# vitoplantamura/OnnxStream

Hardware: AMD Instinct MI355X
Metric: sd15_unet_step_latency_ms+images_per_sec_512x512_20step (higher is better)
Workload: dtype f16

## Files before the change

### include/osgpu.h

```cpp
#ifndef OSGPU_H
#define OSGPU_H

#include <stddef.h>
#include <stdint.h>

#ifdef __cplusplus
extern "C" {
#endif

typedef struct osg_ctx osg_ctx;
typedef struct osg_graph osg_graph;

typedef enum { OSG_U8 = 1, OSG_F16 = 2, OSG_F32 = 3, OSG_I64 = 4 } osg_dtype;

typedef enum {
  OSG_ACT_NONE = 0,
  OSG_ACT_SILU = 1,
  OSG_ACT_SIGMOID = 2,
  OSG_ACT_GEGLU = 3
} osg_act;

typedef enum {
  OSG_UN_SIGMOID = 0,
  OSG_UN_ERF = 1,
  OSG_UN_SQRT = 2,
  OSG_UN_SIN = 3,
  OSG_UN_COS = 4,
  OSG_UN_NEG = 5,
  OSG_UN_POW = 6,
  OSG_UN_SILU = 7,
  OSG_UN_GELU_ERF = 8
} osg_unary_kind;

typedef enum {
  OSG_BIN_ADD = 0,
  OSG_BIN_SUB = 1,
  OSG_BIN_MUL = 2,
  OSG_BIN_DIV = 3
} osg_binary_kind;

int osg_device_count(void);
int osg_init(int device, osg_ctx** out);
void osg_destroy(osg_ctx* ctx);
const char* osg_last_error(const osg_ctx* ctx);
const char* osg_device_name(const osg_ctx* ctx);
void* osg_stream(const osg_ctx* ctx);
int osg_set_autotune(osg_ctx* ctx, int on);
int osg_tune_misses(void);

int osg_malloc(osg_ctx* ctx, size_t bytes, void** dptr);
int osg_free(osg_ctx* ctx, void* dptr);
int osg_upload(osg_ctx* ctx, void* dst, const void* host_src, size_t bytes);
int osg_upload_sync(osg_ctx* ctx, void* dst, const void* host_src, size_t bytes);
int osg_host_register(osg_ctx* ctx, void* host_ptr, size_t bytes);
int osg_host_unregister(osg_ctx* ctx, void* host_ptr);
int osg_upload_pinned(osg_ctx* ctx, void* dst, const void* pinned_host_src, size_t bytes);
int osg_upload_pinned_async(osg_ctx* ctx, void* dst, const void* pinned_host_src, size_t bytes);
int osg_copy_fence(osg_ctx* ctx);
int osg_download(osg_ctx* ctx, void* host_dst, const void* src, size_t bytes);
int osg_marker_record(osg_ctx* ctx, int slot);
int osg_copy_wait_marker(osg_ctx* ctx, int slot);
int osg_copy(osg_ctx* ctx, void* dst, const void* src, size_t bytes);
int osg_memset(osg_ctx* ctx, void* dst, int value, size_t bytes);
int osg_sync(osg_ctx* ctx);

int osg_graph_begin(osg_ctx* ctx);
int osg_graph_end(osg_ctx* ctx, osg_graph** out);
int osg_graph_launch(osg_ctx* ctx, osg_graph* g);
void osg_graph_destroy(osg_graph* g);

int osg_timer_start(osg_ctx* ctx);
int osg_timer_stop(osg_ctx* ctx, float* ms);
int osg_timer_mark(osg_ctx* ctx, int index);
int osg_timer_between(osg_ctx* ctx, int a, int b, float* ms);

void osg_range_push(const char* name);
void osg_range_pop(void);

int osg_conv2d_nhwc(osg_ctx* ctx, osg_dtype dtype, const void* x, const void* w_ohwi, const void* bias, osg_dtype bias_dtype,
                    const void* residual, void* y, int N, int H, int W, int Cin, int Cout, int KH, int KW, int stride_h,
                    int stride_w, int pad_top, int pad_left, int pad_bottom, int pad_right, osg_act act);

int osg_conv2d_nhwc_rb(osg_ctx* ctx, osg_dtype dtype, const void* x, const void* w_ohwi, const void* bias, osg_dtype bias_dtype,
                       const void* image_bias, long image_bias_ld, const void* residual, void* y, int N, int H, int W, int Cin, int Cout,
                       int KH, int KW, int stride_h, int stride_w, int pad_top, int pad_left, int pad_bottom, int pad_right, osg_act act);

int osg_conv2d_nhwc_v(osg_ctx* ctx, osg_dtype dtype, const void* x, const void* w_ohwi, const void* bias, osg_dtype bias_dtype,
                      const void* image_bias, long image_bias_ld, const void* residual, void* y, long y_ld, void* y2, long y2_ld, int N, int H, int W,
                      int Cin, int Cout, int KH, int KW, int stride_h, int stride_w, int pad_top, int pad_left, int pad_bottom, int pad_right,
                      osg_act act);

int osg_gemm(osg_ctx* ctx, osg_dtype dtype, const void* A, const void* B, int b_is_nk, const void* bias, osg_dtype bias_dtype,
             const void* residual, void* C, int M, int N, int K, int batch, long stride_a, long stride_b, long stride_c,
             osg_act act);

int osg_gemm_w8(osg_ctx* ctx, const void* A, const void* Bq_nk, float w_scale, int w_zero_point, const void* bias, osg_dtype bias_dtype,
                const void* residual, void* C, int M, int N, int K, osg_act act);
int osg_conv2d_nhwc_w8(osg_ctx* ctx, const void* x, const void* wq_ohwi, float w_scale, int w_zero_point, const void* bias,
                       osg_dtype bias_dtype, const void* image_bias, long image_bias_ld, const void* residual, void* y, int N, int H, int W,
                       int Cin, int Cout, int KH, int KW, int stride_h, int stride_w, int pad_top, int pad_left, int pad_bottom,
                       int pad_right, osg_act act);
int osg_gemm_w8_v(osg_ctx* ctx, const void* A, const void* Bq_nk, float w_scale, int w_zero_point, const float* w_scale_vec,
                  const float* w_zero_point_vec, const void* bias, osg_dtype bias_dtype, const void* residual, void* C, int M, int N, int K,
                  osg_act act);
int osg_conv2d_nhwc_w8_v(osg_ctx* ctx, const void* x, const void* wq_ohwi, float w_scale, int w_zero_point, const float* w_scale_vec,
                         const float* w_zero_point_vec, const void* bias, osg_dtype bias_dtype, const void* image_bias, long image_bias_ld,
                         const void* residual, void* y, long y_ld, void* y2, long y2_ld, int N, int H, int W, int Cin, int Cout, int KH, int KW,
                         int stride_h, int stride_w, int pad_top, int pad_left, int pad_bottom, int pad_right, osg_act act);

int osg_transpose_kn_to_nk(osg_ctx* ctx, osg_dtype dtype, const void* src_kn, void* dst_nk, int K, int N);
int osg_gemm_ln(osg_ctx* ctx, const void* x, const void* w_nk_folded, const float* c1, const float* c2, float eps, const float* rowstats,
                const void* residual, void* y, int M, int N, int K, osg_act act);
int osg_gemm_rowstats(osg_ctx* ctx, const void* A, const void* B_nk, const void* bias, osg_dtype bias_dtype, const void* residual, void* C,
                      int M, int N, int K, osg_act act, float* rowstats);
int osg_last_route(const osg_ctx* ctx, int out[5]);
int osg_last_epilogue(const osg_ctx* ctx, int out[2]);
int osg_last_kernel(const osg_ctx* ctx, int out[8]);

int osg_gemm_kernarg_check(osg_ctx* ctx, long lda, int splits);
int osg_attention_kernarg_check(osg_ctx* ctx, long kv_stride, int heads, int kv_div);

int osg_attention(osg_ctx* ctx, osg_dtype dtype, const void* q, const void* k, const void* v, void* o, int heads, int Tq, int Tkv,
                  int D, float scale, int k_is_dt);
int osg_attention_strided(osg_ctx* ctx, osg_dtype dtype, const void* q, long q_tok, long q_head, long q_batch, const void* k,
                          long k_tok, long k_head, long k_batch, const void* v, long v_tok, long v_head, long v_batch, void* o,
                          long o_tok, long o_head, long o_batch, int batch, int heads, int Tq, int Tkv, int D, float scale);
typedef struct {
  const void *a1, *x0;
  const void *wo1, *bo1;
  const void *g2, *be2;
  float eps2;
  const void *wq2, *bq2;
  const void *kp, *vtp;
  float scale;
  int Tk;
  const void *wo2, *bo2;
  const void *g3, *be3;
  float eps3;
  const void *w1, *b1, *w2, *b2;
  const void *wpo, *bpo, *xin;
  void *out, *out2;
  long ldo, ldo2;
  int M, rows_per_img, C, heads;
  void* dbg[8];
  int rows_per_block;
} osg_tblock_tail_args;
int osg_tblock_tail_supported(int M, int rows_per_img, int C, int heads, int Tk);
int osg_tblock_tail(osg_ctx* ctx, const osg_tblock_tail_args* a);
int osg_tblock_pack_weight(osg_ctx* ctx, const void* w_nk, int N, int K, void* w_kn8);
size_t osg_tblock_kv_pack_elems(int imgs, int heads, int D);
int osg_tblock_kv_pack_jobs(osg_ctx* ctx, const void* base, long ld, int imgs, int Tk, int heads, int njobs, const int* jobs_dev, void* dst);
int osg_rms_norm(osg_ctx* ctx, osg_dtype dtype, const void* x, const void* w, void* y, long rows, int C, float eps);
int osg_rope(osg_ctx* ctx, osg_dtype dtype, const void* x, const void* cos_t, const void* sin_t, void* y, long bh, long T, int d);
int osg_sdpa(osg_ctx* ctx, osg_dtype dtype, const void* q, const void* k, const void* v, const void* mask, void* o, int batch, int q_heads,
             int kv_heads, int Tq, int Tkv, int D, float scale);

int osg_instance_norm(osg_ctx* ctx, osg_dtype dtype, const void* x, const float* scale, const float* bias, void* y, int rows,
                      long L, int n_scale, float eps);
int osg_group_norm_nhwc(osg_ctx* ctx, osg_dtype dtype, const void* x, const void* gamma, const void* beta, void* y, int N, long HW,
                        int C, int groups, float eps, osg_act act);
int osg_set_stat_sinks(osg_ctx* ctx, void* table0, int groups0, int cpg0, int ch_off0, void* table1, int groups1, int cpg1, int ch_off1, int rows_per_image);
int osg_group_norm_stats_nhwc(osg_ctx* ctx, const void* x, const void* gamma, const void* beta, void* y, int N, long HW, int C, int G, float eps, osg_act act,
                              const void* stat_table);
int osg_layer_norm(osg_ctx* ctx, osg_dtype dtype, const void* x, const void* gamma, const void* beta, void* y, long rows, int C,
                   float eps);
int osg_reduce_mean_last(osg_ctx* ctx, osg_dtype dtype, const void* x, void* y, long rows, long C);
int osg_softmax_last(osg_ctx* ctx, osg_dtype dtype, const void* x, void* y, long rows, long C);

int osg_unary(osg_ctx* ctx, osg_dtype dtype, osg_unary_kind kind, const void* x, void* y, long n, float param);
int osg_binary(osg_ctx* ctx, osg_dtype dtype, osg_binary_kind kind, const void* a, const long* a_shape, const void* b,
               const long* b_shape, void* y, int rank);
int osg_geglu(osg_ctx* ctx, osg_dtype dtype, const void* x, void* y, long rows, long C);

// ... 66 lines not shown
```

### onnxstream_amd/build.py

```python
from __future__ import annotations

import glob
import os
import subprocess
import sys

ROOT = os.path.dirname(os.path.abspath(__file__))
REPO = os.path.dirname(ROOT)
CSRC = os.path.join(ROOT, "csrc")
INC = os.path.join(REPO, "include")
LIB_GPU = os.path.join(ROOT, "libosgpu.so")
LIB_HOST = os.environ.get("OSA_LIB_HOST") or os.path.join(ROOT, "libonnxstream_amd.so")
ORACLE_REF = os.path.join(REPO, "oracle", "_ref", "libonnxstream_ref.so")
HIPCC = os.environ.get("HIPCC", "/opt/rocm/bin/hipcc")
NO_PRELOAD = os.environ.get("OSG_NO_KERNARG_PRELOAD", "") not in ("", "0")
PRELOAD_FLAGS = [] if NO_PRELOAD else ["-mllvm", "-amdgpu-kernarg-preload-count=16"]
LIB_GPU_BUILT = os.path.join(ROOT, "libosgpu_nopreload.so") if NO_PRELOAD else LIB_GPU


def _newer(target, deps):
    if not os.path.exists(target):
        return True
    t = os.path.getmtime(target)
    return any(os.path.getmtime(d) > t for d in deps)


def _run(cmd, **kw):
    r = subprocess.run(cmd, stdout=subprocess.PIPE, stderr=subprocess.STDOUT, text=True, **kw)
    if r.returncode != 0:
        sys.stderr.write(r.stdout)
        raise RuntimeError("build failed: " + " ".join(cmd))
    return r.stdout


def build_gpu(force=False, verbose=False):
    srcs = sorted(glob.glob(os.path.join(CSRC, "osg_*.hip")))
    hdrs = sorted(glob.glob(os.path.join(CSRC, "*.h"))) + [os.path.join(INC, "osgpu.h")]
    objdir = os.path.join(CSRC, "build", "nopreload") if NO_PRELOAD else os.path.join(CSRC, "build")
    os.makedirs(objdir, exist_ok=True)
    objs, procs = [], []
    for s in srcs:
        o = os.path.join(objdir, os.path.basename(s)[:-4] + ".o")
        objs.append(o)
        if force or _newer(o, [s] + hdrs):
            cmd = [HIPCC, "--offload-arch=gfx950", "-O3", "-std=c++17", "-fPIC", "-mllvm", "-amdgpu-mfma-vgpr-form"] + PRELOAD_FLAGS + ["-I" + INC, "-I" + CSRC, "-c", s, "-o", o]
            procs.append((cmd, subprocess.Popen(cmd, stdout=subprocess.PIPE, stderr=subprocess.STDOUT, text=True)))
    for cmd, p in procs:
        out, _ = p.communicate()
        if p.returncode != 0:
            sys.stderr.write(out)
            raise RuntimeError("build failed: " + " ".join(cmd))
        if verbose and out:
            print(out)
    if force or procs or _newer(LIB_GPU_BUILT, objs):
        _run([HIPCC, "--offload-arch=gfx950", "-shared", "-fPIC", "-o", LIB_GPU_BUILT] + objs)
    return LIB_GPU_BUILT


def build_host(force=False):
    hdir = os.path.join(CSRC, "host")
    srcs = sorted(glob.glob(os.path.join(hdir, "*.cpp")))
    if not srcs:
        return None
    hdrs = sorted(glob.glob(os.path.join(hdir, "*.h"))) + sorted(glob.glob(os.path.join(hdir, "*.inc"))) + [os.path.join(INC, "osgpu.h")]
    if force or _newer(LIB_HOST, srcs + hdrs):
        _run(["g++", "-std=c++20", "-O2", "-fPIC", "-shared", "-I" + INC, "-I" + hdir, "-o", LIB_HOST] + srcs +
             ["-ldl", "-lpthread"])
    return LIB_HOST


def build_oracle_ref():
    if os.path.isdir("/root/reference/src"):
        _run(["make", "-C", os.path.join(REPO, "oracle"), "ref"])
    return ORACLE_REF if os.path.exists(ORACLE_REF) else None


def build_all(force=False):
    build_gpu(force)
    build_host(force)
    build_oracle_ref()


if __name__ == "__main__":
    build_all("--force" in sys.argv)
    print("built:", LIB_GPU, LIB_HOST if os.path.exists(LIB_HOST) else "(no host yet)")
```

### onnxstream_amd/csrc/host/backend.h

```cpp
#pragma once

#include <dlfcn.h>

#include <stdexcept>
#include <string>

#include "osgpu.h"

namespace onnxstream {

#define OSG_API_LIST(X) \
    X(osg_device_count) X(osg_init) X(osg_destroy) X(osg_last_error) X(osg_device_name) X(osg_stream) \
    X(osg_set_autotune) X(osg_malloc) X(osg_free) X(osg_upload) X(osg_upload_sync) X(osg_host_register) \
    X(osg_host_unregister) X(osg_upload_pinned) X(osg_upload_pinned_async) X(osg_copy_fence) X(osg_download) X(osg_copy) X(osg_memset) X(osg_sync) \
    X(osg_graph_begin) X(osg_graph_end) X(osg_graph_launch) X(osg_graph_destroy) \
    X(osg_timer_start) X(osg_timer_stop) X(osg_conv2d_nhwc) X(osg_conv2d_nhwc_rb) X(osg_conv2d_nhwc_v) X(osg_set_stat_sinks) X(osg_group_norm_stats_nhwc) X(osg_gemm) \
    X(osg_gemm_ln) X(osg_gemm_rowstats) X(osg_gemm_w8) X(osg_conv2d_nhwc_w8) X(osg_gemm_w8_v) X(osg_conv2d_nhwc_w8_v) X(osg_transpose_kn_to_nk) X(osg_attention) \
    X(osg_attention_strided) X(osg_sdpa) X(osg_rms_norm) X(osg_rope) X(osg_instance_norm) X(osg_group_norm_nhwc) X(osg_layer_norm) \
    X(osg_reduce_mean_last) X(osg_softmax_last) X(osg_unary) X(osg_binary) X(osg_geglu) X(osg_transpose) \
    X(osg_copy_2d) X(osg_concat2) X(osg_resize_nearest) X(osg_gather_rows) X(osg_maxpool_nhwc) X(osg_convert) \
    X(osg_sampler_prepare) X(osg_sampler_cfg_euler_a) X(osg_sampler_cfg_multistep) X(osg_sampler_prepare_rescale) X(osg_sampler_prepare_single) X(osg_sampler_euler_a_single) X(osg_sampler_multistep_single) X(osg_decode_gather) X(osg_decode_blend) X(osg_qu8_conv2d_nhwc) X(osg_qu8_conv2d_nhwc_t) X(osg_qu8_conv_tap_sums) X(osg_qu8_gemm) X(osg_qu8_lut) X(osg_qu8_binary) \
    X(osg_qu8_instance_norm) X(osg_qu8_instance_norm_nhwc) X(osg_qu8_affine_act) X(osg_qu8_norm_affine_act_nhwc) X(osg_qu8_softmax_last) X(osg_range_push) X(osg_range_pop) X(osg_marker_record) \
    X(osg_copy_wait_marker) X(osg_timer_mark) X(osg_timer_between) X(osg_tblock_tail_supported) X(osg_tblock_tail) X(osg_tblock_kv_pack_elems) X(osg_tblock_kv_pack_jobs) X(osg_tblock_pack_weight)

struct OsgApi {
#define OSG_FN(name) decltype(&::name) name = nullptr;
    OSG_API_LIST(OSG_FN)
#undef OSG_FN
};

class HipBackend {
public:
    OsgApi api;
    osg_ctx* ctx = nullptr;

    explicit HipBackend(int device) {
        std::string path;
        if (const char* e = std::getenv("OSGPU_LIB")) path = e;
        if (path.empty()) {
            Dl_info info;
            if (dladdr((void*)&HipBackend::anchor, &info) && info.dli_fname) {
                std::string self = info.dli_fname;
                auto p = self.find_last_of('/');
                path = (p == std::string::npos ? std::string(".") : self.substr(0, p)) + "/libosgpu.so";
            } else {
                path = "libosgpu.so";
            }
        }
        m_handle = dlopen(path.c_str(), RTLD_NOW | RTLD_LOCAL);
        if (!m_handle) throw std::runtime_error("HipBackend: unable to load " + path + ": " + dlerror() + " (no CPU fallback exists)");
#define OSG_FN(name)                                                                                   \
    api.name = reinterpret_cast<decltype(api.name)>(dlsym(m_handle, #name));                           \
    if (!api.name) throw std::runtime_error(std::string("HipBackend: symbol missing in libosgpu.so: ") + #name);
        OSG_API_LIST(OSG_FN)
#undef OSG_FN
        if (api.osg_device_count() <= 0)
            throw std::runtime_error("HipBackend: no HIP device visible; the MI355X backend has no CPU fallback");
        int rc = api.osg_init(device, &ctx);
        if (rc) throw std::runtime_error("HipBackend: osg_init(device " + std::to_string(device) + ") failed with code " + std::to_string(rc));
    }

    ~HipBackend() {
        if (ctx) api.osg_destroy(ctx);
    }

    HipBackend(const HipBackend&) = delete;
    HipBackend& operator=(const HipBackend&) = delete;

    void check(int rc, const char* what) const {
        if (rc) throw std::runtime_error(std::string(what) + ": " + api.osg_last_error(ctx));
    }

    void* malloc(size_t bytes) {
        void* p = nullptr;
        check(api.osg_malloc(ctx, bytes, &p), "osg_malloc");
        return p;
    }
    void free(void* p) { if (p) api.osg_free(ctx, p); }

private:
    static void anchor() {}
    void* m_handle = nullptr;
};

}
```

### onnxstream_amd/csrc/host/exports.cpp

```cpp
#include <cstdio>
#include <cstring>

#include "onnxstream.h"
#include "plan.h"

using namespace onnxstream;

namespace {

char* dup_cstr(const std::string& s) {
    char* p = (char*)std::malloc(s.size() + 1);
    std::memcpy(p, s.c_str(), s.size() + 1);
    return p;
}

struct Handle {
    explicit Handle(int threads) : model(threads) {}
    Model model;
    std::string definition;
    std::string provider;
};

const char* dtype_name(TensorDataType t) {
    switch (t) {
// ... 119 lines not shown
            r->data_num = t.get_vector<float>().size();
            r->data = t.get_vector<float>().data();
            return r;
        }
    return nullptr;
}

void* model_hip_get_tensor_batch(Handle* h, char* name, unsigned int index) {
    struct Ret {
        size_t dims_num;
        size_t* dims;
        size_t data_num;
        float* data;
    };
    for (auto& t : h->model.m_data)
        if (t.m_name == name) {
            Tensor* src = &t;
            if (index > 0) {
                if (!t.m_batch || index - 1 >= t.m_batch->size()) return nullptr;
                src = &(*t.m_batch)[index - 1];
            }
            if (src->m_type != TensorDataType::float32) return nullptr;
            Ret* r = (Ret*)std::malloc(sizeof(Ret));
            r->dims_num = src->m_shape.size();
            r->dims = src->m_shape.data();
            r->data_num = src->get_vector<float>().size();
            r->data = src->get_vector<float>().data();
            return r;
        }
    return nullptr;
}

char* model_get_all_tensor_names(Handle* h) {
    std::string out;
    for (auto& t : h->model.m_data) out += (out.empty() ? "" : "|") + t.m_name;
    return dup_cstr(out);
}

void model_run(Handle* h) {
    try {
        h->model.run();
    } catch (const std::exception& e) {
        printf("=== ERROR === %s\n", e.what());
        throw;
    }
}

char* model_run_2(Handle* h) {
    try {
        h->model.run();
        return nullptr;
    } catch (const std::exception& e) {
        return dup_cstr(e.what());
    }
}

void model_clear_tensors(Handle* h) { h->model.m_data.clear(); }

void model_set_option(Handle* h, char* name, unsigned int value) {
    Model& m = h->model;
    const std::string n = name;
    const bool b = value != 0;
    if (n == "use_fp16_arithmetic") m.m_use_fp16_arithmetic = b;
    else if (n == "use_uint8_qdq") m.m_use_uint8_qdq = b;
    else if (n == "use_uint8_arithmetic") m.m_use_uint8_arithmetic = b;
    else if (n == "fuse_ops_in_attention") m.m_fuse_ops_in_attention = b;
    else if (n == "force_fp16_storage") m.m_force_fp16_storage = b;
    else if (n == "support_dynamic_shapes") m.m_support_dynamic_shapes = b;
    else if (n == "use_ops_cache") m.m_use_ops_cache = b;
    else if (n == "use_scaled_dp_attn_op") m.m_use_scaled_dp_attn_op = b;
    else if (n == "use_next_op_cache") m.m_use_next_op_cache = b;
    else if (n == "ops_printf") m.m_ops_printf = b;
    else if (n == "ops_times_printf") m.m_ops_times_printf = b;
    else if (n == "use_nchw_convs") m.m_use_nchw_convs = b;
    else if (n == "range_data_calibrate") m.m_range_data_calibrate = b;
    else if (n == "attention_fused_ops_parts") m.m_attention_fused_ops_parts = value;
    else if (n == "hip_device") m.m_hip_device = (int)value;
    else if (n == "hip_fusion_level") m.m_hip_fusion_level = (int)value;
    else if (n == "hip_use_graph") m.m_hip_use_graph = b;
    else if (n == "hip_autotune") m.m_hip_autotune = b;
    else if (n == "hip_fuse_ln_gemm") m.m_hip_fuse_ln_gemm = b;
    else if (n == "hip_concat_views") m.m_hip_concat_views = b;
    else if (n == "hip_fuse_tblock") m.m_hip_fuse_tblock = b;
    else if (n == "hip_gn_stats") m.m_hip_gn_stats = (int)value;
    else if (n == "hip_stream_weights") m.m_hip_stream_weights = b;
    else if (n == "hip_w8_resident") m.m_hip_w8_resident = b;
    else if (n == "hip_resident_outputs") m.m_hip_resident_outputs = b;
    else {
        const char* err = "model_set_option: 'name' not found.";
        printf("=== ERROR === %s\n", err);
        throw std::invalid_argument(err);
    }
}

void model_add_extra_output(Handle* h, char* name) { h->model.m_extra_outputs.emplace_back(name); }

void model_free_buffer(void* ptr) { std::free(ptr); }

double model_hip_last_pass_ms(Handle* h) { return h->model.hip_last_pass_ms(); }
unsigned long long model_hip_last_kernel_count(Handle* h) { return h->model.hip_last_kernel_count(); }
void model_hip_invalidate_plan(Handle* h) { h->model.hip_invalidate_plan(); }
unsigned long long model_hip_plans_built(Handle* h) { return h->model.hip_plans_built(); }
unsigned long long model_hip_streamed_bytes(Handle* h) { return h->model.hip_streamed_bytes(); }
unsigned long long model_hip_resident_weight_bytes(Handle* h) { return h->model.hip_resident_weight_bytes(); }
void model_hip_set_vram_budget(Handle* h, unsigned long long bytes) { h->model.set_cuda_options(CudaOptions(bytes, false)); }
void model_hip_set_upcast_substrings(Handle* h, const char* list) {
    std::vector<std::string> subs;
    std::string cur;
    for (const char* p = list ? list : ""; ; p++) {
        if (*p == '|' || *p == 0) {
            if (!cur.empty()) subs.push_back(cur);
            cur.clear();
            if (!*p) break;
        } else cur.push_back(*p);
    }
    if (subs.empty()) h->model.m_requires_upcast = nullptr;
    else
        h->model.m_requires_upcast = [subs](const std::string&, const std::string& name) {
            for (auto& s : subs)
                if (name.find(s) != std::string::npos) return true;
            return false;
        };
    h->model.hip_invalidate_plan();
}
void model_hip_add_outputs_convert(Handle* h, char* name) { h->model.m_outputs_convert_set.insert(name); }
int model_hip_drop_tensor(Handle* h, char* name) {
    auto& d = h->model.m_data;
    for (size_t i = 0; i < d.size(); i++)
        if (d[i].m_name == name) { d.erase(d.begin() + i); return 1; }
    return 0;
}
char* model_hip_fetch_tensor(Handle* h, char* name) {
    try {
        h->model.hip_fetch_tensor(name);
        return nullptr;
    } catch (const std::exception& e) {
        return dup_cstr(e.what());
    }
}
int model_hip_rename_tensor(Handle* h, char* from, char* to) {
    for (auto& t : h->model.m_data)
        if (t.m_name == from) { t.m_name = to; return 1; }
    return 0;
}
char* model_hip_replay(Handle* h, int n, float* ms_each) {
    try {
        h->model.hip_replay(n, ms_each);
        return nullptr;
    } catch (const std::exception& e) {
        return dup_cstr(e.what());
    }
}
char* model_hip_set_input(Handle* h, char* name, long long index, const float* data, unsigned long long count) {
    try {
        h->model.hip_set_input(name, (long)index, data, (size_t)count);
        return nullptr;
    } catch (const std::exception& e) {
        return dup_cstr(e.what());
    }
}
char* model_hip_sampler_loop(Handle* h, char* sample_name, char* timestep_name, char* out_name, int steps, int prompts, float* x, const float* noise,
                             const float* c_in, const float* c_out, const float* t, const float* sigma, const float* d_sigma, const float* sigma_up, float guidance, const float* clip,
                             double* ms) {
    try {
        const double v = h->model.hip_sampler_loop(sample_name, timestep_name, out_name, steps, prompts, x, noise, c_in, c_out, t, sigma, d_sigma, sigma_up, guidance, clip);
        if (ms) *ms = v;
// ... 85 lines not shown
```

### onnxstream_amd/csrc/host/lowering_graph.inc

```
    static bool wants_f32(const Operation& op, size_t idx) {
        if (op.m_type == "InstanceNormalization" && (idx == 1 || idx == 2)) return true;
        if (op.m_type == "Resize") return true;
        if (op.m_type == "Pow" && idx == 1) return true;
        return false;
    }

    template <typename T>
    tensor_vector<T> fetch(WeightsProvider* wp, const std::string& fn) {
        if constexpr (std::is_same_v<T, uint8_t>) return wp->get_uint8(fn);
        else if constexpr (std::is_same_v<T, uint16_t>) return wp->get_float16(fn);
        else if constexpr (std::is_same_v<T, float>) return wp->get_float32(fn);
        else return wp->get_int64(fn);
    }

    struct Occ { std::string fn, key; Shape shape; Lay lay; osg_dtype want; long count; };
    Occ resolve(const Operation& op, size_t i, const Tensor& t, TensorDataType ty) const {
        Occ o;
        o.fn = t.m_name;
        o.shape = to_shape(t.m_shape);
        o.lay = Lay::plain;
        auto pos = o.fn.find("_nchw.bin");
        if (pos != std::string::npos) {
            if (o.shape.size() == 3) o.shape.push_back(1);
            if (o.shape.size() != 4) throw std::invalid_argument("Model::get_tensor_data: layout is nhwc but invalid shape.");
// ... 249 lines not shown
            return (sh.size() == 3 && sh[0] == C) || (sh.size() == 4 && sh[1] == C);
        };
        for (size_t i = 0; i < ops().size(); i++) {
            if (!is((int)i, "Mul")) continue;
            Operation& mu = ops()[i];
            if (mu.m_input.size() != 2 || mu.m_output.size() != 1) continue;
            int xi = -1;
            for (int k = 0; k < 2; k++)
                if (act(mu.m_input[k]) && mu.m_input[k].m_shape.size() == 4 && mu.m_input[k].m_shape[0] == 1 && chan_const(mu.m_input[1 - k], (long)mu.m_input[k].m_shape[1])) xi = k;
            if (xi < 0) continue;
            const Tensor x = mu.m_input[xi], gam = mu.m_input[1 - xi];
            const long C = (long)x.m_shape[1];
            const int ad = sole_consumer(mu.m_output[0]);
            if (!is(ad, "Add") || ops()[ad].m_input.size() != 2) continue;
            const int bidx = other(ops()[ad], mu.m_output[0].m_name);
            if (!chan_const(ops()[ad].m_input[bidx], C)) continue;
            const Tensor bet = ops()[ad].m_input[bidx];
            int sg = -1, m2 = -1;
            const std::string& an = ops()[ad].m_output[0].m_name;
            if (use_count(an) == 2) {
                auto it = consumers.find(an);
                if (it != consumers.end() && it->second.size() == 2) {
                    for (int c : it->second)
                        if (is(c, "Sigmoid")) sg = c;
                        else if (is(c, "Mul")) m2 = c;
                    if (sg >= 0 && m2 >= 0 && sole_consumer(ops()[sg].m_output[0]) == m2 && ops()[m2].m_input.size() == 2) {
                        const std::string &p0 = ops()[m2].m_input[0].m_name, &p1 = ops()[m2].m_input[1].m_name, &sn = ops()[sg].m_output[0].m_name;
                        if (!((p0 == an && p1 == sn) || (p0 == sn && p1 == an))) sg = m2 = -1;
                    } else
                        sg = m2 = -1;
                }
            }
            const bool silu = sg >= 0 && m2 >= 0;
            if (!silu && use_count(an) != 1) {
            }
            Operation f;
            const int last = silu ? m2 : ad;
            f.m_name = ops()[last].m_name;
            f.m_type = "osg.qu8.AffineAct";
            f.m_input = {x, gam, bet};
            f.m_output = {ops()[last].m_output[0]};
            f.m_attributes = {{"mul", mu.m_name}, {"add", ops()[ad].m_name}};
            if (silu) {
                f.m_attributes.emplace_back("sigmoid", ops()[sg].m_name);
                f.m_attributes.emplace_back("mul2", ops()[m2].m_name);
            }
            const int nrm = prod_of(x);
            if (is(nrm, "osg.qu8.InstanceNormNHWC") && use_count(x.m_name) == 1) {
                f.m_type = "osg.qu8.NormAffineAct";
                f.m_input = {ops()[nrm].m_input[0], gam, bet, ops()[nrm].m_input[1], ops()[nrm].m_input[2]};
                f.m_attributes.emplace_back("norm", ops()[nrm].m_name);
                for (auto& a : ops()[nrm].m_attributes) f.m_attributes.emplace_back("norm_" + a.first, a.second);
                dead[nrm] = 1;
            }
            dead[i] = 1;
            if (silu) dead[ad] = dead[sg] = 1;
            ops()[last] = std::move(f);
        }
    }

    void run_fusions() {
        dead.assign(ops().size(), 0);
        if (P.u8 && m.m_hip_fusion_level >= 1 && has_type("InstanceNormalization")) { index_graph(); fuse_u8_instance_norm_nhwc(); }
        if (P.u8 && m.m_hip_fusion_level >= 1 && has_type("Mul") && has_type("Add")) { index_graph(); fuse_u8_affine_act(); }
        if (m.m_use_scaled_dp_attn_op && has_type("Softmax")) { index_graph(); fuse_sdpa(); }
        if (P.fusion >= 1) {
            if (m.m_requires_upcast && has_type("Pow") && has_type("ReduceMean")) { index_graph(); fuse_rms_norm(); }
            if (has_type("Neg") && has_type("Slice")) { index_graph(); fuse_rope(); }
            if (has_type("Sigmoid")) { index_graph(); fuse_silu(); }
            if (has_type("InstanceNormalization")) { index_graph(); fuse_group_norm(); }
            if (has_type("ReduceMean") && has_type("Sub")) { index_graph(); fuse_layer_norm(); }
            if (has_type("Erf")) { index_graph(); fuse_geglu(); }
        }
        if (P.fusion >= 2) {
            if (has_type("Softmax")) { index_graph(); fuse_attention(true); }
            if (has_type("MatMul")) { index_graph(); fuse_linear(); }
            if (has_type("Conv") || has_type("osg.Linear")) { index_graph(); fuse_residual(); }
            if (has_type("Conv")) { index_graph(); fuse_conv_act(); }
            if (has_type("osg.GEGLU")) { index_graph(); fuse_linear_geglu(); }
            if (has_type("osg.Attention") && has_type("osg.LayerNorm")) { index_graph(); fuse_tblock_tail(); }
            if (has_type("osg.SiLU")) { index_graph(); cse_silu(); }
            if (has_type("osg.SiLU") && has_type("Gemm")) { index_graph(); fuse_gemm_act(); }
            if (has_type("Conv")) { index_graph(); fuse_image_bias(); }
        } else if (m.m_fuse_ops_in_attention && has_type("Softmax")) {
            index_graph(); fuse_attention(false);
        }
        std::vector<Operation> live;
        for (size_t i = 0; i < ops().size(); i++)
            if (!dead[i]) live.push_back(std::move(ops()[i]));
        ops() = std::move(live);
    }

    void fuse_silu() {
        for (size_t i = 0; i < ops().size(); i++) {
            if (!is((int)i, "Sigmoid")) continue;
            Operation& sg = ops()[i];
            if (sg.m_input.size() != 1 || sg.m_output.size() != 1 || !act(sg.m_input[0])) continue;
            int j = sole_consumer(sg.m_output[0]);
            if (!is(j, "Mul")) continue;
            Operation& mul = ops()[j];
            if (mul.m_input.size() != 2) continue;
            const std::string& s = sg.m_output[0].m_name;
            int o = other(mul, s);
            if (mul.m_input[o].m_name != sg.m_input[0].m_name || mul.m_input[1 - o].m_name != s) continue;
            mul.m_type = "osg.SiLU";
            Tensor x = mul.m_input[o];
            mul.m_input.clear();
            mul.m_input.push_back(x);
            dead[i] = 1;
        }
    }

    void fuse_group_norm() {
        for (size_t i = 0; i < ops().size(); i++) {
            if (!is((int)i, "InstanceNormalization")) continue;
            Operation& in = ops()[i];
            if (in.m_input.size() != 3 || in.m_output.size() != 1) continue;
            const Val* sc = cval(in.m_input[1]);
            const Val* bi = cval(in.m_input[2]);
            if (!sc || !bi || !sc->host_valid || !bi->host_valid) continue;
            bool unit = true;
            for (float f : sc->host_f) unit &= f == 1.0f;
            for (float f : bi->host_f) unit &= f == 0.0f;
            if (!unit) continue;
            int r0 = prod_of(in.m_input[0]);
            if (!is(r0, "Reshape") || use_count(in.m_input[0].m_name) != 1) continue;
            const Tensor& x = ops()[r0].m_input[0];
            if (!act(x) || x.m_shape.size() != 4) continue;
            if (in.m_input[0].m_shape.size() != 3 || in.m_input[0].m_shape[0] != 1) continue;
            long G = (long)in.m_input[0].m_shape[1];
            int r1 = sole_consumer(in.m_output[0]);
            if (!is(r1, "Reshape") || ops()[r1].m_output[0].m_shape != x.m_shape) continue;
            int mu = sole_consumer(ops()[r1].m_output[0]);
            if (!is(mu, "Mul")) continue;
            int gi = other(ops()[mu], ops()[r1].m_output[0].m_name);
            const Val* gam = cval(ops()[mu].m_input[gi]);
            long C = (long)x.m_shape[1];
            auto chan_shape = [&](const Val* v) {
                if (!v || v->numel() != C) return false;
                const Shape& s = v->shape;
                return (s.size() == 3 && s[0] == C) || (s.size() == 4 && s[1] == C);
            };
            if (!chan_shape(gam)) continue;
            int ad = sole_consumer(ops()[mu].m_output[0]);
            if (!is(ad, "Add")) continue;
            int bidx = other(ops()[ad], ops()[mu].m_output[0].m_name);
            if (!chan_shape(cval(ops()[ad].m_input[bidx]))) continue;
            if (C % G || x.m_shape[0] != 1) continue;
            float eps = 1e-5f;
            if (auto* e = attr(in, "epsilon")) eps = std::stof(*e);
            int last = ad;
            bool silu = false;
            int sl = sole_consumer(ops()[ad].m_output[0]);
            if (is(sl, "osg.SiLU")) { silu = true; last = sl; }
            Operation f;
            f.m_name = in.m_name + "_GroupNorm";
            f.m_type = "osg.GroupNorm";
            f.m_input = {x, ops()[mu].m_input[gi], ops()[ad].m_input[bidx]};
            f.m_output = {ops()[last].m_output[0]};
            f.m_attributes = {{"groups", std::to_string(G)}, {"epsilon", std::to_string(eps)}, {"silu", silu ? "1" : "0"}};
            char buf[64];
            snprintf(buf, sizeof buf, "%.9g", eps);
            f.m_attributes[1].second = buf;
            for (int k : {r0, (int)i, r1, mu, ad}) dead[k] = 1;
            if (silu) dead[sl] = 1;
            dead[last] = 0;
// ... 547 lines not shown
            if (op.m_output.size() != 1 || attr(op, "osg_residual")) continue;
            if (attr(op, "osg_act")) continue;
            int ad = sole_consumer(op.m_output[0]);
            if (!is(ad, "Add")) continue;
            int ti = other(ops()[ad], op.m_output[0].m_name);
            const Tensor& t = ops()[ad].m_input[ti];
            const auto& os = op.m_output[0].m_shape;
            if (!act(t) || os.size() != 4 || t.m_shape != std::vector<size_t>{1, os[1], 1, 1}) continue;
            int u1 = prod_of(t);
            if (!is(u1, "Unsqueeze") || use_count(t.m_name) != 1) continue;
            int u0 = prod_of(ops()[u1].m_input[0]);
            if (!is(u0, "Unsqueeze") || use_count(ops()[u1].m_input[0].m_name) != 1) continue;
            const Tensor g = ops()[u0].m_input[0];
            if (!act(g) || g.m_shape != std::vector<size_t>{1, os[1]} || use_count(g.m_name) != 1) continue;
            Operation f = op;
            while (f.m_input.size() < 4) f.m_input.push_back(Tensor());
            f.m_input.push_back(g);
            f.m_attributes.emplace_back("osg_image_bias", "1");
            f.m_output = {ops()[ad].m_output[0]};
            dead[i] = dead[u0] = dead[u1] = 1;
            ops()[ad] = std::move(f);
        }
    }

    void fuse_linear() {
        for (size_t i = 0; i < ops().size(); i++) {
            if (!is((int)i, "MatMul")) continue;
            Operation& mm = ops()[i];
            const Val* w = cval(mm.m_input[1]);
            if (!act(mm.m_input[0]) || !w || w->shape.size() != 2) continue;
            mm.m_type = "osg.Linear";
            int ad = sole_consumer(mm.m_output[0]);
            if (!is(ad, "Add")) continue;
            int bi = other(ops()[ad], mm.m_output[0].m_name);
            const Val* b = cval(ops()[ad].m_input[bi]);
            if (!b || b->shape.size() != 1 || b->shape[0] != w->shape[1]) continue;
            Operation f = mm;
            f.m_input.push_back(ops()[ad].m_input[bi]);
            f.m_output = {ops()[ad].m_output[0]};
            dead[i] = 1;
            ops()[ad] = std::move(f);
        }
    }

    void fuse_residual() {
        for (size_t i = 0; i < ops().size(); i++) {
            const bool conv = is((int)i, "Conv"), lin = is((int)i, "osg.Linear");
            if (!conv && !lin) continue;
            Operation& op = ops()[i];
            if (op.m_output.size() != 1) continue;
            if (attr(op, "osg_residual")) continue;
            int ad = sole_consumer(op.m_output[0]);
            if (!is(ad, "Add")) continue;
            int ri = other(ops()[ad], op.m_output[0].m_name);
            const Tensor& r = ops()[ad].m_input[ri];
            if (!act(r) || r.m_shape != op.m_output[0].m_shape || r.m_name == op.m_output[0].m_name) continue;
            if (conv && op.m_output[0].m_shape.size() != 4) continue;
            Operation f = op;
            if (conv && f.m_input.size() == 2) f.m_input.push_back(Tensor());
            if (lin && f.m_input.size() == 2) f.m_input.push_back(Tensor());
            f.m_input.push_back(r);
            f.m_attributes.emplace_back("osg_residual", "1");
            f.m_output = {ops()[ad].m_output[0]};
            dead[i] = 1;
            ops()[ad] = std::move(f);
        }
    }

    void fuse_conv_act() {
        for (size_t i = 0; i < ops().size(); i++) {
            if (!is((int)i, "Conv")) continue;
            Operation& op = ops()[i];
            if (op.m_output.size() != 1 || attr(op, "osg_act")) continue;
            int sl = sole_consumer(op.m_output[0]);
            if (!is(sl, "osg.SiLU") || ops()[sl].m_input.size() != 1) continue;
            Operation f = op;
            f.m_attributes.emplace_back("osg_act", "silu");
            f.m_output = {ops()[sl].m_output[0]};
            dead[i] = 1;
            ops()[sl] = std::move(f);
        }
    }

    void fuse_gemm_act() {
        for (size_t i = 0; i < ops().size(); i++) {
            if (!is((int)i, "Gemm")) continue;
            Operation& op = ops()[i];
            if (op.m_output.size() != 1 || op.m_input.size() != 3 || attr(op, "osg_act")) continue;
            const Val* w = cval(op.m_input[1]);
            if (!w || (w->dtype != OSG_F16 && w->dtype != OSG_U8)) continue;
            int sl = sole_consumer(op.m_output[0]);
            if (!is(sl, "osg.SiLU") || ops()[sl].m_input.size() != 1) continue;
            Operation f = op;
            f.m_attributes.emplace_back("osg_act", "silu");
            f.m_output = {ops()[sl].m_output[0]};
            dead[i] = 1;
            ops()[sl] = std::move(f);
        }
    }

    int in_val_raw(const Tensor& t) {
        if (is_const_tensor(t)) return const_val(t);
        auto it = P.by_name.find(t.m_name);
        if (it == P.by_name.end()) throw std::invalid_argument("Model::get_tensor_data: input tensor not found: " + t.m_name);
        const int r = P.root_of(it->second);
        if (V(r).host_only && !V(r).dptr) {
            const size_t bytes = std::max<size_t>(P.val_bytes(r), 8);
            V(r).dptr = P.small_alloc(bytes);
            if (V(r).dtype == OSG_I64) be.check(be.api.osg_upload_sync(be.ctx, V(r).dptr, V(r).host_i.data(), V(r).host_i.size() * 8), "osg_upload_sync");
            else if (V(r).dtype == OSG_F32 && P.fp16) {
                std::vector<uint16_t> h(V(r).host_f.size());
                for (size_t k = 0; k < h.size(); k++) h[k] = float_to_half(V(r).host_f[k]);
                be.check(be.api.osg_upload_sync(be.ctx, V(r).dptr, h.data(), h.size() * 2), "osg_upload_sync");
                V(r).dtype = OSG_F16;
            } else if (V(r).dtype == OSG_F32) be.check(be.api.osg_upload_sync(be.ctx, V(r).dptr, V(r).host_f.data(), V(r).host_f.size() * 4), "osg_upload_sync");
            else throw std::invalid_argument("Model::get_tensor_data: unsupported tensor data format.");
        }
        return it->second;
    }
    const Val* hval(const Tensor& t) const {
        if (is_const_tensor(t)) return &P.vals[const_val(t)];
        auto it = P.by_name.find(t.m_name);
        if (it == P.by_name.end()) return nullptr;
        const Val& v = P.vals[it->second];
        return v.host_valid && v.host_only ? &v : nullptr;
    }
    int host_val(const Operation& op, const Shape& shape, std::vector<int64_t> ints, std::vector<float> floats = {}) {
        const bool is_int = floats.empty();
        check_out(op, shape);
        int v = P.new_val(op.m_output[0].m_name, shape, is_int ? OSG_I64 : OSG_F32, Lay::plain, false);
        V(v).is_const = true;
        V(v).host_valid = V(v).host_only = true;
        V(v).host_i = std::move(ints);
        V(v).host_f = std::move(floats);
        return v;
    }

    struct HT {
        Shape shape;
        bool is_int = true;
        std::vector<double> v;
        long numel() const { return (long)v.size(); }
    };
    static HT to_ht(const Val* v) {
        HT h;
        h.shape = v->shape;
        h.is_int = v->dtype == OSG_I64;
        if (h.is_int) h.v.assign(v->host_i.begin(), v->host_i.end());
        else h.v.assign(v->host_f.begin(), v->host_f.end());
        return h;
    }
    int host_out(const Operation& op, HT h) {
        if (h.is_int) {
            std::vector<int64_t> o(h.v.size());
            for (size_t k = 0; k < o.size(); k++) o[k] = (int64_t)h.v[k];
            return host_val(op, h.shape, std::move(o));
        }
        std::vector<float> f(h.v.size());
        for (size_t k = 0; k < f.size(); k++) f[k] = (float)h.v[k];
        check_out(op, h.shape);
        int v = P.new_val(op.m_output[0].m_name, h.shape, OSG_F32, Lay::plain, false);
        V(v).is_const = true;
        V(v).host_valid = V(v).host_only = true;
        V(v).host_f = std::move(f);
        return v;
    }
// ... 293 lines not shown
```

### onnxstream_amd/csrc/host/lowering_ops.inc

```
    void lower(const Operation& op) {
        const std::string& t = op.m_type;
        if (try_host_eval(op)) return;
        if (P.u8) return lower_u8(op);
        if (t == "Gather") return lower_gather(op);
        if (t == "Cast") return lower_cast(op);
        if (t == "Conv") {
            conv1d_out = Conv1dOut{};
            lower_conv(op);
            if (conv1d_out.y >= 0) {
                check_out(op, {1, conv1d_out.Cout, conv1d_out.Lo});
                P.alias(P.ensure_plain(conv1d_out.y), {1, conv1d_out.Cout, conv1d_out.Lo}, Lay::plain, op.m_output[0].m_name);
            }
            return;
        }
        if (t == "MatMul") return lower_matmul(op);
        if (t == "osg.Linear") return lower_linear(op);
        if (t == "Gemm") return lower_gemm(op);
        if (t == "Add" || t == "Sub" || t == "Mul" || t == "Div") return lower_binary(op);
        if (t == "Sigmoid" || t == "Erf" || t == "Sqrt" || t == "Sin" || t == "Cos" || t == "Neg" || t == "osg.SiLU") return lower_unary(op);
        if (t == "Pow") return lower_pow(op);
        if (t == "InstanceNormalization") return lower_instance_norm(op);
        if (t == "osg.GroupNorm") return lower_group_norm(op);
        if (t == "osg.LayerNorm") return lower_layer_norm(op);
        if (t == "osg.GEGLU") return lower_geglu(op);
        if (t == "osg.Attention") return lower_attention(op);
        if (t == "osg.TBlockTail") return lower_tblock_tail(op);
        if (t == "AttentionFusedOps") return lower_attention_fused_ops(op);
        if (t == "ScaledDotProductAttention") return lower_sdpa(op);
        if (t == "Expand") return lower_expand(op);
        if (t == "osg.RMSNorm") return lower_rms_norm(op);
        if (t == "osg.RoPE") return lower_rope(op);
        if (t == "ReduceMean") return lower_reduce_mean(op);
        if (t == "Softmax") return lower_softmax(op);
        if (t == "Reshape") return lower_reshape(op);
        if (t == "Flatten") return lower_flatten(op);
        if (t == "Unsqueeze" || t == "Squeeze") return lower_squeeze(op, t == "Unsqueeze");
        if (t == "Transpose") return lower_transpose(op);
        if (t == "Concat") return lower_concat(op);
        if (t == "Split") return lower_split(op);
        if (t == "Slice") return lower_slice(op);
        if (t == "Resize") return lower_resize(op);
        if (t == "MaxPool") return lower_maxpool(op);
        throw std::invalid_argument("Model::run: operation not implemented on the HIP backend: " + t);
    }

    static void need(const Operation& op, bool cond, const char* msg) {
        if (!cond) throw std::invalid_argument(op.m_type + ": " + msg);
    }

    struct RsProducer { size_t step; int a, w, bias, res, y; long M, N, K; };
    std::map<int, RsProducer> rs_producers;
    void note_rs_producer(int a, int w, int bias, int res, int y, long M, long Nn, long K) {
        if (P.fusion < 2 || !P.fuse_ln_gemm || Nn % 32 || K % 64 || Nn > 1280) return;
        rs_producers[P.root_of(y)] = RsProducer{P.steps.size() - 1, a, w, bias, res, y, M, Nn, K};
    }
    int upgrade_rs_producer(int x, long rows, long C) {
        auto it = rs_producers.find(P.root_of(x));
        if (it == rs_producers.end()) return -1;
        const RsProducer r = it->second;
        if (r.M != rows || r.N != C || V(x).view_off != 0 || r.step >= P.steps.size()) return -1;
        if (viewed_steps.count(r.step)) return -1;
        {
            auto cpit = conv_producers.find(P.root_of(r.y));
            if (cpit != conv_producers.end() && (cpit->second.out->sink[0].off >= 0 || cpit->second.out->sink[1].off >= 0)) return -1;
        }
        if (V(r.y).batched != V(x).batched) return -1;
        int rs = P.new_val("", {r.M / (V(x).batched ? N : 1), C / 32, 2}, OSG_F32, Lay::plain, V(x).batched);
        Step& st = P.steps[r.step];
        st.writes.push_back(rs);
        st.what += " +rowstats";
        const int a = r.a, w = r.w, bias = r.bias, res = r.res, y = r.y;
        const long M = r.M, Nn = r.N, K = r.K;
        const std::string what = st.what;
        st.run = [=, this] {
            be.check(be.api.osg_gemm_rowstats(be.ctx, P.ptr(a), P.ptr(w), bias >= 0 ? P.ptr(bias) : nullptr, bias >= 0 ? P.vals[bias].dtype : OSG_F16,
                                              res >= 0 ? P.ptr(res) : nullptr, P.ptr(y), (int)M, (int)Nn, (int)K, OSG_ACT_NONE, (float*)P.ptr(rs)),
                     what.c_str());
        };
        rs_producers.erase(it);
        conv_producers.erase(P.root_of(y));
        return rs;
    }

    struct StatSinkRef { long off = -1; int groups = 0, cpg = 0, ch_off = 0; };
    struct ConvOut { int dst; long dst_ld = 0; size_t dst_off = 0; int dst2 = -1; long dst2_ld = 0; size_t dst2_off = 0; StatSinkRef sink[2]; int sink_hw = 0; bool no_sinks = false; };
    struct ConcatPart { std::shared_ptr<ConvOut> out; int slot; long ch_off; size_t step; };
    std::map<int, std::vector<ConcatPart>> concat_parts;
    struct ConvProducer { size_t step; std::shared_ptr<ConvOut> out; int y; };
    std::map<int, ConvProducer> conv_producers;
    std::set<size_t> viewed_steps;

    struct Conv1dOut { int y = -1; long Cout = 0, Lo = 0; } conv1d_out;
    void lower_conv(const Operation& op) {
        const bool has_res = attr(op, "osg_residual") != nullptr;
        const bool has_ib = attr(op, "osg_image_bias") != nullptr;
        const osg_act cact = attr(op, "osg_act") ? OSG_ACT_SILU : OSG_ACT_NONE;
        const size_t nin = op.m_input.size();
        need(op, nin == 2 || nin == 3 || (has_res && nin == 4) || (has_ib && nin == 5), "wrong number of inputs.");
        need(op, op.m_output.size() == 1, "wrong number of outputs.");
        std::vector<int> dil = {1, 1}, ks, pads = {0, 0, 0, 0}, strides = {1, 1};
        int group = 1;
        for (auto& a : op.m_attributes) {
            if (a.first == "dilations") dil = int_list(a.second);
            else if (a.first == "group") group = std::stoi(a.second);
            else if (a.first == "kernel_shape") ks = int_list(a.second);
            else if (a.first == "pads") pads = int_list(a.second);
            else if (a.first == "strides") strides = int_list(a.second);
            else if (a.first == "osg_residual" || a.first == "osg_image_bias" || a.first == "osg_act") {}
            else throw std::invalid_argument(op.m_type + ": unrecognized attribute: " + a.first + ".");
        }
        int x = in_val(op.m_input[0]);
        const bool is1d = V(x).shape.size() == 3;
        for (auto& a : op.m_attributes)
            if (a.first == "dilations") need(op, (dil.size() == 1) == is1d, "invalid dilations attribute value.");
        if (is1d) {
            need(op, !has_res && !has_ib, "Conv1D with fused epilogue inputs not implemented on the HIP backend.");
            bool have_pads = false, have_strides = false, have_dil = false;
            for (auto& a : op.m_attributes) { have_pads |= a.first == "pads"; have_strides |= a.first == "strides"; have_dil |= a.first == "dilations"; }
            if (have_dil) { need(op, dil.size() == 1, "invalid dilations attribute value."); dil.push_back(1); }
            if (!ks.empty()) { need(op, ks.size() == 1, "invalid kernel_shape attribute value."); ks.push_back(1); }
            if (have_pads) { need(op, pads.size() == 2, "invalid pads attribute value."); pads = {pads[0], 0, pads[1], 0}; }
            if (have_strides) { need(op, strides.size() == 1, "invalid strides attribute value."); strides.push_back(strides[0]); }
            Shape s4 = V(x).shape;
            s4.push_back(1);
            x = P.alias(P.ensure_plain(x), s4, Lay::plain);
        }
        need(op, V(x).shape.size() == 4, "invalid shape of input.");
        for (int d : dil) need(op, d == 1, "dilations != 1 not supported (not implemented).");
        need(op, group == 1, "group != 1 not supported (not implemented).");
        need(op, pads.size() == 4 && strides.size() == 2, "invalid pads/strides.");
        x = P.ensure_nhwc(x);
        int w = in_val(op.m_input[1]);
        const Shape ws = V(w).shape;
        need(op, V(w).is_const && V(w).lay == Lay::nhwc && ws.size() == 4, "weights must be a static *_nchw.bin tensor.");
        const Shape xs = V(x).shape;
        need(op, xs[0] == 1, "batch size must be 1 (push several samples instead).");
        const long Cin = xs[1], H = xs[2], W = xs[3], Cout = ws[0], KH = ws[2], KW = ws[3];
        need(op, ws[1] == Cin, "invalid shape of weights.");
        if (!ks.empty()) need(op, ks.size() == 2 && ks[0] == KH && ks[1] == KW, "kernel_shape does not match the weights.");
        const int ph = pads[0] + pads[2], pw = pads[1] + pads[3];
        const int pt = ph / 2, pb = ph - pt, pl = pw / 2, pr = pw - pl;
        const long Ho = (H + ph - KH) / strides[0] + 1, Wo = (W + pw - KW) / strides[1] + 1;
        int bias = -1;
        if (nin >= 3 && !op.m_input[2].m_name.empty()) {
            bias = in_val(op.m_input[2]);
            need(op, V(bias).numel() == Cout, "invalid shape of bias.");
        }
        int res = -1;
        if (has_res) res = P.ensure_nhwc(in_val(op.m_input[3]));
        int ib = -1;
        long ib_ld = 0;
        if (has_ib) {
            ib = in_val_raw(op.m_input[4]);
            need(op, V(ib).numel() == Cout && V(ib).dtype == OSG_F16 && V(ib).batched == V(x).batched, "invalid image bias.");
            ib_ld = V(ib).ld ? V(ib).ld : Cout;
        }
        int y = is1d ? P.new_val("", {1, Cout, Ho, Wo}, OSG_F16, Lay::nhwc, V(x).batched) : out_val(op, {1, Cout, Ho, Wo}, Lay::nhwc, V(x).batched);
        if (is1d) conv1d_out = Conv1dOut{y, Cout, Ho};
        const long nb = B(x);
        const int sh = strides[0], sw = strides[1];
        std::vector<int> reads = {x, w};
        if (bias >= 0) reads.push_back(bias);
        if (res >= 0) reads.push_back(res);
        if (ib >= 0) reads.push_back(ib);
        const bool w8 = V(w).dtype == OSG_U8;
        const float qs = w8 ? V(w).qscale : 0.f;
        const int qz = w8 ? V(w).qzp : 0;
        auto co = std::make_shared<ConvOut>();
        co->dst = y;
        P.add_step((w8 ? "Conv w8 " : "Conv ") + op.m_name, reads, {y}, [=, this] {
            const ConvOut& o = *co;
            if (o.sink[0].off >= 0 || o.sink[1].off >= 0)
                be.check(be.api.osg_set_stat_sinks(be.ctx, o.sink[0].off >= 0 ? P.gn_stats + o.sink[0].off : nullptr, o.sink[0].groups, o.sink[0].cpg, o.sink[0].ch_off,
                                                   o.sink[1].off >= 0 ? P.gn_stats + o.sink[1].off : nullptr, o.sink[1].groups, o.sink[1].cpg, o.sink[1].ch_off, o.sink_hw),
                         "osg_set_stat_sinks");
            if (w8)
                be.check(be.api.osg_conv2d_nhwc_w8_v(be.ctx, P.ptr(x), P.ptr(w), qs, qz, nullptr, nullptr, bias >= 0 ? P.ptr(bias) : nullptr,
                                                     bias >= 0 ? P.vals[bias].dtype : OSG_F16, ib >= 0 ? P.ptr(ib) : nullptr, ib_ld,
                                                     res >= 0 ? P.ptr(res) : nullptr, (char*)P.ptr(o.dst) + o.dst_off, o.dst_ld,
                                                     o.dst2 >= 0 ? (char*)P.ptr(o.dst2) + o.dst2_off : nullptr, o.dst2_ld, (int)nb, (int)H, (int)W, (int)Cin,
                                                     (int)Cout, (int)KH, (int)KW, sh, sw, pt, pl, pb, pr, cact),
                         "Conv");
            else
            be.check(be.api.osg_conv2d_nhwc_v(be.ctx, OSG_F16, P.ptr(x), P.ptr(w), bias >= 0 ? P.ptr(bias) : nullptr,
                                              bias >= 0 ? P.vals[bias].dtype : OSG_F16, ib >= 0 ? P.ptr(ib) : nullptr, ib_ld,
                                              res >= 0 ? P.ptr(res) : nullptr, (char*)P.ptr(o.dst) + o.dst_off, o.dst_ld,
                                              o.dst2 >= 0 ? (char*)P.ptr(o.dst2) + o.dst2_off : nullptr, o.dst2_ld, (int)nb, (int)H, (int)W, (int)Cin, (int)Cout,
                                              (int)KH, (int)KW, sh, sw, pt, pl, pb, pr, cact),
                     "Conv");
        });
        P.steps.back().flops = 2.0 * nb * Ho * Wo * Cout * KH * KW * Cin;
        if (V(w).dtype == OSG_F16 || w8) conv_producers[P.root_of(y)] = ConvProducer{P.steps.size() - 1, co, y};
        if (KH == 1 && KW == 1 && sh == 1 && sw == 1 && ph == 0 && pw == 0 && ib < 0 && cact == OSG_ACT_NONE)
            if (!w8) note_rs_producer(x, w, bias, res, y, nb * Ho * Wo, Cout, Cin);
    }

    int weight_nk(int w) {
        Val& wv = V(w);
        if (wv.as_nhwc >= 0) return wv.as_nhwc;
        const long K = wv.shape[0], Nn = wv.shape[1];
        int t = P.new_val("", {Nn, K}, OSG_F16, Lay::plain, false);
        Val& tv = V(t);
        tv.is_const = true;
        tv.name = V(w).name + "|nk";
        size_t bytes = (size_t)K * Nn * 2;
        bool fresh;
        tv.dptr = P.const_alloc(tv.name, bytes, &fresh);
        if (fresh) be.check(be.api.osg_transpose_kn_to_nk(be.ctx, OSG_F16, P.ptr(w), tv.dptr, (int)K, (int)Nn), "osg_transpose_kn_to_nk");
        V(w).as_nhwc = t;
        return t;
    }

    int weight_nk_u8(int w) {
        if (V(w).as_nk_u8 >= 0) return V(w).as_nk_u8;
        const long K = V(w).shape[0], Nn = V(w).shape[1];
        int t = P.new_val("", {Nn, K}, OSG_U8, Lay::plain, false);
        V(t).is_const = true;
        V(t).name = V(w).name + "|nk_u8";
        V(t).qscale = V(w).qscale;
        V(t).qzp = V(w).qzp;
        bool fresh;
        V(t).dptr = P.const_alloc(V(t).name, (size_t)K * Nn, &fresh);
        if (fresh) {
            long shape[2] = {K, Nn};
            int perm[2] = {1, 0};
            be.check(be.api.osg_transpose(be.ctx, 1, P.ptr(w), V(t).dptr, 2, shape, perm), "osg_transpose");
            be.check(be.api.osg_sync(be.ctx), "osg_sync");
        }
        V(w).as_nk_u8 = t;
        return t;
    }

    void emit_gemm_w8q(const std::string& what, int a, int wq, int qv, int bias, int res, int y, long M, long Nn, long K, osg_act act_ = OSG_ACT_NONE) {
        const float qs = V(wq).qscale;
        const int qz = V(wq).qzp;
        std::vector<int> reads = {a, wq};
        if (qv >= 0) reads.push_back(qv);
        if (bias >= 0) reads.push_back(bias);
        if (res >= 0) reads.push_back(res);
        P.add_step(what, reads, {y}, [=, this] {
            const float* sc = qv >= 0 ? (const float*)P.ptr(qv) : nullptr;
            be.check(be.api.osg_gemm_w8_v(be.ctx, P.ptr(a), P.ptr(wq), qs, qz, sc, sc ? sc + Nn : nullptr, bias >= 0 ? P.ptr(bias) : nullptr,
                                          bias >= 0 ? P.vals[bias].dtype : OSG_F16, res >= 0 ? P.ptr(res) : nullptr, P.ptr(y), (int)M, (int)Nn, (int)K, act_),
                     what.c_str());
        });
        P.steps.back().flops = 2.0 * M * Nn * K;
    }
    void emit_gemm_w8(const std::string& what, int a, int w, int bias, int res, int y, long M, long Nn, long K, osg_act act_ = OSG_ACT_NONE) {
        emit_gemm_w8q(what, a, weight_nk_u8(w), -1, bias, res, y, M, Nn, K, act_);
    }

    struct LnFold { int x, g, b; float eps; long C; int rs; };

    void emit_gemm(const std::string& what, int a, int wnk, int bias, int res, int y, long M, long Nn, long K, long batch, long sa, long sb,
                   long sc, int b_is_nk, osg_act act_ = OSG_ACT_NONE) {
        std::vector<int> reads = {a, wnk};
        if (bias >= 0) reads.push_back(bias);
        if (res >= 0) reads.push_back(res);
        P.add_step(what, reads, {y}, [=, this] {
            be.check(be.api.osg_gemm(be.ctx, OSG_F16, P.ptr(a), P.ptr(wnk), b_is_nk, bias >= 0 ? P.ptr(bias) : nullptr,
                                     bias >= 0 ? P.vals[bias].dtype : OSG_F16, res >= 0 ? P.ptr(res) : nullptr, P.ptr(y), (int)M, (int)Nn,
                                     (int)K, (int)batch, sa, sb, sc, act_),
                     what.c_str());
        });
        P.steps.back().flops = 2.0 * M * Nn * K * batch;
        if (b_is_nk && batch == 1 && V(y).ld == 0 && act_ == OSG_ACT_NONE) note_rs_producer(a, wnk, bias, res, y, M, Nn, K);
    }

    struct LinGroup {
        std::vector<int> members;
        std::vector<long> off;
        long ntot = 0;
        int y = -1;
    };
    bool indexed = false;
    std::vector<LinGroup> groups;
    std::map<int, std::pair<int, int>> group_of;
// ... 1254 lines not shown
```

### onnxstream_amd/csrc/host/model.cpp

```cpp
#include "onnxstream.h"

#include <algorithm>
#include <cstring>

#include <thread>

#include "backend.h"
#include "plan.h"
#include <chrono>
#include <cstdio>
#include <cstdlib>

namespace onnxstream {

std::string& trim(std::string& s) {
    const char* ws = " \t\n\r\f\v";
    s.erase(s.find_last_not_of(ws) + 1);
    s.erase(0, s.find_first_not_of(ws));
    return s;
}

namespace {

std::vector<std::string> split(const std::string& s, char delim) {
    std::vector<std::string> out;
    size_t b = 0;
    for (;;) {
        size_t e = s.find(delim, b);
        if (e == std::string::npos) {
            out.emplace_back(s.substr(b));
            return out;
        }
        out.emplace_back(s.substr(b, e - b));
        b = e + 1;
    }
}

}

Model::Model(int threads_count) {
    m_backend_wanted = threads_count >= 0;
    m_threads = threads_count > 0 ? (size_t)threads_count : std::max(1u, std::thread::hardware_concurrency());
}

Model::~Model() {
    m_data.clear();
    delete m_plan;
    m_alive.reset();
    if (m_pool && m_backend) m_pool->clear(*m_backend);
    delete m_pool;
    delete m_backend;
}

void Model::hip_fetch_tensor(const std::string& name) {
    for (auto& t : m_data)
        if (t.m_name == name) {
            if (!t.m_hip_resident) return;
            if (!m_backend) throw std::runtime_error("Model::hip_fetch_tensor: no backend.");
            tensor_vector<uint16_t> host(t.m_hip_resident_bytes / 2);
            m_backend->check(m_backend->api.osg_download(m_backend->ctx, host.data(), t.m_hip_resident.get(), t.m_hip_resident_bytes), "osg_download");
            t.set_vector(std::move(host));
            t.m_hip_resident.reset();
            t.m_hip_resident_bytes = 0;
            return;
        }
    throw std::invalid_argument("Model::hip_fetch_tensor: tensor not found: " + name);
}

void Model::set_cuda_options(const CudaOptions& options) { m_cuda_options = options; }

void Model::read_file(const char* filename) {
    m_model = onnxstream::read_file<std::vector<char>>(filename);
    std::string fn(filename);
    auto sep = fn.find_last_of("/\\");
    m_path = sep == std::string::npos ? std::string() : fn.substr(0, sep + 1);
    get_wp()->m_path = m_path;
    m_ops_parsed = false;
    m_init_done = false;
    hip_invalidate_plan();
    if (m_pool && m_backend) m_pool->clear(*m_backend);
}

void Model::read_string(const char* string, const char* path_with_slash) {
    m_model.assign(string, string + std::strlen(string));
    m_path = path_with_slash;
    get_wp()->m_path = m_path;
    m_ops_parsed = false;
    m_init_done = false;
    hip_invalidate_plan();
    if (m_pool && m_backend) m_pool->clear(*m_backend);
}

std::string Model::next_line() {
    const size_t n = m_model.size();
    while (m_pos < n && (m_model[m_pos] == '\r' || m_model[m_pos] == '\n')) m_pos++;
    const size_t start = m_pos;
    while (m_pos < n && m_model[m_pos] != '\r' && m_model[m_pos] != '\n') m_pos++;
    return std::string(m_model.data() + start, m_pos - start);
}

Tensor Model::parse_tensor_string(std::string& str) {
    Tensor t;
    if (str.empty()) return t;
    const auto open = str.find('(');
    if (open == std::string::npos || open == 0 || str.back() != ')' || str.find('(', open + 1) != std::string::npos ||
        str.size() < open + 2)
        throw std::invalid_argument("Model::parse_tensor_string: invalid tensor format.");
    t.m_name = str.substr(0, open);
    std::string inner = str.substr(open + 1, str.size() - open - 2);

    std::string shape = inner;
    const auto fields = split(inner, ':');
    if (fields.size() == 2) {
        const std::string& ty = fields[0];
        shape = fields[1];
        if (ty.rfind("uint8[", 0) == 0 && ty.back() == ']') {
            auto rng = split(ty.substr(6, ty.size() - 7), ',');
            if (rng.size() != 2) throw std::invalid_argument("Model::parse_tensor_string: invalid uint8 range.");
            t.m_type = TensorDataType::uint8;
            t.m_scale = (float)std::stod(rng[0]);
            t.m_zero_point = (uint8_t)std::stoi(rng[1]);
        } else if (ty == "float16") t.m_type = TensorDataType::float16;
        else if (ty == "float32") t.m_type = TensorDataType::float32;
        else if (ty == "int64") t.m_type = TensorDataType::int64;
        else throw std::invalid_argument("Model::parse_tensor_string: unsupported tensor data format.");
    } else if (fields.size() != 1) {
        throw std::invalid_argument("Model::parse_tensor_string: invalid tensor format.");
    }
    if (!shape.empty())
        for (auto& d : split(shape, ',')) {
            int i = std::stoi(d);
            if (i < 0) throw std::invalid_argument("Model::parse_tensor_string: invalid shape (dim < 0).");
            if (i == 0 && !m_support_dynamic_shapes) throw std::invalid_argument("Model::parse_tensor_string: invalid shape (dim == 0).");
            t.m_shape.push_back((size_t)i);
// ... 191 lines not shown
```

### onnxstream_amd/csrc/host/plan.cpp

```cpp
#include "plan.h"
#include "qu8.h"

#include <algorithm>
#include <chrono>
#include <cmath>
#include <cstdio>
#include <cstring>
#include <thread>
#include <string_view>
#include <unordered_map>
#include <unordered_set>

namespace onnxstream {

namespace {

using Shape = std::vector<long>;

long prod(const Shape& s, size_t from = 0, size_t to = (size_t)-1) {
    long n = 1;
    for (size_t i = from; i < std::min(to, s.size()); i++) n *= s[i];
    return n;
}

Shape to_shape(const std::vector<size_t>& s) { return Shape(s.begin(), s.end()); }

std::string shape_str(const Shape& s) {
    std::string r = "(";
    for (size_t i = 0; i < s.size(); i++) r += (i ? "," : "") + std::to_string(s[i]);
    return r + ")";
}

std::vector<int> int_list(const std::string& s) {
    std::vector<int> out;
    size_t b = 0;
    while (b <= s.size()) {
        size_t e = s.find(',', b);
        if (e == std::string::npos) e = s.size();
        if (e > b) out.push_back(std::stoi(s.substr(b, e - b)));
        b = e + 1;
    }
    return out;
}

const std::string* attr(const Operation& op, const char* key) {
    for (auto& a : op.m_attributes)
        if (a.first == key) return &a.second;
    return nullptr;
}

size_t esize(osg_dtype d) { return d == OSG_U8 ? 1 : d == OSG_F16 ? 2 : d == OSG_F32 ? 4 : 8; }


uint16_t float_to_half(float f) {
    uint32_t x;
    std::memcpy(&x, &f, 4);
    const uint32_t sign = (x >> 16) & 0x8000u;
    int32_t e = (int32_t)((x >> 23) & 0xff) - 127 + 15;
    uint32_t m = x & 0x7fffffu;
    if (((x >> 23) & 0xff) == 0xff) return (uint16_t)(sign | 0x7c00u | (m ? 0x200u : 0));
    if (e >= 31) return (uint16_t)(sign | 0x7c00u);
    if (e <= 0) {
        if (e < -10) return (uint16_t)sign;
        m |= 0x800000u;
        const int shift = 14 - e;
        uint32_t hm = m >> shift;
        const uint32_t rem = m & ((1u << shift) - 1), half = 1u << (shift - 1);
        if (rem > half || (rem == half && (hm & 1))) hm++;
        return (uint16_t)(sign | hm);
    }
    uint32_t h = ((uint32_t)e << 10) | (m >> 13);
    const uint32_t rem = m & 0x1fffu;
    if (rem > 0x1000u || (rem == 0x1000u && (h & 1))) h++;
    return (uint16_t)(sign | h);
}

bool is_const_tensor(const Tensor& t) { return !t.m_name.empty() && t.m_type != TensorDataType::none; }

}

Plan::Plan(Model& model, HipBackend& backend, ConstPool& cpool, size_t batch) : m(model), be(backend), pool(cpool), N((long)batch) {
    fp16 = m.m_use_fp16_arithmetic;
    fusion = fusion_req = m.m_hip_fusion_level;
    stream_weights = m.m_hip_stream_weights;
    vram_budget = (size_t)m.m_cuda_options.m_vram_to_use;
    budgeted = vram_budget > 0;
    if (budgeted) stream_weights = true;
    w8_resident = m.m_hip_w8_resident && !stream_weights;
    fuse_ln_gemm = m.m_hip_fuse_ln_gemm;
    concat_views = m.m_hip_concat_views;
    fuse_tblock = m.m_hip_fuse_tblock;
    gn_stats_req = m.m_hip_gn_stats;
    gn_stats_min_elems = m.m_hip_gn_stats == 2 ? (8L << 20) : 0;
    gn_stats_on = m.m_hip_gn_stats != 0 && !stream_weights && m.m_hip_fusion_level >= 2 && !m.m_use_uint8_arithmetic && !m.m_range_data_calibrate;
    u8 = m.m_use_uint8_arithmetic;
    u8_qdq = m.m_use_uint8_qdq;
    autotune = m.m_hip_autotune;
    calibrate = m.m_range_data_calibrate;
    fuse_attn = m.m_fuse_ops_in_attention;
    sdp_attn = m.m_use_scaled_dp_attn_op;
    outputs_convert_set = m.m_outputs_convert_set;
    extra_outputs = m.m_extra_outputs;
    recycle = m.m_support_dynamic_shapes && !stream_weights;
    resident_outputs = m.m_hip_resident_outputs && m.m_support_dynamic_shapes && !stream_weights && !m.m_outputs_convert_set.empty();
}

bool Plan::compatible(Model& mm, size_t batch) const {
    static const bool say = getenv("OSG_PLAN_TIMING") != nullptr;
    auto no = [&](const char* why) {
        if (say) fprintf(stderr, "[plan] re-plan: %s\n", why);
        return false;
    };
    const bool want_stream = mm.m_hip_stream_weights || mm.m_cuda_options.m_vram_to_use > 0;
    if ((long)batch != N) return no("batch size");
    if (mm.m_use_fp16_arithmetic != fp16 || mm.m_use_uint8_arithmetic != u8 || mm.m_use_uint8_qdq != u8_qdq) return no("arithmetic type");
    if (mm.m_hip_fusion_level != fusion_req || mm.m_hip_fuse_ln_gemm != fuse_ln_gemm || mm.m_hip_concat_views != concat_views || mm.m_hip_fuse_tblock != fuse_tblock || mm.m_hip_gn_stats != gn_stats_req ||
        mm.m_fuse_ops_in_attention != fuse_attn || mm.m_use_scaled_dp_attn_op != sdp_attn || mm.m_hip_autotune != autotune)
        return no("fusion / tuning options");
    if (want_stream != stream_weights || (size_t)mm.m_cuda_options.m_vram_to_use != vram_budget ||
        (mm.m_hip_w8_resident && !want_stream) != w8_resident)
        return no("weight residency options");
    if (mm.m_extra_outputs != extra_outputs || mm.m_outputs_convert_set != outputs_convert_set ||
        (mm.m_hip_resident_outputs && mm.m_support_dynamic_shapes && !want_stream && !mm.m_outputs_convert_set.empty()) != resident_outputs)
        return no("output set");
    if (mm.m_range_data_calibrate != calibrate) return no("calibration mode");
    for (auto& in : inputs)
        for (auto& t : mm.m_data)
            if (t.m_name == in.name) {
                if (t.m_type != in.host_type || t.m_shape != in.shape) return no("an input's type or shape");
                if (t.m_hip_resident != in.resident) return no("a device-resident input");
                if (t.m_type == TensorDataType::int64) {
                    auto& v = t.get_vector<int64_t>();
                    if (v.size() != in.ivals.size() || !std::equal(v.begin(), v.end(), in.ivals.begin())) return no("an int64 input's values");
                }
            }
    return true;
}

int Plan::new_val(const std::string& name, const Shape& shape, osg_dtype dt, Lay lay, bool batched) {
    Val v;
    v.name = name;
    v.shape = shape;
    v.dtype = dt;
    v.lay = lay;
    v.batched = batched;
    vals.push_back(std::move(v));
    int id = (int)vals.size() - 1;
    if (!name.empty()) by_name[name] = id;
    return id;
}

int Plan::root_of(int v) const {
    while (vals[v].root >= 0) v = vals[v].root;
    return v;
}

int Plan::alias(int v, const Shape& shape, Lay lay, const std::string& name) {
    Val a;
    a.name = name;
    a.shape = shape;
    a.dtype = vals[v].dtype;
    a.lay = lay;
    a.batched = vals[v].batched;
    a.is_const = vals[v].is_const;
    a.root = v;
    a.qscale = vals[v].qscale;
    a.qzp = vals[v].qzp;
    a.qdyn = vals[v].qdyn;
    a.host_f = vals[v].host_f;
    a.host_i = vals[v].host_i;
    a.host_valid = vals[v].host_valid;
    vals.push_back(std::move(a));
    int id = (int)vals.size() - 1;
    if (!name.empty()) by_name[name] = id;
    return id;
}

const Val& Plan::qv(int v) const {
    for (int guard = 0; guard < 64; guard++) {
        if (vals[v].qown) break;
        if (vals[v].qsrc >= 0) v = vals[v].qsrc;
        else if (vals[v].root >= 0) v = vals[v].root;
        else break;
    }
    return vals[v];
}

void Plan::share_q(int dst, int src) {
    if (vals[src].dtype != OSG_U8 || dst == src) return;
    int s = src;
    while (!vals[s].qown && vals[s].qsrc < 0 && vals[s].root >= 0) s = vals[s].root;
    if (!vals[s].qown && vals[s].qsrc >= 0) s = vals[s].qsrc;
    int d = dst;
    while (!vals[d].qown && vals[d].root >= 0) d = vals[d].root;
    if (d == s) return;
    vals[d].qsrc = s;
    vals[d].qscale = vals[s].qscale;
    vals[d].qzp = vals[s].qzp;
    vals[d].qdyn = vals[s].qdyn;
// ... 137 lines not shown
        long shape[3] = {b, C, HW};
        int perm[3] = {0, 2, 1};
        be.check(be.api.osg_transpose(be.ctx, es, ptr(v), ptr(o), 3, shape, perm), "osg_transpose");
    });
    vals[v].as_nhwc = o;
    share_q(o, v);
    return o;
}

struct Lowering {
    Plan& P;
    Model& m;
    HipBackend& be;
    long N;
    std::unordered_map<std::string, int> uses;
    std::unordered_map<std::string, int> producer;
    std::unordered_map<std::string, std::vector<int>> consumers;
    std::vector<char> dead;
    std::map<std::string, int> const_cache;

    explicit Lowering(Plan& p) : P(p), m(p.m), be(p.be), N(p.N) {}

    std::vector<Operation>& ops() { return P.ops; }
    Val& V(int v) { return P.vals[v]; }
    osg_dtype act_dtype() const { return OSG_F16; }

#include "lowering_graph.inc"
#include "lowering_u8.inc"
#include "lowering_ops.inc"
};

Plan::~Plan() {
    if (in_flight) be.api.osg_sync(be.ctx);
    steps.clear();
    steps.shrink_to_fit();
    delete lowering;
    lowering = nullptr;
    for (auto& o : outputs)
        if (o.dev) pool.give_class(be, o.dev, ConstPool::size_class(o.dev_bytes));
    for (auto& r : recyclable) pool.give(be, r.first, r.second);
    for (auto& kv : registered) be.api.osg_host_unregister(be.ctx, (void*)kv.first);
    if (graph) be.api.osg_graph_destroy(graph);
    if (samp_x) be.api.osg_free(be.ctx, samp_x);
    if (samp_noise) be.api.osg_free(be.ctx, samp_noise);
    if (samp_hist) be.api.osg_free(be.ctx, samp_hist);
    if (dec_lat) be.api.osg_free(be.ctx, dec_lat);
    if (dec_img) be.api.osg_free(be.ctx, dec_img);
    if (dec_pix) be.api.osg_free(be.ctx, dec_pix);
    if (ring) be.free(ring);
    for (void* p : owned) be.free(p);
    if (arena && !arena_pooled) be.free(arena);
}

void Plan::build() {
    if (!fp16 && !u8)
        throw std::runtime_error("Model::run: the HIP backend implements f16 arithmetic (m_use_fp16_arithmetic, the configuration the reference uses for "
                                 "the SD UNet, src/sd.cpp:1633) and uint8 arithmetic (m_use_uint8_arithmetic, src/sd.cpp:1218); fp32 arithmetic is not implemented.");
    if (m.m_use_uint8_qdq)
        throw std::runtime_error("Model::run: m_use_uint8_qdq (uint8 storage between fp32 ops) is not implemented on the HIP backend.");
    if (m.m_requires_upcast && u8)
        throw std::runtime_error("Model::run: m_requires_upcast with uint8 arithmetic is not implemented on the HIP backend.");
    if (calibrate) {
        if (u8) throw std::invalid_argument("Model::run: m_range_data_calibrate runs in floating-point arithmetic (src/sd.cpp:1216-1222), not with m_use_uint8_arithmetic.");
        fusion = 0;
    }
    if (calibrate && stream_weights)
        throw std::invalid_argument("Model::run: m_range_data_calibrate cannot be combined with streamed weights (hip_stream_weights / a VRAM budget) on the HIP backend: calibrate with resident weights.");
    if (u8) {
        if (N != 1) throw std::invalid_argument("Model::run: uint8 arithmetic runs one sample per pass on the HIP backend (every pushed sample is quantised with its own scale).");
        fusion = 0;
    }
    be.check(be.api.osg_set_autotune(be.ctx, m.m_hip_autotune ? 1 : 0), "osg_set_autotune");
    static const bool timing = std::getenv("OSG_PLAN_TIMING") != nullptr;
    auto now = [] { return std::chrono::steady_clock::now(); };
    auto ms_since = [&](std::chrono::steady_clock::time_point t0) { return std::chrono::duration<double, std::milli>(now() - t0).count(); };
    const auto t_begin = now();
    vals.reserve(m.m_ops.size() * 12 + 1024);
    lowering = new Lowering(*this);
    Lowering& L = *lowering;
    std::string key;
    const bool cacheable = m.m_support_dynamic_shapes && !stream_weights && !budgeted;
    if (cacheable) {
        key = std::to_string(fusion) + "|" + std::to_string(m.m_hip_fusion_level) + (u8 ? "|u8" : "|f") + (fp16 ? "h" : "-") + (w8_resident ? "8" : "-") + (fuse_attn ? "a" : "-") +
              (sdp_attn ? "s" : "-") + (fuse_ln_gemm ? "l" : "-") + "|" + std::to_string(m.m_attention_fused_ops_parts) + "|" + std::to_string(m.m_ops.size()) + "|";
        for (auto& e : extra_outputs) key += e + ",";
        key += "|";
        if (m.m_requires_upcast)
            for (auto& op : m.m_ops) key += m.m_requires_upcast(op.m_type, op.m_name) ? '1' : '0';
    }
    const bool reuse = cacheable && pool.complete && pool.fused_valid && pool.fused_key == key && pool.snap_vals.size() == pool.fused_const_vals && !pool.snap_vals.empty();
    if (reuse) {
        vals.assign(pool.snap_vals.begin(), pool.snap_vals.end());
        weight_bytes = pool.snap_weight_bytes;
        ops = pool.fused_ops;
        L.dead.assign(ops.size(), 0);
    } else {
        ops = m.m_ops;
        L.load_weights();
    }
    const double t_weights = ms_since(t_begin);
    const size_t n_const_vals_after_load = vals.size();

    {
        std::vector<std::string> found;
        if (!(reuse && !pool.in_names.empty())) {
            std::unordered_set<std::string_view> produced, seen;
            produced.reserve(m.m_ops.size() * 2);
            for (auto& op : m.m_ops)
                for (auto& o : op.m_output) produced.insert(o.m_name);
            for (auto& op : m.m_ops)
                for (auto& in : op.m_input) {
                    if (in.m_name.empty() || in.m_type != TensorDataType::none || produced.count(in.m_name) || seen.count(in.m_name)) continue;
                    seen.insert(in.m_name);
                    found.push_back(in.m_name);
                }
            if (cacheable) pool.in_names = found;
        }
        for (const std::string& iname : (reuse && !pool.in_names.empty()) ? pool.in_names : found) {
            Tensor* src = nullptr;
            for (auto& t : m.m_data)
                if (t.m_name == iname) { src = &t; break; }
            if (!src) throw std::invalid_argument("Model::get_tensor_data: input tensor not found: " + iname);
            if (src->m_type != TensorDataType::float32 && src->m_type != TensorDataType::int64 && !(src->m_type == TensorDataType::float16 && fp16 && !u8))
                throw std::invalid_argument("Model::run: graph inputs must be float32, float16 (fp16 arithmetic) or int64 host tensors on the HIP backend (" + iname + ").");
            Shape shape = to_shape(src->m_shape);
            In inp;
            inp.name = iname;
            inp.host_type = src->m_type;
            inp.shape = src->m_shape;
            if (src->m_type == TensorDataType::int64) {
                if (u8 || N != 1) throw std::invalid_argument("Model::run: int64 graph inputs need one sample per pass and floating-point arithmetic (" + iname + ").");
                auto& iv = src->get_vector<int64_t>();
                inp.ivals.assign(iv.begin(), iv.end());
                inp.staging = inp.val = new_val(iname, shape, OSG_I64, Lay::plain, false);
                vals[inp.val].is_const = true;
                vals[inp.val].host_valid = vals[inp.val].host_only = true;
                vals[inp.val].host_i = inp.ivals;
                inputs.push_back(std::move(inp));
                continue;
            }
            if (src->m_type == TensorDataType::float16 && prod(shape) != 0 && src->m_hip_resident) {
                if (N != 1) throw std::invalid_argument("Model::run: float16 graph inputs need one sample per pass (" + iname + ").");
                if (src->m_hip_resident_bytes != (size_t)prod(shape) * 2) throw std::invalid_argument("Model::get_tensor_data: mismatch between tensor shape and data size.");
                inp.staging = inp.val = new_val(iname, shape, OSG_F16, Lay::plain, true);
                vals[inp.val].dptr = src->m_hip_resident.get();
                vals[inp.val].pinned = true;
                inp.resident = src->m_hip_resident;
                inputs.push_back(std::move(inp));
                continue;
            }
            if (src->m_type == TensorDataType::float16 && prod(shape) != 0) {
                if (N != 1) throw std::invalid_argument("Model::run: float16 graph inputs need one sample per pass (" + iname + ").");
                inp.staging = inp.val = new_val(iname, shape, OSG_F16, Lay::plain, true);
                vals[inp.val].dptr = small_alloc(val_bytes(inp.val));
                vals[inp.val].pinned = true;
                inputs.push_back(std::move(inp));
                continue;
            }
            if (prod(shape) == 0) {
                inp.staging = inp.val = new_val(iname, shape, u8 ? OSG_U8 : OSG_F16, Lay::plain, true);
                vals[inp.val].pinned = true;
                inputs.push_back(std::move(inp));
                continue;
            }
            if (u8) {
                inp.staging = inp.val = new_val(iname, shape, OSG_U8, Lay::plain, true);
                vals[inp.val].dptr = small_alloc(val_bytes(inp.val));
// ... 187 lines not shown
```

### onnxstream_amd/csrc/host/plan.h

```cpp
#pragma once

#include <cmath>
#include <cstdint>
#include <functional>
#include <map>
#include <unordered_map>
#include <set>
#include <string>
#include <vector>

#include "backend.h"
#include "onnxstream.h"

namespace onnxstream {

enum class Lay { plain, nhwc };

struct Val {
    std::string name;
    std::vector<long> shape;
    osg_dtype dtype = OSG_F16;
    Lay lay = Lay::plain;
    bool batched = false;
    bool is_const = false;
// ... 34 lines not shown
    struct Base {
        void* dptr = nullptr;
        size_t bytes = 0;
        std::vector<float> host_f;
        std::vector<int64_t> host_i;
        bool host_valid = false;
    };
    std::map<std::string, Base> base;
    std::map<std::string, std::pair<void*, size_t>> derived;
    std::vector<TensorDataType> occ_types;
    bool complete = false;
    size_t bytes = 0;
    std::string fused_key;
    std::vector<Operation> fused_ops;
    size_t fused_const_vals = 0;
    bool fused_valid = false;
    std::vector<Val> snap_vals;
    size_t snap_weight_bytes = 0;
    std::vector<std::string> in_names;
    std::vector<std::pair<void*, size_t>> spare;
    void* take(size_t bytes, size_t* got) {
        int best = -1;
        for (size_t i = 0; i < spare.size(); i++)
            if (spare[i].second >= bytes && (best < 0 || spare[i].second < spare[best].second)) best = (int)i;
        if (best < 0 || spare[best].second > 4 * bytes + ((size_t)8 << 20)) return nullptr;
        void* p = spare[best].first;
        *got = spare[best].second;
        spare.erase(spare.begin() + best);
        return p;
    }
    std::map<size_t, std::vector<void*>> spare_class;
    static size_t size_class(size_t bytes) {
        size_t c = 4096;
        while (c < bytes) c <<= 1;
        return c;
    }
    void* take_class(HipBackend& be, size_t cls) {
        auto it = spare_class.find(cls);
        if (it != spare_class.end() && !it->second.empty()) {
            void* p = it->second.back();
            it->second.pop_back();
            return p;
        }
        return be.malloc(cls);
    }
    void give_class(HipBackend& be, void* p, size_t cls) {
        auto& v = spare_class[cls];
        if (v.size() >= 512) be.free(p);
        else v.push_back(p);
    }
    void give(HipBackend& be, void* p, size_t bytes) {
        if (spare.size() >= 8) {
            size_t k = 0;
            for (size_t i = 1; i < spare.size(); i++)
                if (spare[i].second < spare[k].second) k = i;
            be.free(spare[k].first);
            spare.erase(spare.begin() + k);
        }
        spare.push_back({p, bytes});
    }
    void clear(HipBackend& be) {
        for (auto& kv : base) be.free(kv.second.dptr);
        for (auto& kv : derived) be.free(kv.second.first);
        for (auto& sp : spare) be.free(sp.first);
        spare.clear();
        for (auto& kv : spare_class)
            for (void* p : kv.second) be.free(p);
        spare_class.clear();
        base.clear(); derived.clear(); occ_types.clear();
        complete = false; bytes = 0;
        fused_valid = false; fused_ops.clear(); fused_key.clear(); snap_vals.clear(); snap_weight_bytes = 0; in_names.clear();
    }
};

inline float half_to_float(uint16_t h) {
    uint32_t sign = (h >> 15) & 1, exp = (h >> 10) & 0x1f, man = h & 0x3ff;
    float v;
    if (exp == 0) v = std::ldexp((float)man, -24);
    else if (exp == 31) v = man ? NAN : INFINITY;
    else v = std::ldexp((float)(man | 0x400), (int)exp - 25);
    return sign ? -v : v;
}

struct Plan {
    Plan(Model& m, HipBackend& be, ConstPool& pool, size_t batch);
    ~Plan();
    void build();
    void execute(const std::function<void()>& while_device_runs = nullptr);
    void replay(int n, float* ms_each);
    void set_input(const std::string& name, long index, const float* data, size_t count);
    double sampler_loop(const std::string& sample_name, const std::string& timestep_name, const std::string& out_name, int n_steps, int prompts,
                        float* x, const float* noise, const float* c_in, const float* c_out, const float* t, const float* sigma, const float* d_sigma,
                        const float* sigma_up, float guidance, const float* clip, int branches = 2);
    double sampler_loop_multistep(const std::string& sample_name, const std::string& timestep_name, const std::string& out_name, int n_steps, int prompts,
                                  int sampler, float* x, const float* c_in, const float* c_out, const float* t, const float* sigma, const int* order,
                                  const float* coef, size_t n_coef, const double* dcoef, size_t n_dcoef, float guidance, int branches = 2);
    static double run_sampler_loop_multistep(Model& m, const std::string& sample_name, const std::string& timestep_name, const std::string& out_name,
                                             int n_steps, int prompts, int sampler, float* x, const float* c_in, const float* c_out, const float* t,
                                             const float* sigma, const int* order, const float* coef, size_t n_coef, const double* dcoef, size_t n_dcoef,
                                             float guidance, int branches = 2);
    static double run_sampler_loop(Model& m, const std::string& sample_name, const std::string& timestep_name, const std::string& out_name, int n_steps,
                                   int prompts, float* x, const float* noise, const float* c_in, const float* c_out, const float* t, const float* sigma,
                                   const float* d_sigma, const float* sigma_up, const float* clip, int branches);
    double decode_tiles(const std::string& in_name, const std::string& out_name, int images, int H, int W, float factor, const float* latents, float* image,
                        size_t image_elems, uint8_t* pixels, size_t pixels_elems);
    static double run_decode(Model& m, const std::string& in_name, const std::string& out_name, int images, int H, int W, float factor, const float* latents,
                             float* image, size_t image_elems, uint8_t* pixels, size_t pixels_elems);
    std::string profile(int reps);
    std::string info() const;
    bool compatible(Model& m, size_t batch) const;
    size_t kernel_count() const { return steps.size(); }
    double last_ms() const { return m_last_ms; }

    Model& m;
    HipBackend& be;
    ConstPool& pool;
    long N;

    std::vector<Operation> ops;
    std::vector<Val> vals;
    std::unordered_map<std::string, int> by_name;
    std::vector<Step> steps;
    std::vector<char> io_block;
    size_t gathered_up = 0, gathered_down = 0;
    std::vector<std::pair<char*, size_t>> slabs;
    bool in_one_slab(const char* lo, const char* hi) const;
    std::vector<void*> owned;
    std::vector<std::pair<void*, size_t>> recyclable;
    bool recycle = false, arena_pooled = false;
    void* pooled_malloc(size_t bytes);
    void* small_alloc(size_t bytes);
    char* slab = nullptr;
    size_t slab_left = 0;
    void* arena = nullptr;
    size_t arena_bytes = 0, weight_bytes = 0;

    struct WRecipe {
        int val = -1;
        std::string fn;
        TensorDataType ty = TensorDataType::none;
        osg_dtype have = OSG_F16, want = OSG_F16;
        long count = 0;
        float scale = 1.f;
        int zp = 0;
        void* raw = nullptr;
        bool resident = false;
        bool ring = false;
    };
    size_t vram_budget = 0, resident_bytes = 0, ring_weight_bytes = 0;
    bool budgeted = false;
    void* ring = nullptr;
    size_t ring_bytes = 0, ring_head = 0;
    struct RingOcc { size_t off, size; int last; int marker; };
    std::vector<RingOcc> ring_occ;
    int next_marker = 0, cur_step = 0;
    std::vector<WRecipe> recipes;
    std::vector<size_t> flush_upto;
    std::map<const void*, size_t> registered;
    size_t streamed_bytes = 0;
    void restream(const WRecipe& r);

    struct In {
        std::string name; int val; int staging; TensorDataType host_type; std::vector<size_t> shape; std::vector<int64_t> ivals;
        std::shared_ptr<void> resident;
    };
    struct Out {
        std::string name; int val; int f32val; std::vector<size_t> shape; bool raw16 = false;
        void* dev = nullptr;
        size_t dev_bytes = 0;
    };
    bool resident_outputs = false;
    struct Calib { int step; std::string op; int val; };
    std::vector<Calib> calib;
    std::vector<In> inputs;
    std::vector<Out> outputs;

    void* samp_x = nullptr;
    void* samp_noise = nullptr;
    void* samp_hist = nullptr;
    size_t samp_x_bytes = 0, samp_noise_bytes = 0, samp_hist_bytes = 0;
    struct SamplerIO { const In* in_s = nullptr; const In* in_t = nullptr; const Out* out = nullptr; long L = 0, TL = 0; };
    void sampler_check_state(const std::string& fn, int prompts, int branches) const;
    SamplerIO sampler_io(const std::string& fn, const std::string& sample_name, const std::string& timestep_name, const std::string& out_name) const;
    void sampler_grow(void*& p, size_t& have, size_t need);
    void* dec_lat = nullptr;
    void* dec_img = nullptr;
    void* dec_pix = nullptr;
    size_t dec_lat_bytes = 0, dec_img_bytes = 0, dec_pix_bytes = 0;

    osg_graph* graph = nullptr;
    Lowering* lowering = nullptr;
    int runs = 0;
    bool in_capture = false;
    double m_last_ms = 0;
    bool fp16 = true;
    bool u8_qdq = false, autotune = false, calibrate = false, fuse_attn = false, sdp_attn = false;
    std::set<std::string> outputs_convert_set;
    bool u8 = false;
    bool stream_weights = false;
    bool fuse_ln_gemm = false;
    bool concat_views = true;
    bool fuse_tblock = true;
    bool in_flight = false;
    bool gn_stats_on = false;
    int gn_stats_req = 2;
    long gn_stats_min_elems = 0;
    char* gn_stats = nullptr;
    size_t gn_stats_bytes = 0;
    void zero_gn_stats();
    void run_steps(size_t begin = 0, size_t end = (size_t)-1);
    size_t dyn_end = 0;
    bool w8_resident = false;
    int fusion = 2;
    int fusion_req = 2;
    std::vector<std::string> extra_outputs;

    int new_val(const std::string& name, const std::vector<long>& shape, osg_dtype dt, Lay lay, bool batched);
    int alias(int v, const std::vector<long>& shape, Lay lay, const std::string& name = "");
    int root_of(int v) const;
    void* ptr(int v) const;
    size_t val_bytes(int v) const;
    long total_elems(int v) const;
    void add_step(const std::string& what, std::vector<int> reads, std::vector<int> writes, std::function<void()> fn);
    const Val& qv(int v) const;
    void share_q(int dst, int src);
    void own_q(int v, float scale, int zp);
    int ensure_plain(int v);
    int ensure_nhwc(int v);
    void* const_alloc(const std::string& tag, size_t bytes, bool* fresh);
    int ensure_dense(int v);
};

}
```

### onnxstream_amd/csrc/osg_conv3x3_kernel.h

```cpp
#pragma once
#include "osg_gemm_common.h"
#include <algorithm>
#include <array>
#include <cmath>
#include <cstdlib>
#include <type_traits>

using namespace osg_mm;

namespace {

template <int I> using ic = std::integral_constant<int, I>;
template <int B, int E, class F>
__device__ __forceinline__ void static_for(F&& f) {
    if constexpr (B < E) {
        f(ic<B>{});
        static_for<B + 1, E>(f);
    }
}

template <int N> __device__ __forceinline__ void wait_vmcnt() { asm volatile("s_waitcnt vmcnt(%0)" ::"n"(N) : "memory"); }

template <int W_, int BN, int NLW = 4, int WQ = 0>
struct Geo {
    static constexpr int TI = W_ == 8 ? 2 : 1;
    static constexpr int TH = 128 / (W_ * TI);
    static constexpr int PW = W_ == 8 ? 16 : W_ + 2;
    static constexpr int PH = TH + 2;
    static constexpr int PPI = PH * PW;
    static constexpr int PP = TI * PPI;
    static constexpr int NPW = ((PP + 7) / 8 + NLW - 1) / NLW;
    static constexpr int PATCH_BYTES = NPW * NLW * 1024;
    static constexpr int BRW = WQ ? 16 : 8;
    static constexpr int WLB = ((BN + BRW - 1) / BRW + NLW - 1) / NLW;
    static constexpr int BST_BYTES = WLB * NLW * 1024;
    static constexpr int NSTW_ = (160 * 1024 - 2 * PATCH_BYTES) / BST_BYTES;
    static constexpr int NSTW = NSTW_ > 8 ? 8 : NSTW_;
    static constexpr int D = NSTW - 1;
    static constexpr int PT = 10 - D;
    static constexpr int PPT = (NPW + PT - 1) / PT;
    static constexpr size_t SMEM = 2 * (size_t)PATCH_BYTES + (size_t)NSTW * BST_BYTES;
    static constexpr bool OK = D >= 3 && PT >= 2;
    static constexpr int patch_loads(int t) {
        if (t >= PT) return 0;
        int n = NPW - t * PPT;
        return n < 0 ? 0 : (n > PPT ? PPT : n);
    }
    static constexpr int allowed_outstanding(int t) {
        int n = 0;
        for (int d = 1; d <= D - 2; d++) n += WLB + patch_loads((t - d + 18) % 9);
        return n;
    }
};

template <int W_, int BN, int WGM, int WGN, int MODE, int NLW, int WQ = 0>
__device__ __forceinline__ void conv3x3_body(const GemmParams& p) {
    using G = Geo<W_, BN, NLW, WQ>;
    constexpr int TI = G::TI, TH = G::TH, PW = G::PW, PPI = G::PPI, PP = G::PP, NPW = G::NPW, PATCH_BYTES = G::PATCH_BYTES;
    constexpr int WLB = G::WLB, BST_BYTES = G::BST_BYTES, NSTW = G::NSTW, D = G::D, PPT = G::PPT;
    constexpr int WM = 128 / WGM, WN = BN / WGN, TM = WM / 16, TN = WN / 16;
    static_assert(WM % 16 == 0 && WN % 16 == 0 && WGM * WGN == 4, "bad wave layout");
    constexpr unsigned OOB = 0x80000000u;

    extern __shared__ __attribute__((aligned(16))) char smem3[];
    typedef __attribute__((address_space(3))) void* lds_ptr;
    char* const patch0 = smem3;
    char* const bst0 = smem3 + 2 * PATCH_BYTES;

    kdbg_stamp(p, 0);
    const int tid = threadIdx.x;
    const int lane = tid & 63;
    const int wave8 = __builtin_amdgcn_readfirstlane(tid >> 6);
    const bool loader = wave8 >= 4;
    const int wave = loader ? wave8 - 4 : wave8;

    int L;
    {
        const int total = p.grid, bid = blockIdx.x, x = bid & 7, i = bid >> 3, q = total >> 3, r = total & 7;
        L = (x < r ? x * (q + 1) : r * (q + 1) + (x - r) * q) + i;
    }
    int m_tile, n_tile, zs;
    if (p.n_major) {
        n_tile = L / (p.splits * p.mt); L -= n_tile * p.splits * p.mt;
        zs = L / (p.mt); m_tile = L - zs * p.mt;
    } else {
        m_tile = L / (p.splits * p.nt); L -= m_tile * p.splits * p.nt;
        zs = L / (p.nt); n_tile = L - zs * p.nt;
    }
    const int m0 = m_tile * 128, n0 = n_tile * BN;
    const int slab_b = zs * (p.k_per_split >> 6);
    const int slab_e = min(p.Cin >> 6, slab_b + (p.k_per_split >> 6));

    if (loader) {
        const int img0 = m0 / (p.H * W_);
        const int y0 = (m0 - img0 * p.H * W_) / W_;
        __amdgpu_buffer_rsrc_t rsA = __builtin_amdgcn_make_buffer_rsrc((void*)p.A, 0, p.a_bytes, 0x00020000);
        __amdgpu_buffer_rsrc_t rsB = __builtin_amdgcn_make_buffer_rsrc((void*)p.Bt, 0, p.b_bytes, 0x00020000);
        const int rsub = lane >> 3;
        const int gch = (lane & 7) ^ rsub;
        unsigned pa_off[NPW];
#pragma unroll
        for (int pc = 0; pc < NPW; pc++) {
            const int pp = (pc * NLW + wave) * 8 + rsub;
            const int ti = pp / PPI, rr = pp - ti * PPI;
            const int py = rr / PW, px = rr - py * PW;
            const int img = img0 + ti, y = y0 + py - 1, x = px - 1;
            const bool ok = pp < PP && (unsigned)y < (unsigned)p.H && (unsigned)x < (unsigned)W_ && img * p.H * W_ < p.M;
            pa_off[pc] = ok ? (unsigned)((((img * p.H + y) * W_ + x) * p.Cin + gch * 8) * 2) : OOB;
        }
        unsigned b_off[WLB];
#pragma unroll
        for (int j = 0; j < WLB; j++) {
            if constexpr (WQ) {
                const int nl = (j * NLW + wave) * 16 + (lane >> 2);
                const int n = n0 + nl;
                b_off[j] = (nl < BN && n < p.N) ? (unsigned)((long)n * p.K + (((lane & 3) ^ ((lane >> 4) & 3)) << 4)) : OOB;
            } else {
                const int nl = (j * NLW + wave) * 8 + rsub;
                const int n = n0 + nl;
                b_off[j] = (nl < BN && n < p.N) ? (unsigned)(((long)n * p.K + gch * 8) * 2) : OOB;
            }
        }
        auto issue_patch_piece = [&](int pc, int slab, char* buf) {
            if (MODE >= 3 && MODE != 6) return;
            const unsigned kill = (slab < slab_e && MODE != 2) ? 0u : OOB;
            __builtin_amdgcn_raw_ptr_buffer_load_lds(rsA, (lds_ptr)(buf + (pc * NLW + wave) * 1024), 16, pa_off[pc] | kill, slab * 128, 0, 0);
        };
        auto issue_weights = [&](int stage, int tap, int slab) {
            if (MODE >= 3 && MODE != 6) return;
            const unsigned kill = (slab < slab_e && MODE != 2) ? 0u : OOB;
            const int soff = (tap * p.Cin + slab * 64) * (WQ ? 1 : 2);
            char* dst = bst0 + stage * BST_BYTES;
#pragma unroll
            for (int j = 0; j < WLB; j++)
                __builtin_amdgcn_raw_ptr_buffer_load_lds(rsB, (lds_ptr)(dst + (j * NLW + wave) * 1024), 16, b_off[j] | kill, soff, 0, 0);
        };
        issue_weights(0, 0, slab_b);
#pragma unroll
        for (int pc = 0; pc < NPW; pc++) issue_patch_piece(pc, slab_b, patch0);
#pragma unroll
        for (int d = 1; d < D; d++) issue_weights(d, d % 9, slab_b + d / 9);
        wait_vmcnt<(D - 1) * WLB>();
        __builtin_amdgcn_s_barrier();
        int ust = 0;
        for (int slab = slab_b; slab < slab_e; slab++) {
            char* patch_next = patch0 + (((slab - slab_b) & 1) ^ 1) * PATCH_BYTES;
            static_for<0, 9>([&](auto tc) {
                constexpr int t = decltype(tc)::value;
                wait_vmcnt<G::allowed_outstanding(t)>();
                if (MODE != 5) __builtin_amdgcn_s_barrier();
                constexpr int td = (t + D) % 9;
                int std_ = ust + D;
                std_ = std_ >= NSTW ? std_ - NSTW : std_;
                issue_weights(std_, td, slab + (t + D) / 9);
                static_for<0, G::patch_loads(t)>([&](auto pc) { issue_patch_piece(t * PPT + decltype(pc)::value, slab + 1, patch_next); });
                ust = ust + 1 == NSTW ? 0 : ust + 1;
            });
        }
        asm volatile("s_waitcnt vmcnt(0)" ::: "memory");
        return;
    }

    OSG_PIN(p.bias); OSG_PIN(p.residual); OSG_PIN(p.rowbias); OSG_PIN(p.rb_ld); OSG_PIN(p.rb_rows); OSG_PIN(p.bias_f32); OSG_PIN(p.act); OSG_PIN(p.no_epre);
    if constexpr (WQ) { OSG_PIN(p.wq_sc); OSG_PIN(p.wq_zp); OSG_PIN(p.w_zp); }
    const int wm0 = (wave / WGN) * WM;
    const int wn0 = (wave % WGN) * WN;
    f32x4 acc[TM][TN];
#pragma unroll
    for (int i = 0; i < TM; i++)
#pragma unroll
        for (int j = 0; j < TN; j++) acc[i][j] = f32x4{0.f, 0.f, 0.f, 0.f};

    const int frow = lane & 15, fq = lane >> 4;
    int pp0[TM];
#pragma unroll
    for (int i = 0; i < TM; i++) {
        const int ml = wm0 + i * 16 + frow;
        const int ti = ml / (TH * W_), rr = ml - ti * (TH * W_);
        const int ty = rr / W_, tx = rr - ty * W_;
        pp0[i] = ti * PPI + ty * PW + tx;
    }
    const int b_rd = WQ ? (wn0 + frow) * 64 + ((((lane >> 5) & 1) ^ ((frow >> 2) & 3)) << 4) + ((lane >> 4) & 1) * 8 : (wn0 + frow) * 128 + ((fq ^ (frow & 7)) << 4);
    constexpr bool W8SC = false;
    W8Ops<WQ ? TN : 1, W8SC> w8;
    if constexpr (WQ) w8_prefetch<TN, W8SC>(p, w8, n0, wn0, lane);

    f16x8 fa0[TM], fb0[TN], fa1[TM], fb1[TN];
    auto read_frags = [&](f16x8 (&fa)[TM], f16x8 (&fb)[TN], const char* pbuf, const char* bbuf, int tap_off, int ks) {
        if (MODE == 1 || (MODE == 4 && ks == 1)) return;
#pragma unroll
        for (int i = 0; i < TM; i++) {
            const int pp = pp0[i] + tap_off;
            fa[i] = *reinterpret_cast<const f16x8*>(pbuf + ((pp * 128 + ((fq ^ (pp & 7)) << 4)) ^ (ks << 6)));
        }
#pragma unroll
        for (int j = 0; j < TN; j++) {
            if constexpr (WQ) fb[j] = w8_frag(*reinterpret_cast<const u32x2v*>(bbuf + ((b_rd + j * 16 * 64) ^ (ks << 5))), w8.zz[j]);
            else fb[j] = *reinterpret_cast<const f16x8*>(bbuf + ((b_rd + j * 16 * 128) ^ (ks << 6)));
        }
    };
    auto mma = [&](f16x8 (&fa)[TM], f16x8 (&fb)[TN]) {
        if (MODE == 1) return;
#pragma unroll
        for (int i = 0; i < TM; i++)
#pragma unroll
            for (int j = 0; j < TN; j++) acc[i][j] = __builtin_amdgcn_mfma_f32_16x16x32_f16(fb[j], fa[i], acc[i][j], 0, 0, 0);
    };

    u32x2v rb0[WQ ? TN : 1], rb1[WQ ? TN : 1];
    auto read_a = [&](f16x8 (&fa)[TM], const char* pbuf, int tap_off, int ks) {
#pragma unroll
        for (int i = 0; i < TM; i++) {
            const int pp = pp0[i] + tap_off;
            fa[i] = *reinterpret_cast<const f16x8*>(pbuf + ((pp * 128 + ((fq ^ (pp & 7)) << 4)) ^ (ks << 6)));
        }
    };
    auto read_codes = [&](u32x2v (&rb)[WQ ? TN : 1], const char* bbuf, int ks) {
        if constexpr (WQ) {
#pragma unroll
            for (int j = 0; j < TN; j++) rb[j] = *reinterpret_cast<const u32x2v*>(bbuf + ((b_rd + j * 16 * 64) ^ (ks << 5)));
        }
    };
    auto convert = [&](f16x8 (&fb)[TN], const u32x2v (&rb)[WQ ? TN : 1]) {
        if constexpr (WQ) {
#pragma unroll
            for (int j = 0; j < TN; j++) fb[j] = w8_frag(rb[j], w8.zz[j]);
        }
    };

    constexpr bool EPRE = TM * TN <= 10 && NLW == 4;
    EpiOps<TM, TN, true, EPRE> epre;
    epi_prefetch<TM, TN, true, EPRE>(p, epre, m0, n0, wm0, wn0, lane, 0);
    kdbg_stamp(p, 1);
    __builtin_amdgcn_s_barrier();
    kdbg_stamp(p, 2);
    if constexpr (WQ) {
        w8_finalize<TN, W8SC>(w8);
        read_a(fa0, patch0, 0, 0);
        read_codes(rb0, bst0, 0);
        read_codes(rb1, bst0, 1);
        convert(fb0, rb0);
    } else
    read_frags(fa0, fb0, patch0, bst0, 0, 0);
    if (MODE == 4) {
#pragma unroll
        for (int i = 0; i < TM; i++) fa1[i] = fa0[i];
#pragma unroll
        for (int j = 0; j < TN; j++) fb1[j] = fb0[j];
    }
    int ust = 0;
    for (int slab = slab_b; slab < slab_e; slab++) {
        const char* patch = patch0 + ((slab - slab_b) & 1) * PATCH_BYTES;
        const char* patch_next = patch0 + (((slab - slab_b) & 1) ^ 1) * PATCH_BYTES;
        static_for<0, 9>([&](auto tc) {
            constexpr int t = decltype(tc)::value;
            if (MODE != 5) __builtin_amdgcn_s_barrier();
            constexpr int kh = t / 3, kw = t % 3;
            const char* Bs = bst0 + ust * BST_BYTES;
            if constexpr (WQ) {
                constexpr int KV = (8 * TN + TM * TN - 1) / (TM * TN);
                const int ustn = ust + 1 == NSTW ? 0 : ust + 1;
                const char* Bn = bst0 + ustn * BST_BYTES;
                read_a(fa1, patch, kh * PW + kw, 1);
                read_codes(rb0, Bn, 0);
                convert(fb1, rb1);
                mma(fa0, fb0);
                static_for<0, TM * TN>([&](auto ic_) {
                    __builtin_amdgcn_sched_group_barrier(0x008, 1, 0);
                    if constexpr (decltype(ic_)::value < TM + TN) __builtin_amdgcn_sched_group_barrier(0x100, 1, 0);
                    __builtin_amdgcn_sched_group_barrier(0x002, KV, 0);
                });
                __builtin_amdgcn_sched_barrier(0);
                ust = ustn;
                constexpr int tn8 = (t + 1) % 9;
                read_a(fa0, t == 8 ? patch_next : patch, (tn8 / 3) * PW + tn8 % 3, 0);
                read_codes(rb1, Bn, 1);
                convert(fb0, rb0);
                mma(fa1, fb1);
                static_for<0, TM * TN>([&](auto ic_) {
                    __builtin_amdgcn_sched_group_barrier(0x008, 1, 0);
                    if constexpr (decltype(ic_)::value < TM + TN) __builtin_amdgcn_sched_group_barrier(0x100, 1, 0);
                    __builtin_amdgcn_sched_group_barrier(0x002, KV, 0);
                });
                __builtin_amdgcn_sched_barrier(0);
            } else if constexpr (MODE == 0 || MODE == 7) {
                read_frags(fa1, fb1, patch, Bs, kh * PW + kw, 1);
                mma(fa0, fb0);
                if constexpr (MODE == 0) {
                    static_for<0, TM + TN>([&](auto) { __builtin_amdgcn_sched_group_barrier(0x008, 1, 0); __builtin_amdgcn_sched_group_barrier(0x100, 1, 0); });
                    __builtin_amdgcn_sched_group_barrier(0x008, TM * TN - (TM + TN), 0);
                } else {
                    static_for<0, TM + TN>([&](auto) { __builtin_amdgcn_sched_group_barrier(0x100, 1, 0); __builtin_amdgcn_sched_group_barrier(0x008, 1, 0); });
                    __builtin_amdgcn_sched_group_barrier(0x008, TM * TN - (TM + TN), 0);
                }
                __builtin_amdgcn_sched_barrier(0);
                ust = ust + 1 == NSTW ? 0 : ust + 1;
                constexpr int tn6 = (t + 1) % 9;
                read_frags(fa0, fb0, t == 8 ? patch_next : patch, bst0 + ust * BST_BYTES, (tn6 / 3) * PW + tn6 % 3, 0);
                mma(fa1, fb1);
                if constexpr (MODE == 0) {
                    static_for<0, TM + TN>([&](auto) { __builtin_amdgcn_sched_group_barrier(0x008, 1, 0); __builtin_amdgcn_sched_group_barrier(0x100, 1, 0); });
                    __builtin_amdgcn_sched_group_barrier(0x008, TM * TN - (TM + TN), 0);
                } else {
                    static_for<0, TM + TN>([&](auto) { __builtin_amdgcn_sched_group_barrier(0x100, 1, 0); __builtin_amdgcn_sched_group_barrier(0x008, 1, 0); });
                    __builtin_amdgcn_sched_group_barrier(0x008, TM * TN - (TM + TN), 0);
                }
                __builtin_amdgcn_sched_barrier(0);
            } else {
            read_frags(fa1, fb1, patch, Bs, kh * PW + kw, 1);
            __builtin_amdgcn_sched_barrier(0);
            mma(fa0, fb0);
            __builtin_amdgcn_sched_barrier(0);
            ust = ust + 1 == NSTW ? 0 : ust + 1;
            constexpr int tn = (t + 1) % 9;
            if (MODE != 4) read_frags(fa0, fb0, t == 8 ? patch_next : patch, bst0 + ust * BST_BYTES, (tn / 3) * PW + tn % 3, 0);
            __builtin_amdgcn_sched_barrier(0);
            mma(fa1, fb1);
            __builtin_amdgcn_sched_barrier(0);
            }
        });
    }
    kdbg_stamp(p, 3);
    if constexpr (WQ) { if constexpr (W8SC) w8_scale_acc<TM, TN>(w8, acc); else w8_scale_acc_late<TM, TN>(p, acc, n0, wn0, lane); }
    kdbg_stamp(p, 4);
    float* stat_lds = nullptr;
    if (OSG_UNLIKELY(p.sink[0].table || p.sink[1].table)) {
        __builtin_amdgcn_s_barrier();
        stat_lds = reinterpret_cast<float*>(smem3) + (wave8 & 3) * (WN * 2);
    }
    if constexpr (MODE == 0) {
        if (OSG_UNLIKELY(p.splits > 1 && p.fold_acc)) {
            if (!splitk_fold_acc<TM, TN>(p, acc, m_tile * p.nt + n_tile, zs, reinterpret_cast<int*>(smem3), tid)) return;
            EpiOps<TM, TN, true, false> none;
            none.have = false;
            gemm_epilogue_fast<TM, TN, true, false, false>(p, acc, m0, n0, wm0, wn0, lane, 0, none, nullptr);
            return;
        }
    }
    gemm_epilogue<TM, TN, true, EPRE, false>(p, acc, m0, n0, wm0, wn0, lane, 0, zs, epre, stat_lds);
    kdbg_stamp(p, 5);
    if (OSG_UNLIKELY(p.kdbg != nullptr)) { asm volatile("s_waitcnt vmcnt(0)" ::: "memory"); kdbg_stamp(p, 6); }
}

template <int W_, int BN, int WGM, int WGN, int MODE, int NLW, int WQ = 0>
__global__ __launch_bounds__(256 + 64 * NLW) void conv3x3_kernel(const void* A, const void* Bt, int M, int N, int K, int k_per_split, unsigned a_bytes, unsigned b_bytes, int grid,
                                                                 int H, int Cin, unsigned sp_nm, GemmParams pk) {
    GemmParams p = pk;
    p.A = (const f16*)A; p.Bt = (const f16*)Bt; p.M = M; p.N = N; p.K = K; p.k_per_split = k_per_split; p.a_bytes = a_bytes; p.b_bytes = b_bytes; p.grid = grid; p.H = H; p.Cin = Cin;
    p.splits = (int)(sp_nm & ((1u << kPackSplitsBits) - 1)); p.n_major = (sp_nm & kPackNMajor) != 0;
    p.mt = (M + 127) / 128; p.nt = (N + BN - 1) / BN;
    p.kdbg = nullptr;
    if (OSG_UNLIKELY(sp_nm & kPackKdbg)) p.kdbg = kernarg_rare(pk.kdbg);
    conv3x3_body<W_, BN, WGM, WGN, MODE, NLW, WQ>(p);
}

template <int W_, int BN, int WGM, int WGN, int MODE = 0, int NLW = 4, int WQ = 0>
int launch3(osg_ctx* ctx, GemmParams& p) {
    constexpr size_t smem = Geo<W_, BN, NLW, WQ>::SMEM;
    static_assert(smem <= 160 * 1024, "LDS budget");
    static_assert(Geo<W_, BN, NLW, WQ>::OK, "pipeline depth out of range");
    auto kern = conv3x3_kernel<W_, BN, WGM, WGN, MODE, NLW, WQ>;
    static unsigned long long attr_mask = 0;
    if (osg_first_on_device(attr_mask)) {
        OSG_HIP(ctx, hipFuncSetAttribute((const void*)kern, hipFuncAttributeMaxDynamicSharedMemorySize, (int)smem));
    }
    p.mt = (p.M + 127) / 128;
    p.nt = (p.N + BN - 1) / BN;
    p.no_epre = osg_mm::no_epi_prefetch();
    p.kdbg = kdbg_buffer(ctx, (long)p.mt * p.nt * p.splits);
    const osg_mm::StatSink sinks_in[2] = {p.sink[0], p.sink[1]};
    if (p.sink[0].table || p.sink[1].table) {
        const bool ok = !ctx->tuning && p.splits == 1 && MODE == 0 && (p.N & 3) == 0 && ((p.ldc | p.ldc2) & 3) == 0 && p.sink_hw > 0 && p.sink_hw % 128 == 0 && p.M % p.sink_hw == 0;
        if (ok) { ctx->sink_fused = true; p.sink_imgs = p.M / p.sink_hw; p.sink_per_xcd = ctx->xcd_ids8 ? 1 : 0; }
        else p.sink[0].table = p.sink[1].table = nullptr;
    }
    p.grid = p.mt * p.nt * p.splits;
    int lda32;
    unsigned sp_nm;
    const int bad = kernarg_pack(ctx, 0, p.splits, p.n_major, p.kdbg != nullptr, false, &lda32, &sp_nm);
    if (!bad) hipLaunchKernelGGL(kern, dim3((unsigned)p.grid), dim3(256 + 64 * NLW), smem, ctx->compute, (const void*)p.A, (const void*)p.Bt, p.M, p.N, p.K, p.k_per_split, p.a_bytes, p.b_bytes, p.grid, p.H, p.Cin, sp_nm, p);
    p.sink[0] = sinks_in[0]; p.sink[1] = sinks_in[1];
    if (bad) return 1;
    OSG_LAUNCH_CHECK(ctx);
    return 0;
}

using V3Launch = int (*)(osg_ctx*, GemmParams&);
template <int UNIT, int I>
constexpr V3Launch v3_launcher() {
    constexpr V3Entry e = kV3Entries[I];
    if constexpr (v3_unit(e) == UNIT) return launch3<e.w, e.bn, e.wgm, e.wgn, 0, e.nlw, e.wq>;
    else return nullptr;
}
template <int UNIT, size_t... I>
constexpr std::array<V3Launch, kV3Count> v3_launchers(std::index_sequence<I...>) { return {v3_launcher<UNIT, (int)I>()...}; }
template <int UNIT>
int launch3_in_unit(int entry, osg_ctx* ctx, GemmParams& p) {
    static constexpr std::array<V3Launch, kV3Count> table = v3_launchers<UNIT>(std::make_index_sequence<kV3Count>{});
    return table[entry](ctx, p);
}

}
```

### onnxstream_amd/csrc/osg_gemm_common.h

```cpp
#pragma once
#include <utility>
#include <vector>
#include "osg_common.h"
#include "osg_gemm_select.h"
#include "osg_gemm_epi.h"

#include <algorithm>
#include <type_traits>
#ifndef OSG_EPI_STORE_AUX
#define OSG_EPI_STORE_AUX 0
#endif
namespace osg_mm {

struct StatSink {
    long long* table;
    int groups, cpg, ch_off;
};
constexpr int kStatCopies = 8;
constexpr float kStatSX = 1048576.f;
__host__ __device__ inline int stat_q_shift(long elems) {
    int lg = 0;
    while ((1L << lg) < elems) lg++;
    const int e = 36 - lg;
    return e < 10 ? 10 : (e > 20 ? 20 : e);
}
__host__ __device__ inline float stat_q_scale(long elems) { return (float)(1L << stat_q_shift(elems)); }

struct GemmParams {
    const f16* A;
    const f16* Bt;
    long long* kdbg;
    long lda;
    long strideA, strideB;
    int M, N, K;
    int splits, k_per_split;
    unsigned a_bytes, b_bytes;
    int mt, nt, n_major;
    int grid;
    int H, W, Cin, Ho, Wo, KW, sh, sw, pt, pl;
    const void* bias;
    const f16* residual;
    const f16* rowbias;
    long rb_ld;
    long strideC;
    const float* ln_c1;
    const float* rs_in;
    int rb_rows;
    int bias_f32, act;
    int no_epre;
    int rs_np;
    unsigned rb_bytes;
    f16* C;
    float* partial;
    long a_bytes_l;
    int* tickets;
    int* xcd_err;
    float w_scale;
    int w_zp;
    const float* wq_sc;
    const float* wq_zp;
    int w8;
    float ln_eps;
    float* rs_out;
    long ldc;
    f16* C2;
    long ldc2;
    StatSink sink[2];
    int sink_hw;
    int sink_imgs, sink_per_xcd;
    int fold_acc;
};
constexpr int kPackSplitsBits = 16;
constexpr unsigned kPackNMajor = 1u << 16, kPackKdbg = 1u << 17, kPackBatch = 1u << 18;
template <class T>
__device__ __forceinline__ T kernarg_rare(T v) {
    asm volatile("" : "+s"(v));
    return v;
}
inline int kernarg_pack(osg_ctx* ctx, long lda, int splits, int n_major, bool kdbg, bool batched, int* lda32, unsigned* sp_nm) {
    if (lda < 0 || lda > 0x7fffffffL) {
        ctx->err = "contraction launch: the row pitch of A does not fit the 32-bit kernel parameter";
        return 1;
    }
    if (splits < 1 || splits >= (1 << kPackSplitsBits)) {
        ctx->err = "contraction launch: the number of k-slices does not fit its 16-bit kernel parameter field";
        return 1;
    }
    *lda32 = (int)lda;
// ... 97 lines not shown
        if (PARTIAL) {
            s += __shfl_xor(s, 16, 64); q += __shfl_xor(q, 16, 64);
            s += __shfl_xor(s, 32, 64); q += __shfl_xor(q, 32, 64);
        }
        const double ik = (double)(1.0f / (float)p.K);
        const double mean_d = (double)s * ik;
        const float var = fmaxf((float)((double)q * ik - mean_d * mean_d), 0.f);
        const float mean = (float)mean_d;
        const float rstd = 1.0f / sqrtf(var + p.ln_eps);
#pragma unroll
        for (int j = 0; j < TN; j++) {
            const int n = n0 + wn0 + j * 16 + (lane >> 4) * 4;
            f32x4 c = {0.f, 0.f, 0.f, 0.f};
            if (n < p.N) c = *reinterpret_cast<const f32x4*>(p.ln_c1 + n);
#pragma unroll
            for (int r = 0; r < 4; r++) acc[i][j][r] = rstd * (acc[i][j][r] - mean * c[r]);
        }
    }
}

template <int TM, int TN, bool RB = true, bool ON = true>
struct EpiOps {
    bool have;
    f32x4 bias32[ON ? TN : 1];
    f16x4 bias16[ON ? TN : 1];
    f16x4 rb[ON && RB ? TM : 1][ON && RB ? TN : 1];
    f16x4 res[ON ? TM : 1][ON ? TN : 1];
};
template <int TM, int TN, bool RB, bool ON, int EPI = EPI_ANY>
__device__ __forceinline__ void epi_prefetch(const GemmParams& p, EpiOps<TM, TN, RB, ON>& e, int m0, int n0, int wm0, int wn0, int lane, int zb) {
    const int N = p.N;
    e.have = ON && EPI_ALWAYS(!p.no_epre && p.splits == 1 && (N & 3) == 0 && p.act != OSG_ACT_GEGLU && N >= 4 && (RB || !p.rowbias));
    if constexpr (!ON) return;
    if (__builtin_expect(!e.have, 0)) return;
    const f16* __restrict__ R = EPI_ON(EPI_RESIDUAL, p.residual != nullptr) ? p.residual + zb * p.strideC : nullptr;
#pragma unroll
    for (int j = 0; j < TN; j++) {
        const int n = EPI_CLAMP(n0 + wn0 + j * 16 + (lane >> 4) * 4, N - 4);
        if (EPI_ON(EPI_BIAS16 | EPI_BIAS32, p.bias != nullptr)) {
            if (EPI_ON(EPI_BIAS32, p.bias_f32 != 0)) e.bias32[j] = *reinterpret_cast<const f32x4*>((const float*)p.bias + n);
            else e.bias16[j] = *reinterpret_cast<const f16x4*>((const f16*)p.bias + n);
        }
    }
#pragma unroll
    for (int i = 0; i < TM; i++) {
        const int m = EPI_CLAMP(m0 + wm0 + i * 16 + (lane & 15), p.M - 1);
#pragma unroll
        for (int j = 0; j < TN; j++) {
            const int n = EPI_CLAMP(n0 + wn0 + j * 16 + (lane >> 4) * 4, N - 4);
            if constexpr (RB) {
                if (EPI_ON(EPI_ROWBIAS, p.rowbias != nullptr)) e.rb[i][j] = *reinterpret_cast<const f16x4*>(p.rowbias + (long)(m / p.rb_rows) * p.rb_ld + n);
            }
            if (EPI_ON(EPI_RESIDUAL, R != nullptr)) e.res[i][j] = *reinterpret_cast<const f16x4*>(R + (long)m * N + n);
        }
    }
    asm volatile("" ::: "memory");
}

__device__ __forceinline__ void stat_add(int per_xcd, unsigned long long* table, long copy_stride, long cell, float S, float Q, float qscale) {
    const unsigned long long vs = (unsigned long long)__float2ll_rn(S * kStatSX), vq = (unsigned long long)__float2ll_rn(Q * qscale);
    if (per_xcd) {
        unsigned xcc;
        asm volatile("s_getreg_b32 %0, hwreg(HW_REG_XCC_ID)" : "=s"(xcc));
        unsigned long long* c = table + (long)(xcc & 7u) * copy_stride + cell;
        __hip_atomic_fetch_add(c, vs, __ATOMIC_RELAXED, __HIP_MEMORY_SCOPE_WORKGROUP);
        __hip_atomic_fetch_add(c + 1, vq, __ATOMIC_RELAXED, __HIP_MEMORY_SCOPE_WORKGROUP);
    } else {
        atomicAdd(table + cell, vs);
        atomicAdd(table + cell + 1, vq);
    }
}

template <int CTRL>
__device__ __forceinline__ float dpp_get(float v) {
    return __int_as_float(__builtin_amdgcn_update_dpp(0, __float_as_int(v), CTRL, 0xf, 0xf, false));
}
__device__ __forceinline__ float dpp_sum16(float v) {
    v += dpp_get<0xB1>(v);
    v += dpp_get<0x4E>(v);
    v += dpp_get<0x124>(v);
    v += dpp_get<0x128>(v);
    return v;
}
template <int TM, int TN>
__device__ __forceinline__ void gemm_colstats(const GemmParams& p, const f16x4 (&o)[TM][TN], int mrow0, int ncol0, int lane, float* st) {
    const int mb = mrow0 + (lane & 15);
#pragma unroll
    for (int j = 0; j < TN; j++)
#pragma unroll
        for (int r = 0; r < 4; r++) {
            float s = 0.f, q = 0.f;
#pragma unroll
            for (int i = 0; i < TM; i++)
                if (mb + i * 16 < p.M) {
                    const float f = (float)o[i][j][r];
                    s += f;
                    q = fmaf(f, f, q);
                }
            s = dpp_sum16(s);
            q = dpp_sum16(q);
            if ((lane & 15) == 0) {
                const int c = j * 16 + (lane >> 4) * 4 + r;
                st[c * 2] = s;
                st[c * 2 + 1] = q;
            }
        }
    asm volatile("s_waitcnt lgkmcnt(0)" ::: "memory");
    const int n_img = mrow0 / p.sink_hw;
    const int wn = min(TN * 16, p.N - ncol0);
#pragma unroll
    for (int k = 0; k < 2; k++) {
        const StatSink sk = p.sink[k];
        if (!sk.table || wn <= 0) continue;
        const int c_lo = ncol0 + sk.ch_off, c_hi = c_lo + wn;
        const int g = c_lo / sk.cpg + lane;
        if (g * sk.cpg < c_hi) {
            const int a = max(g * sk.cpg, c_lo) - c_lo, b = min((g + 1) * sk.cpg, c_hi) - c_lo;
            float S = 0.f, Q = 0.f;
            for (int c = a; c < b; c++) { S += st[c * 2]; Q += st[c * 2 + 1]; }
            stat_add(p.sink_per_xcd, reinterpret_cast<unsigned long long*>(sk.table), (long)p.sink_imgs * sk.groups * 2, ((long)n_img * sk.groups + g) * 2, S, Q,
                     stat_q_scale((long)p.sink_hw * sk.cpg));
        }
    }
}

constexpr unsigned kEpiOob = 0x80000000u;
constexpr int kEpiMaxBM = 128;
__host__ __device__ inline unsigned epi_extent(int rows_left, long pitch, int N) {
    const long bytes = ((long)(rows_left - 1) * pitch + N) * 2;
    return bytes < (long)kEpiOob ? (unsigned)bytes : kEpiOob;
}
inline int epi_check(osg_ctx* ctx, GemmParams& p) {
    const long ldc = p.ldc ? p.ldc : (long)p.N;
    const long pitch = std::max(std::max(ldc, p.C2 ? p.ldc2 : 0L), (long)p.N);
    if ((long)kEpiMaxBM * pitch * 2 >= (long)kEpiOob) {
        ctx->err = "contraction epilogue: an output row pitch of 8 Mi elements or more does not fit the 32-bit store offsets of a 128-row tile";
        return 1;
    }
    p.rb_bytes = 0;
    if (p.rowbias) {
        const long rb_rows = p.rb_rows > 0 ? p.rb_rows : 1;
        const long bytes = (((long)p.M - 1) / rb_rows * p.rb_ld + p.N) * 2;
        if (bytes >= (long)kEpiOob) {
            ctx->err = "contraction epilogue: the per-image bias must be smaller than 2 GiB";
            return 1;
        }
        p.rb_bytes = (unsigned)bytes;
    }
    return 0;
}

template <int TM, int TN, bool RB, bool ON, bool BATCH = true, int EPI = EPI_ANY>
__device__ __forceinline__ void gemm_epilogue_fast(const GemmParams& p, f32x4 (&acc)[TM][TN], int m0, int n0, int wm0, int wn0, int lane, int zb,
                                                   const EpiOps<TM, TN, RB, ON>& pre, float* stat_lds = nullptr) {
    const int N = p.N;
    f16* __restrict__ C = p.C + zb * p.strideC;
    const f16* __restrict__ R = EPI_ON(EPI_RESIDUAL, p.residual != nullptr) ? p.residual + zb * p.strideC : nullptr;
    const long ldc = p.ldc ? p.ldc : (long)N;
    const int nb = n0 + wn0 + (lane >> 4) * 4;
    const int mb = m0 + wm0 + (lane & 15);
    bool done = false;
    if constexpr (ON) {
        if (EPI_ALWAYS(pre.have)) {
            done = true;
            if (EPI_ON(EPI_BIAS16 | EPI_BIAS32, p.bias != nullptr)) {
                if (EPI_ON(EPI_BIAS32, p.bias_f32 != 0)) {
#pragma unroll
                    for (int i = 0; i < TM; i++)
#pragma unroll
                        for (int j = 0; j < TN; j++) acc[i][j] += pre.bias32[j];
                } else {
#pragma unroll
                    for (int i = 0; i < TM; i++)
#pragma unroll
                        for (int j = 0; j < TN; j++)
#pragma unroll
                            for (int r = 0; r < 4; r++) acc[i][j][r] += (float)pre.bias16[j][r];
                }
            }
            if constexpr (RB) {
                if (EPI_ON(EPI_ROWBIAS, p.rowbias != nullptr)) {
#pragma unroll
                    for (int i = 0; i < TM; i++)
#pragma unroll
                        for (int j = 0; j < TN; j++)
#pragma unroll
                            for (int r = 0; r < 4; r++) acc[i][j][r] += (float)pre.rb[i][j][r];
                }
            }
            if (EPI_ON(EPI_RESIDUAL, R != nullptr)) {
#pragma unroll
                for (int i = 0; i < TM; i++)
#pragma unroll
                    for (int j = 0; j < TN; j++)
#pragma unroll
                        for (int r = 0; r < 4; r++) acc[i][j][r] += (float)pre.res[i][j][r];
            }
        }
    }
    if constexpr (BATCH) if (!done) {
        const bool hb32 = EPI_ON(EPI_BIAS32, p.bias && p.bias_f32), hb16 = EPI_ON(EPI_BIAS16, p.bias && !p.bias_f32), hrb = EPI_ON(EPI_ROWBIAS, p.rowbias != nullptr),
                   hres = EPI_ON(EPI_RESIDUAL, R != nullptr);
        typedef unsigned u32x2 __attribute__((ext_vector_type(2)));
        typedef unsigned u32x4 __attribute__((ext_vector_type(4)));
        const unsigned nbytes = (unsigned)N * 2u;
        __amdgpu_buffer_rsrc_t rsB32 = __builtin_amdgcn_make_buffer_rsrc((void*)p.bias, 0, hb32 ? nbytes * 2u : 0u, 0x00020000);
        __amdgpu_buffer_rsrc_t rsB16 = __builtin_amdgcn_make_buffer_rsrc((void*)p.bias, 0, hb16 ? nbytes : 0u, 0x00020000);
        __amdgpu_buffer_rsrc_t rsRB = __builtin_amdgcn_make_buffer_rsrc((void*)p.rowbias, 0, hrb ? p.rb_bytes : 0u, 0x00020000);
        __amdgpu_buffer_rsrc_t rsR = __builtin_amdgcn_make_buffer_rsrc((void*)(hres ? R + (long)m0 * N : nullptr), 0, hres ? epi_extent(p.M - m0, N, N) : 0u, 0x00020000);
        if (TM * TN <= 16 && OSG_LIKELY(!hrb && !hres)) {
            if (hb32) {
                f32x4 b32[TN];
#pragma unroll
                for (int j = 0; j < TN; j++) b32[j] = __builtin_bit_cast(f32x4, __builtin_amdgcn_raw_buffer_load_b128(rsB32, (unsigned)nb * 4u + j * 64, 0, 0));
#pragma unroll
                for (int i = 0; i < TM; i++)
#pragma unroll
                    for (int j = 0; j < TN; j++)
#pragma unroll
                        for (int r = 0; r < 4; r++) acc[i][j][r] += b32[j][r];
            } else if (hb16) {
                f16x4 b16[TN];
#pragma unroll
                for (int j = 0; j < TN; j++) b16[j] = __builtin_bit_cast(f16x4, __builtin_amdgcn_raw_buffer_load_b64(rsB16, (unsigned)nb * 2u + j * 32, 0, 0));
#pragma unroll
                for (int i = 0; i < TM; i++)
#pragma unroll
                    for (int j = 0; j < TN; j++)
#pragma unroll
                        for (int r = 0; r < 4; r++) acc[i][j][r] += (float)b16[j][r];
            }
        } else {
        f32x4 b32[TN];
        f16x4 b16[TN];
#pragma unroll
        for (int j = 0; j < TN; j++) {
            b32[j] = __builtin_bit_cast(f32x4, __builtin_amdgcn_raw_buffer_load_b128(rsB32, (unsigned)nb * 4u + j * 64, 0, 0));
// ... 13 lines not shown
                    const unsigned rs = (unsigned)(wm0 + (lane & 15) + (i0 + ii) * 16) * nbytes + (unsigned)nb * 2u;
#pragma unroll
                    for (int jj = 0; jj < JB; jj++) {
                        rbv[ii][jj] = __builtin_bit_cast(f16x4, __builtin_amdgcn_raw_buffer_load_b64(rsRB, ro + (j0 + jj) * 32, 0, 0));
                        rsv[ii][jj] = __builtin_bit_cast(f16x4, __builtin_amdgcn_raw_buffer_load_b64(rsR, rs + (j0 + jj) * 32, 0, 0));
                    }
                }
#pragma unroll
                for (int ii = 0; ii < IB; ii++)
#pragma unroll
                    for (int jj = 0; jj < JB; jj++)
#pragma unroll
                        for (int r = 0; r < 4; r++) {
                            float x = acc[i0 + ii][j0 + jj][r];
                            x += EPI_ON(EPI_BIAS16 | EPI_BIAS32, p.bias != nullptr) ? (hb32 ? b32[j0 + jj][r] : (float)b16[j0 + jj][r]) : -0.0f;
                            x += hrb ? (float)rbv[ii][jj][r] : -0.0f;
                            x += hres ? (float)rsv[ii][jj][r] : -0.0f;
                            acc[i0 + ii][j0 + jj][r] = x;
                        }
            }
        }
    }
    if constexpr (!BATCH) if (!done) {
        if (EPI_ON(EPI_BIAS16 | EPI_BIAS32, p.bias != nullptr)) {
#pragma unroll
            for (int j = 0; j < TN; j++) {
                const int n = min(nb + j * 16, N - 4);
                f32x4 bv;
                if (EPI_ON(EPI_BIAS32, p.bias_f32 != 0)) bv = *reinterpret_cast<const f32x4*>((const float*)p.bias + n);
                else {
                    const f16x4 b16 = *reinterpret_cast<const f16x4*>((const f16*)p.bias + n);
#pragma unroll
                    for (int r = 0; r < 4; r++) bv[r] = (float)b16[r];
                }
#pragma unroll
                for (int i = 0; i < TM; i++) acc[i][j] += bv;
            }
        }
        if (EPI_ON(EPI_ROWBIAS, p.rowbias != nullptr)) {
#pragma unroll
            for (int i = 0; i < TM; i++) {
                const long ro = (long)(min(mb + i * 16, p.M - 1) / p.rb_rows) * p.rb_ld;
#pragma unroll
                for (int j = 0; j < TN; j++) {
                    const f16x4 rb = *reinterpret_cast<const f16x4*>(p.rowbias + ro + min(nb + j * 16, N - 4));
#pragma unroll
                    for (int r = 0; r < 4; r++) acc[i][j][r] += (float)rb[r];
                }
            }
        }
        if (EPI_ON(EPI_RESIDUAL, R != nullptr)) {
#pragma unroll
            for (int i = 0; i < TM; i++) {
                const long ro = (long)min(mb + i * 16, p.M - 1) * N;
#pragma unroll
                for (int j = 0; j < TN; j++) {
                    const f16x4 rv = *reinterpret_cast<const f16x4*>(R + ro + min(nb + j * 16, N - 4));
#pragma unroll
                    for (int r = 0; r < 4; r++) acc[i][j][r] += (float)rv[r];
                }
            }
        }
    }
    if (OSG_UNLIKELY_IF(BATCH, (EPI_ON(EPI_SILU, p.act != OSG_ACT_NONE)))) {
        const int act = EPI_ACT(p.act);
#pragma unroll
        for (int i = 0; i < TM; i++)
#pragma unroll
            for (int j = 0; j < TN; j++)
#pragma unroll
                for (int r = 0; r < 4; r++) acc[i][j][r] = osg_apply_act(acc[i][j][r], act);
    }
    f16x4 o[TM][TN];
#pragma unroll
    for (int i = 0; i < TM; i++)
#pragma unroll
        for (int j = 0; j < TN; j++)
#pragma unroll
            for (int r = 0; r < 4; r++) o[i][j][r] = (f16)acc[i][j][r];
#if OSG_EPI_STORE_AUX >= 0
    {
        typedef unsigned u32x2 __attribute__((ext_vector_type(2)));
        const int mr = wm0 + (lane & 15), rows_left = p.M - m0;
        __amdgpu_buffer_rsrc_t rsC = __builtin_amdgcn_make_buffer_rsrc((void*)(C + (long)m0 * ldc), 0, epi_extent(rows_left, ldc, N), 0x00020000);
#pragma unroll
        for (int i = 0; i < TM; i++) {
            const int r = mr + i * 16;
#pragma unroll
            for (int j = 0; j < TN; j++) {
                const int n = nb + j * 16;
                const unsigned off = EPI_ALWAYS(r < rows_left && n < N) ? ((unsigned)r * (unsigned)ldc + (unsigned)n) * 2u : kEpiOob;
                __builtin_amdgcn_raw_buffer_store_b64(__builtin_bit_cast(u32x2, o[i][j]), rsC, off, 0, OSG_EPI_STORE_AUX);
            }
        }
        if (OSG_UNLIKELY_IF(BATCH, (EPI_ON(EPI_C2, p.C2 != nullptr)))) {
            __amdgpu_buffer_rsrc_t rsC2 = __builtin_amdgcn_make_buffer_rsrc((void*)(p.C2 + (long)m0 * p.ldc2), 0, epi_extent(rows_left, p.ldc2, N), 0x00020000);
#pragma unroll
            for (int i = 0; i < TM; i++) {
                const int r = mr + i * 16;
#pragma unroll
                for (int j = 0; j < TN; j++) {
                    const int n = nb + j * 16;
                    const unsigned off = EPI_ALWAYS(r < rows_left && n < N) ? ((unsigned)r * (unsigned)p.ldc2 + (unsigned)n) * 2u : kEpiOob;
                    __builtin_amdgcn_raw_buffer_store_b64(__builtin_bit_cast(u32x2, o[i][j]), rsC2, off, 0, OSG_EPI_STORE_AUX);
                }
            }
        }
    }
#else
#pragma unroll
    for (int i = 0; i < TM; i++) {
        const int m = mb + i * 16;
#pragma unroll
        for (int j = 0; j < TN; j++) {
            const int n = nb + j * 16;
            if (m < p.M && n < N) *reinterpret_cast<f16x4*>(C + (long)m * ldc + n) = o[i][j];
        }
    }
    if (p.C2) {
        f16* __restrict__ C2 = p.C2;
#pragma unroll
        for (int i = 0; i < TM; i++) {
            const int m = mb + i * 16;
#pragma unroll
            for (int j = 0; j < TN; j++) {
                const int n = nb + j * 16;
                if (m < p.M && n < N) *reinterpret_cast<f16x4*>(C2 + (long)m * p.ldc2 + n) = o[i][j];
            }
        }
    }
#endif
    if (OSG_UNLIKELY_IF(BATCH, (EPI_ON(EPI_SINKS, stat_lds != nullptr)))) gemm_colstats<TM, TN>(p, o, m0 + wm0, n0 + wn0, lane, stat_lds);
    if (OSG_UNLIKELY_IF(BATCH, (EPI_ON(EPI_ROWSTATS, p.rs_out != nullptr)))) {
#pragma unroll
        for (int i = 0; i < TM; i++) {
            const int m = mb + i * 16;
            if (!EPI_ALWAYS(m < p.M)) continue;
#pragma unroll
            for (int h = 0; h < TN / 2; h++) {
                float s = 0.f, q = 0.f;
#pragma unroll
                for (int jj = 0; jj < 2; jj++) {
                    const int j = 2 * h + jj;
                    if (EPI_ALWAYS(nb + j * 16 < N)) {
#pragma unroll
                        for (int r = 0; r < 4; r++) {
                            const float f = (float)o[i][j][r];
                            s += f;
                            q = fmaf(f, f, q);
                        }
                    }
                }
                s += __shfl_xor(s, 16, 64); q += __shfl_xor(q, 16, 64);
                s += __shfl_xor(s, 32, 64); q += __shfl_xor(q, 32, 64);
                const int slot = ((n0 + wn0) >> 5) + h;
                if ((lane >> 4) == 0 && EPI_ALWAYS(slot < p.rs_np)) {
                    float* d = p.rs_out + ((long)m * p.rs_np + slot) * 2;
                    d[0] = s;
                    d[1] = q;
                }
            }
        }
    }
}

template <int TM, int TN, bool RB, bool ON, bool BATCH = true, int EPI = EPI_ANY>
__device__ __forceinline__ void gemm_epilogue(const GemmParams& p, f32x4 (&acc)[TM][TN], int m0, int n0, int wm0, int wn0, int lane,
                                              int zb, int zslab, const EpiOps<TM, TN, RB, ON>& pre, float* stat_lds = nullptr) {
    const int N = p.N;
    if (OSG_LIKELY(EPI_OFF(EPI_SPLIT, p.splits == 1))) {
        if (OSG_LIKELY(EPI_ALWAYS((N & 3) == 0 && ((p.ldc | p.ldc2) & 3) == 0))) {
            gemm_epilogue_fast<TM, TN, RB, ON, BATCH, EPI>(p, acc, m0, n0, wm0, wn0, lane, zb, pre, stat_lds);
            return;
        }
        f16* __restrict__ C = p.C + zb * p.strideC;
        const f16* __restrict__ R = p.residual ? p.residual + zb * p.strideC : nullptr;
        const long ldc = p.ldc ? p.ldc : (long)N;
        f16* __restrict__ C2 = p.C2;
#pragma unroll
        for (int i = 0; i < TM; i++) {
            const int m = m0 + wm0 + i * 16 + (lane & 15);
            if (m >= p.M) continue;
#pragma unroll
            for (int j = 0; j < TN; j++) {
                const int n = n0 + wn0 + j * 16 + (lane >> 4) * 4;
                if (n >= N) continue;
#pragma unroll
                for (int r = 0; r < 4; r++) {
                    if (n + r >= N) break;
                    float x = acc[i][j][r];
                    if (p.bias) x += p.bias_f32 ? ((const float*)p.bias)[n + r] : (float)((const f16*)p.bias)[n + r];
                    if (p.rowbias) x += (float)p.rowbias[(long)(m / p.rb_rows) * p.rb_ld + n + r];
                    if (R) x += (float)R[(long)m * N + n + r];
                    const f16 o1 = (f16)osg_apply_act(x, p.act);
                    C[(long)m * ldc + n + r] = o1;
                    if (C2) C2[(long)m * p.ldc2 + n + r] = o1;
                }
            }
        }
    } else {
        float* __restrict__ P = p.partial + ((long)zslab) * p.M * N;
#pragma unroll
        for (int i = 0; i < TM; i++) {
            const int m = m0 + wm0 + i * 16 + (lane & 15);
            if (!EPI_ALWAYS(m < p.M)) continue;
#pragma unroll
            for (int j = 0; j < TN; j++) {
                const int n = n0 + wn0 + j * 16 + (lane >> 4) * 4;
                if (!EPI_ALWAYS(n < N)) continue;
                if (EPI_ALWAYS((N & 3) == 0)) {
                    *reinterpret_cast<f32x4*>(P + (long)m * N + n) = acc[i][j];
                } else {
#pragma unroll
                    for (int r = 0; r < 4; r++)
                        if (n + r < N) P[(long)m * N + n + r] = acc[i][j][r];
// ... 205 lines not shown
```

### onnxstream_amd/osgpu.py

```python
from __future__ import annotations

import ctypes
import os
from typing import Optional, Sequence

import numpy as np

_HERE = os.path.dirname(os.path.abspath(__file__))
LIB_PATH = os.environ.get("OSGPU_LIB") or os.path.join(_HERE, "libosgpu.so")

U8, F16, F32, I64 = 1, 2, 3, 4
_NP2DT = {np.dtype(np.uint8): U8, np.dtype(np.float16): F16, np.dtype(np.float32): F32, np.dtype(np.int64): I64}
ACT_NONE, ACT_SILU, ACT_SIGMOID = 0, 1, 2
UN = dict(sigmoid=0, erf=1, sqrt=2, sin=3, cos=4, neg=5, pow=6, silu=7, gelu_erf=8)
BIN = dict(add=0, sub=1, mul=2, div=3)

EXPORTS = [
    "osg_device_count", "osg_init", "osg_destroy", "osg_last_error", "osg_device_name", "osg_stream", "osg_set_autotune", "osg_tune_misses",
    "osg_malloc", "osg_free", "osg_upload", "osg_upload_sync", "osg_host_register", "osg_host_unregister", "osg_upload_pinned", "osg_upload_pinned_async", "osg_copy_fence", "osg_download", "osg_copy", "osg_memset", "osg_sync",
    "osg_graph_begin", "osg_graph_end", "osg_graph_launch", "osg_graph_destroy", "osg_timer_start", "osg_timer_stop",
    "osg_conv2d_nhwc", "osg_conv2d_nhwc_rb", "osg_conv2d_nhwc_v", "osg_gemm", "osg_gemm_ln", "osg_gemm_rowstats", "osg_last_route", "osg_last_epilogue", "osg_last_kernel", "osg_gemm_kernarg_check", "osg_attention_kernarg_check", "osg_gemm_w8", "osg_conv2d_nhwc_w8", "osg_gemm_w8_v", "osg_conv2d_nhwc_w8_v", "osg_transpose_kn_to_nk", "osg_attention", "osg_attention_strided", "osg_sdpa", "osg_rms_norm", "osg_rope",
    "osg_instance_norm", "osg_group_norm_nhwc", "osg_layer_norm", "osg_reduce_mean_last", "osg_softmax_last",
    "osg_unary", "osg_binary", "osg_geglu", "osg_transpose", "osg_copy_2d", "osg_concat2", "osg_resize_nearest", "osg_gather_rows",
    "osg_maxpool_nhwc", "osg_convert", "osg_sampler_prepare", "osg_sampler_cfg_euler_a", "osg_sampler_cfg_multistep", "osg_sampler_prepare_rescale",
    "osg_sampler_prepare_single", "osg_sampler_euler_a_single", "osg_sampler_multistep_single",
    "osg_decode_gather", "osg_decode_blend",
    "osg_range_push", "osg_range_pop", "osg_marker_record", "osg_copy_wait_marker", "osg_timer_mark", "osg_timer_between", "osg_set_stat_sinks", "osg_group_norm_stats_nhwc", "osg_qu8_conv2d_nhwc", "osg_qu8_conv2d_nhwc_t", "osg_qu8_conv_tap_sums", "osg_qu8_gemm", "osg_qu8_lut", "osg_qu8_binary", "osg_qu8_instance_norm", "osg_qu8_instance_norm_nhwc", "osg_qu8_affine_act", "osg_qu8_norm_affine_act_nhwc", "osg_qu8_softmax_last", "osg_kdbg_read",
    "osg_tblock_tail_supported", "osg_tblock_tail", "osg_tblock_kv_pack_elems", "osg_tblock_kv_pack_jobs", "osg_tblock_pack_weight", 
]


class OsgError(RuntimeError):
    pass


class TBlockTailArgs(ctypes.Structure):
    _vp, _cf, _ci, _cl = ctypes.c_void_p, ctypes.c_float, ctypes.c_int, ctypes.c_long
    _fields_ = [("a1", _vp), ("x0", _vp), ("wo1", _vp), ("bo1", _vp), ("g2", _vp), ("be2", _vp), ("eps2", _cf), ("wq2", _vp), ("bq2", _vp),
                ("kp", _vp), ("vtp", _vp), ("scale", _cf), ("Tk", _ci), ("wo2", _vp), ("bo2", _vp), ("g3", _vp), ("be3", _vp), ("eps3", _cf),
                ("w1", _vp), ("b1", _vp), ("w2", _vp), ("b2", _vp), ("wpo", _vp), ("bpo", _vp), ("xin", _vp), ("out", _vp), ("out2", _vp),
                ("ldo", _cl), ("ldo2", _cl), ("M", _ci), ("rows_per_img", _ci), ("C", _ci), ("heads", _ci), ("dbg", _vp * 8), ("rows_per_block", _ci)]


def load_library(path: str = LIB_PATH) -> ctypes.CDLL:
    if not os.path.exists(path):
        raise OsgError(f"{path} not found: build it with `python -m onnxstream_amd.build` (hipcc, gfx950)")
    lib = ctypes.CDLL(path)
    vp, ci, cl, cf = ctypes.c_void_p, ctypes.c_int, ctypes.c_long, ctypes.c_float
    lib.osg_init.argtypes = [ci, ctypes.POINTER(vp)]
    lib.osg_destroy.argtypes = [vp]
    lib.osg_destroy.restype = None
    lib.osg_last_error.argtypes = [vp]
    lib.osg_last_error.restype = ctypes.c_char_p
    lib.osg_device_name.argtypes = [vp]
    lib.osg_device_name.restype = ctypes.c_char_p
    lib.osg_stream.argtypes = [vp]
    lib.osg_stream.restype = vp
    lib.osg_malloc.argtypes = [vp, ctypes.c_size_t, ctypes.POINTER(vp)]
    lib.osg_free.argtypes = [vp, vp]
    lib.osg_host_register.argtypes = [vp, vp, ctypes.c_size_t]
    lib.osg_host_unregister.argtypes = [vp, vp]
    for f in ("osg_upload", "osg_upload_sync", "osg_upload_pinned", "osg_upload_pinned_async", "osg_download", "osg_copy"):
        getattr(lib, f).argtypes = [vp, vp, vp, ctypes.c_size_t]
    lib.osg_memset.argtypes = [vp, vp, ci, ctypes.c_size_t]
    lib.osg_sync.argtypes = [vp]
    lib.osg_copy_fence.argtypes = [vp]
    lib.osg_graph_begin.argtypes = [vp]
    lib.osg_graph_end.argtypes = [vp, ctypes.POINTER(vp)]
    lib.osg_graph_launch.argtypes = [vp, vp]
    lib.osg_graph_destroy.argtypes = [vp]
    lib.osg_graph_destroy.restype = None
    lib.osg_timer_start.argtypes = [vp]
    lib.osg_timer_stop.argtypes = [vp, ctypes.POINTER(cf)]
    lib.osg_conv2d_nhwc.argtypes = [vp, ci, vp, vp, vp, ci, vp, vp] + [ci] * 14
    lib.osg_conv2d_nhwc_rb.argtypes = [vp, ci, vp, vp, vp, ci, vp, cl, vp, vp] + [ci] * 14
    lib.osg_conv2d_nhwc_v.argtypes = [vp, ci, vp, vp, vp, ci, vp, cl, vp, vp, cl, vp, cl] + [ci] * 14
    lib.osg_gemm_w8.argtypes = [vp, vp, vp, cf, ci, vp, ci, vp, vp, ci, ci, ci, ci]
    lib.osg_conv2d_nhwc_w8.argtypes = [vp, vp, vp, cf, ci, vp, ci, vp, cl, vp, vp] + [ci] * 14
    lib.osg_gemm_w8_v.argtypes = [vp, vp, vp, cf, ci, vp, vp, vp, ci, vp, vp, ci, ci, ci, ci]
    lib.osg_conv2d_nhwc_w8_v.argtypes = [vp, vp, vp, cf, ci, vp, vp, vp, ci, vp, cl, vp, vp, cl, vp, cl] + [ci] * 14
    lib.osg_gemm.argtypes = [vp, ci, vp, vp, ci, vp, ci, vp, vp, ci, ci, ci, ci, cl, cl, cl, ci]
    lib.osg_transpose_kn_to_nk.argtypes = [vp, ci, vp, vp, ci, ci]
    lib.osg_attention.argtypes = [vp, ci, vp, vp, vp, vp, ci, ci, ci, ci, cf, ci]
    lib.osg_attention_strided.argtypes = [vp, ci, vp, cl, cl, cl, vp, cl, cl, cl, vp, cl, cl, cl, vp, cl, cl, cl, ci, ci, ci, ci,
                                          ci, cf]
    lib.osg_sdpa.argtypes = [vp, ci, vp, vp, vp, vp, vp, ci, ci, ci, ci, ci, ci, cf]
    lib.osg_rms_norm.argtypes = [vp, ci, vp, vp, vp, cl, ci, cf]
    lib.osg_rope.argtypes = [vp, ci, vp, vp, vp, vp, cl, cl, ci]
    lib.osg_instance_norm.argtypes = [vp, ci, vp, vp, vp, vp, ci, cl, ci, cf]
    lib.osg_group_norm_nhwc.argtypes = [vp, ci, vp, vp, vp, vp, ci, cl, ci, ci, cf, ci]
    lib.osg_layer_norm.argtypes = [vp, ci, vp, vp, vp, vp, cl, ci, cf]
    lib.osg_reduce_mean_last.argtypes = [vp, ci, vp, vp, cl, cl]
    lib.osg_softmax_last.argtypes = [vp, ci, vp, vp, cl, cl]
    lib.osg_unary.argtypes = [vp, ci, ci, vp, vp, cl, cf]
    lib.osg_binary.argtypes = [vp, ci, ci, vp, ctypes.POINTER(cl), vp, ctypes.POINTER(cl), vp, ci]
    lib.osg_geglu.argtypes = [vp, ci, vp, vp, cl, cl]
    lib.osg_transpose.argtypes = [vp, ci, vp, vp, ci, ctypes.POINTER(cl), ctypes.POINTER(ci)]
    lib.osg_copy_2d.argtypes = [vp, ci, vp, cl, cl, vp, cl, cl, cl, cl]
    lib.osg_resize_nearest.argtypes = [vp, ci, vp, vp] + [ci] * 7
    lib.osg_gather_rows.argtypes = [vp, ci, vp, vp, vp, cl, cl, cl]
    lib.osg_maxpool_nhwc.argtypes = [vp, ci, vp, vp] + [ci] * 12
    lib.osg_convert.argtypes = [vp, ci, ci, vp, vp, cl, cf, ci]
    lib.osg_concat2.argtypes = [vp, ci, vp, cl, vp, cl, vp, cl]
    lib.osg_gemm_ln.argtypes = [vp, vp, vp, vp, vp, cf, vp, vp, vp, ci, ci, ci, ci]
    lib.osg_gemm_rowstats.argtypes = [vp, vp, vp, vp, ci, vp, vp, ci, ci, ci, ci, vp]
    lib.osg_last_route.argtypes = [vp, ctypes.POINTER(ci)]
    lib.osg_last_kernel.argtypes = [vp, ctypes.POINTER(ci)]
    if hasattr(lib, "osg_last_epilogue"):
        lib.osg_last_epilogue.argtypes = [vp, ctypes.POINTER(ci)]
    if hasattr(lib, "osg_gemm_kernarg_check"):
        lib.osg_gemm_kernarg_check.argtypes = [vp, cl, ci]
        lib.osg_attention_kernarg_check.argtypes = [vp, cl, ci, ci]
    lib.osg_sampler_prepare.argtypes = [vp, vp, vp, vp, ci, cl, cf, cf, cl]
    lib.osg_sampler_cfg_euler_a.argtypes = [vp, vp, vp, vp, ci, cl, cf, cf, cf, cf, cf, cf]
    lib.osg_sampler_cfg_multistep.argtypes = [vp, ci, vp, vp, vp, vp, vp, vp, ci, cl, cf, cf, cf, cf, cf, cf, cf, cf, ctypes.c_double, ctypes.c_double]
    lib.osg_sampler_prepare_rescale.argtypes = [vp, vp, vp, vp, ci, cl, cf, cf, cf, cl]
    lib.osg_sampler_prepare_single.argtypes = [vp, vp, vp, vp, ci, cl, cf, cf, cf, cl]
    lib.osg_sampler_euler_a_single.argtypes = [vp, vp, vp, vp, ci, cl, cf, cf, cf, cf, cf]
    lib.osg_sampler_multistep_single.argtypes = [vp, ci, vp, vp, vp, vp, vp, vp, ci, cl, cf, cf, cf, cf, cf, cf, cf, ctypes.c_double, ctypes.c_double]
    lib.osg_decode_gather.argtypes = [vp, vp, vp, ci, ci, ci, ci, cf]
    lib.osg_decode_blend.argtypes = [vp, vp, vp, vp, ci, ci, ci, ci, ci]
    lib.osg_set_stat_sinks.argtypes = [vp, vp, ci, ci, ci, vp, ci, ci, ci, ci]
    lib.osg_group_norm_stats_nhwc.argtypes = [vp, vp, vp, vp, vp, ci, ctypes.c_long, ci, ci, cf, ci, vp]
    lib.osg_qu8_conv2d_nhwc.argtypes = [vp, vp, cf, ci, vp, cf, ci, vp, cf, ci, vp] + [ci] * 13
    lib.osg_qu8_conv2d_nhwc_t.argtypes = [vp, vp, cf, ci, vp, cf, ci, vp, cf, ci, vp] + [ci] * 13 + [vp]
    lib.osg_qu8_conv_tap_sums.argtypes = [vp, vp, ci, ci, ci, ci, vp]
    lib.osg_qu8_gemm.argtypes = [vp, vp, cl, cf, ci, vp, cf, ci, vp, cf, ci, vp, ci, ci, ci, ci, cl, cl, cl]
    lib.osg_qu8_lut.argtypes = [vp, vp, vp, cl, vp]
    lib.osg_qu8_binary.argtypes = [vp, ci, vp, ctypes.POINTER(cl), cf, ci, vp, ctypes.POINTER(cl), cf, ci, vp, cf, ci, ci]
    lib.osg_qu8_instance_norm.argtypes = [vp, vp, vp, ci, cl, ci, vp, vp, cf, cf, ci, cf, ci]
    lib.osg_qu8_affine_act.argtypes = [vp, vp, cf, ci, vp, cf, ci, cf, ci, vp, cf, ci, cf, ci, vp, cf, ci, cf, ci, vp, cl, ci, cl]
    lib.osg_qu8_instance_norm_nhwc.argtypes = [vp, vp, vp, cl, ci, ci, ci, vp, vp, cf, cf, ci, cf, ci]
    lib.osg_qu8_norm_affine_act_nhwc.argtypes = [vp, vp, cl, ci, ci, ci, vp, vp, cf, cf, ci, cf, ci, vp, cf, ci, cf, ci, vp, cf, ci, cf, ci, vp, cf, ci, cf, ci, vp]
    lib.osg_qu8_softmax_last.argtypes = [vp, vp, vp, cl, cl, vp]
    lib.osg_tblock_tail_supported.argtypes = [ci] * 5
    lib.osg_tblock_tail.argtypes = [vp, ctypes.POINTER(TBlockTailArgs)]
    lib.osg_tblock_kv_pack_elems.argtypes = [ci, ci, ci]
    lib.osg_tblock_kv_pack_elems.restype = ctypes.c_size_t
    lib.osg_tblock_kv_pack_jobs.argtypes = [vp, vp, cl, ci, ci, ci, ci, vp, vp]
    lib.osg_tblock_pack_weight.argtypes = [vp, vp, ci, ci, vp]
    return lib


class DevBuf:

    def __init__(self, gpu: "Gpu", shape, dtype):
        self.gpu = gpu
        self.shape = tuple(int(s) for s in shape)
        self.dtype = np.dtype(dtype)
        self.nbytes = int(np.prod(self.shape, dtype=np.int64)) * self.dtype.itemsize
        p = ctypes.c_void_p()
        gpu._ck(gpu.lib.osg_malloc(gpu.ctx, max(self.nbytes, 16), ctypes.byref(p)))
        self.ptr = p.value

    @property
    def size(self):
        return int(np.prod(self.shape, dtype=np.int64))

    def numpy(self) -> np.ndarray:
# ... 538 lines not shown
```

Measured before the change: 10.53.

## Fuse nearest 2x upsample with 3x3 conv via per-phase 2x2 combined weights

Result: no change. 10.61, median of 6 (+0.8%).

```diff
diff --git a/include/osgpu.h b/include/osgpu.h
--- a/include/osgpu.h
+++ b/include/osgpu.h
@@ -89,6 +89,10 @@
                       const void* image_bias, long image_bias_ld, const void* residual, void* y, long y_ld, void* y2, long y2_ld, int N, int H, int W,
                       int Cin, int Cout, int KH, int KW, int stride_h, int stride_w, int pad_top, int pad_left, int pad_bottom, int pad_right,
                       osg_act act);
+
+int osg_upconv2x_supported(osg_dtype w_dtype, int N, int H, int W, int Cin, int Cout, long max_pitch);
+int osg_upconv2x_nhwc_v(osg_ctx* ctx, const void* x, const void* w_phases, const void* bias, osg_dtype bias_dtype, void* y, long y_ld, void* y2, long y2_ld,
+                        int N, int H, int W, int Cin, int Cout, osg_act act);
 
 int osg_gemm(osg_ctx* ctx, osg_dtype dtype, const void* A, const void* B, int b_is_nk, const void* bias, osg_dtype bias_dtype,
              const void* residual, void* C, int M, int N, int K, int batch, long stride_a, long stride_b, long stride_c,
diff --git a/onnxstream_amd/build.py b/onnxstream_amd/build.py
--- a/onnxstream_amd/build.py
+++ b/onnxstream_amd/build.py
@@ -62,7 +62,8 @@
     srcs = sorted(glob.glob(os.path.join(hdir, "*.cpp")))
     if not srcs:
         return None
-    hdrs = sorted(glob.glob(os.path.join(hdir, "*.h"))) + sorted(glob.glob(os.path.join(hdir, "*.inc"))) + [os.path.join(INC, "osgpu.h")]
+    hdrs = sorted(glob.glob(os.path.join(hdir, "*.h"))) + sorted(glob.glob(os.path.join(hdir, "*.inc"))) + [os.path.join(INC, "osgpu.h")] + \
+        [os.path.join(CSRC, h) for h in ("osg_upconv.h", "osg_gemm_select.h", "osg_gemm_routes.h")]
     if force or _newer(LIB_HOST, srcs + hdrs):
         _run(["g++", "-std=c++20", "-O2", "-fPIC", "-shared", "-I" + INC, "-I" + hdir, "-o", LIB_HOST] + srcs +
              ["-ldl", "-lpthread"])
diff --git a/onnxstream_amd/csrc/host/backend.h b/onnxstream_amd/csrc/host/backend.h
--- a/onnxstream_amd/csrc/host/backend.h
+++ b/onnxstream_amd/csrc/host/backend.h
@@ -21,7 +21,8 @@
     X(osg_copy_2d) X(osg_concat2) X(osg_resize_nearest) X(osg_gather_rows) X(osg_maxpool_nhwc) X(osg_convert) \
     X(osg_sampler_prepare) X(osg_sampler_cfg_euler_a) X(osg_sampler_cfg_multistep) X(osg_sampler_prepare_rescale) X(osg_sampler_prepare_single) X(osg_sampler_euler_a_single) X(osg_sampler_multistep_single) X(osg_decode_gather) X(osg_decode_blend) X(osg_qu8_conv2d_nhwc) X(osg_qu8_conv2d_nhwc_t) X(osg_qu8_conv_tap_sums) X(osg_qu8_gemm) X(osg_qu8_lut) X(osg_qu8_binary) \
     X(osg_qu8_instance_norm) X(osg_qu8_instance_norm_nhwc) X(osg_qu8_affine_act) X(osg_qu8_norm_affine_act_nhwc) X(osg_qu8_softmax_last) X(osg_range_push) X(osg_range_pop) X(osg_marker_record) \
-    X(osg_copy_wait_marker) X(osg_timer_mark) X(osg_timer_between) X(osg_tblock_tail_supported) X(osg_tblock_tail) X(osg_tblock_kv_pack_elems) X(osg_tblock_kv_pack_jobs) X(osg_tblock_pack_weight)
+    X(osg_copy_wait_marker) X(osg_timer_mark) X(osg_timer_between) X(osg_tblock_tail_supported) X(osg_tblock_tail) X(osg_tblock_kv_pack_elems) X(osg_tblock_kv_pack_jobs) X(osg_tblock_pack_weight) \
+    X(osg_upconv2x_supported) X(osg_upconv2x_nhwc_v)
 
 struct OsgApi {
 #define OSG_FN(name) decltype(&::name) name = nullptr;
diff --git a/onnxstream_amd/csrc/host/exports.cpp b/onnxstream_amd/csrc/host/exports.cpp
--- a/onnxstream_amd/csrc/host/exports.cpp
+++ b/onnxstream_amd/csrc/host/exports.cpp
@@ -225,6 +225,7 @@
     else if (n == "hip_fuse_ln_gemm") m.m_hip_fuse_ln_gemm = b;
     else if (n == "hip_concat_views") m.m_hip_concat_views = b;
     else if (n == "hip_fuse_tblock") m.m_hip_fuse_tblock = b;
+    else if (n == "hip_fuse_upconv") set_hip_fuse_upconv(m, b);
     else if (n == "hip_gn_stats") m.m_hip_gn_stats = (int)value;
     else if (n == "hip_stream_weights") m.m_hip_stream_weights = b;
     else if (n == "hip_w8_resident") m.m_hip_w8_resident = b;
diff --git a/onnxstream_amd/csrc/host/lowering_graph.inc b/onnxstream_amd/csrc/host/lowering_graph.inc
--- a/onnxstream_amd/csrc/host/lowering_graph.inc
+++ b/onnxstream_amd/csrc/host/lowering_graph.inc
@@ -355,6 +355,7 @@
             if (has_type("osg.SiLU")) { index_graph(); cse_silu(); }
             if (has_type("osg.SiLU") && has_type("Gemm")) { index_graph(); fuse_gemm_act(); }
             if (has_type("Conv")) { index_graph(); fuse_image_bias(); }
+            if (has_type("Resize") && has_type("Conv")) { index_graph(); pair_upconv(); }
         } else if (m.m_fuse_ops_in_attention && has_type("Softmax")) {
             index_graph(); fuse_attention(false);
         }
@@ -1068,6 +1069,52 @@
         }
     }
 
+    void pair_upconv() {
+        if (!P.fuse_upconv || P.u8 || P.w8_resident || P.stream_weights || !P.fp16) return;
+        static const long min_rows = getenv("OSG_UPCONV_MIN_ROWS") ? atol(getenv("OSG_UPCONV_MIN_ROWS")) : osg_up::kMinRowsDefault;
+        for (size_t i = 0; i < ops().size(); i++) {
+            if (!is((int)i, "Resize")) continue;
+            const Operation& rz = ops()[i];
+            if (rz.m_output.size() != 1 || !(rz.m_input.size() == 3 || (rz.m_input.size() == 4 && rz.m_input[3].m_name.empty()))) continue;
+            bool attrs_ok = true;
+            for (auto& a : rz.m_attributes)
+                attrs_ok = attrs_ok && ((a.first == "coordinate_transformation_mode" && a.second == "asymmetric") || (a.first == "mode" && a.second == "nearest") ||
+                                        (a.first == "nearest_mode" && a.second == "floor") || a.first == "cubic_coeff_a");
+            if (!attrs_ok) continue;
+            const Val* sc = cval(rz.m_input[2]);
+            if (!sc || !sc->host_valid || sc->host_f != std::vector<float>{1.f, 1.f, 2.f, 2.f}) continue;
+            const Tensor x = rz.m_input[0];
+            if (!act(x) || x.m_shape.size() != 4 || x.m_shape[0] != 1) continue;
+            const long Cin = (long)x.m_shape[1], H = (long)x.m_shape[2], W = (long)x.m_shape[3];
+            const int cv = sole_consumer(rz.m_output[0]);
+            if (!is(cv, "Conv")) continue;
+            const Operation& co = ops()[cv];
+            if (co.m_output.size() != 1 || co.m_input.size() < 2 || co.m_input.size() > 3 || co.m_input[0].m_name != rz.m_output[0].m_name) continue;
+            if (attr(co, "osg_residual") || attr(co, "osg_image_bias")) continue;
+            bool conv_ok = true;
+            for (auto& a : co.m_attributes) {
+                if (a.first == "dilations") conv_ok = conv_ok && int_list(a.second) == std::vector<int>{1, 1};
+                else if (a.first == "group") conv_ok = conv_ok && std::stoi(a.second) == 1;
+                else if (a.first == "kernel_shape") conv_ok = conv_ok && int_list(a.second) == std::vector<int>{3, 3};
+                else if (a.first == "pads") conv_ok = conv_ok && int_list(a.second) == std::vector<int>{1, 1, 1, 1};
+                else if (a.first == "strides") conv_ok = conv_ok && int_list(a.second) == std::vector<int>{1, 1};
+                else if (a.first != "osg_act") conv_ok = false;
+            }
+            if (!conv_ok || !attr(co, "pads")) continue;
+            const Val* w = cval(co.m_input[1]);
+            if (!w || w->dtype != OSG_F16 || w->lay != Lay::nhwc || w->shape != Shape{w->shape.empty() ? 0 : w->shape[0], Cin, 3, 3} || !w->dptr) continue;
+            if (co.m_input.size() == 3 && !co.m_input[2].m_name.empty() && !cval(co.m_input[2])) continue;
+            const long Cout = w->shape[0];
+            if (N * H * W < min_rows) continue;
+            if (!be.api.osg_upconv2x_supported(OSG_F16, (int)N, (int)H, (int)W, (int)Cin, (int)Cout, 0)) continue;
+            Operation f = co;
+            f.m_input[0] = x;
+            f.m_attributes.emplace_back("osg_up2x", "1");
+            dead[i] = 1;
+            ops()[cv] = std::move(f);
+        }
+    }
+
     void fuse_gemm_act() {
         for (size_t i = 0; i < ops().size(); i++) {
             if (!is((int)i, "Gemm")) continue;
diff --git a/onnxstream_amd/csrc/host/lowering_ops.inc b/onnxstream_amd/csrc/host/lowering_ops.inc
--- a/onnxstream_amd/csrc/host/lowering_ops.inc
+++ b/onnxstream_amd/csrc/host/lowering_ops.inc
@@ -106,7 +106,7 @@
             else if (a.first == "kernel_shape") ks = int_list(a.second);
             else if (a.first == "pads") pads = int_list(a.second);
             else if (a.first == "strides") strides = int_list(a.second);
-            else if (a.first == "osg_residual" || a.first == "osg_image_bias" || a.first == "osg_act") {}
+            else if (a.first == "osg_residual" || a.first == "osg_image_bias" || a.first == "osg_act" || a.first == "osg_up2x") {}
             else throw std::invalid_argument(op.m_type + ": unrecognized attribute: " + a.first + ".");
         }
         int x = in_val(op.m_input[0]);
@@ -140,7 +140,9 @@
         if (!ks.empty()) need(op, ks.size() == 2 && ks[0] == KH && ks[1] == KW, "kernel_shape does not match the weights.");
         const int ph = pads[0] + pads[2], pw = pads[1] + pads[3];
         const int pt = ph / 2, pb = ph - pt, pl = pw / 2, pr = pw - pl;
-        const long Ho = (H + ph - KH) / strides[0] + 1, Wo = (W + pw - KW) / strides[1] + 1;
+        const bool up2x = attr(op, "osg_up2x") != nullptr;
+        if (up2x) need(op, !is1d && !has_res && !has_ib && KH == 3 && KW == 3 && strides[0] == 1 && strides[1] == 1 && ph == 2 && pw == 2 && V(w).dtype == OSG_F16, "invalid up2x form.");
+        const long Ho = up2x ? 2 * H : (H + ph - KH) / strides[0] + 1, Wo = up2x ? 2 * W : (W + pw - KW) / strides[1] + 1;
         int bias = -1;
         if (nin >= 3 && !op.m_input[2].m_name.empty()) {
             bias = in_val(op.m_input[2]);
@@ -168,6 +170,24 @@
         const int qz = w8 ? V(w).qzp : 0;
         auto co = std::make_shared<ConvOut>();
         co->dst = y;
+        if (up2x) {
+            const int wc = weight_up2x(w, Cout, Cin);
+            reads[1] = wc;
+            P.add_step("Conv " + op.m_name + " <up2x", reads, {y}, [=, this] {
+                const ConvOut& o = *co;
+                if (o.sink[0].off >= 0 || o.sink[1].off >= 0)
+                    be.check(be.api.osg_set_stat_sinks(be.ctx, o.sink[0].off >= 0 ? P.gn_stats + o.sink[0].off : nullptr, o.sink[0].groups, o.sink[0].cpg, o.sink[0].ch_off,
+                                                       o.sink[1].off >= 0 ? P.gn_stats + o.sink[1].off : nullptr, o.sink[1].groups, o.sink[1].cpg, o.sink[1].ch_off, o.sink_hw),
+                             "osg_set_stat_sinks");
+                be.check(be.api.osg_upconv2x_nhwc_v(be.ctx, P.ptr(x), P.ptr(wc), bias >= 0 ? P.ptr(bias) : nullptr, bias >= 0 ? P.vals[bias].dtype : OSG_F16,
+                                                    (char*)P.ptr(o.dst) + o.dst_off, o.dst_ld, o.dst2 >= 0 ? (char*)P.ptr(o.dst2) + o.dst2_off : nullptr, o.dst2_ld,
+                                                    (int)nb, (int)H, (int)W, (int)Cin, (int)Cout, cact),
+                         "Conv <up2x");
+            });
+            P.steps.back().flops = 2.0 * nb * Ho * Wo * Cout * 4 * Cin;
+            conv_producers[P.root_of(y)] = ConvProducer{P.steps.size() - 1, co, y};
+            return;
+        }
         P.add_step((w8 ? "Conv w8 " : "Conv ") + op.m_name, reads, {y}, [=, this] {
             const ConvOut& o = *co;
             if (o.sink[0].off >= 0 || o.sink[1].off >= 0)
@@ -193,6 +213,24 @@
         if (V(w).dtype == OSG_F16 || w8) conv_producers[P.root_of(y)] = ConvProducer{P.steps.size() - 1, co, y};
         if (KH == 1 && KW == 1 && sh == 1 && sw == 1 && ph == 0 && pw == 0 && ib < 0 && cact == OSG_ACT_NONE)
             if (!w8) note_rs_producer(x, w, bias, res, y, nb * Ho * Wo, Cout, Cin);
+    }
+
+    int weight_up2x(int w, long Cout, long Cin) {
+        int t = P.new_val("", {4, Cout, 2, 2, Cin}, OSG_F16, Lay::plain, false);
+        Val& tv = V(t);
+        tv.is_const = true;
+        tv.name = V(w).name + "|up2x";
+        const size_t n3 = (size_t)Cout * 9 * Cin, n2 = (size_t)4 * Cout * 4 * Cin;
+        bool fresh;
+        tv.dptr = P.const_alloc(tv.name, n2 * 2, &fresh);
+        if (fresh) {
+            std::vector<uint16_t> src(n3), dst(n2);
+            be.check(be.api.osg_sync(be.ctx), "osg_sync");
+            be.check(be.api.osg_download(be.ctx, src.data(), P.ptr(w), n3 * 2), "osg_download");
+            osg_up::combine_weights(src.data(), Cout, Cin, dst.data());
+            be.check(be.api.osg_upload_sync(be.ctx, tv.dptr, dst.data(), n2 * 2), "osg_upload_sync");
+        }
+        return t;
     }
 
     int weight_nk(int w) {
diff --git a/onnxstream_amd/csrc/host/model.cpp b/onnxstream_amd/csrc/host/model.cpp
--- a/onnxstream_amd/csrc/host/model.cpp
+++ b/onnxstream_amd/csrc/host/model.cpp
@@ -50,6 +50,7 @@
     if (m_pool && m_backend) m_pool->clear(*m_backend);
     delete m_pool;
     delete m_backend;
+    set_hip_fuse_upconv(*this, true);
 }
 
 void Model::hip_fetch_tensor(const std::string& name) {
diff --git a/onnxstream_amd/csrc/host/plan.cpp b/onnxstream_amd/csrc/host/plan.cpp
--- a/onnxstream_amd/csrc/host/plan.cpp
+++ b/onnxstream_amd/csrc/host/plan.cpp
@@ -1,11 +1,13 @@
 #include "plan.h"
 #include "qu8.h"
+#include "../osg_upconv.h"
 
 #include <algorithm>
 #include <chrono>
 #include <cmath>
 #include <cstdio>
 #include <cstring>
+#include <mutex>
 #include <thread>
 #include <string_view>
 #include <unordered_map>
@@ -79,6 +81,20 @@
 
 }
 
+namespace {
+std::mutex g_upconv_off_mutex;
+std::unordered_set<const Model*> g_upconv_off;
+}
+bool hip_fuse_upconv(const Model& m) {
+    std::lock_guard<std::mutex> lock(g_upconv_off_mutex);
+    return g_upconv_off.count(&m) == 0;
+}
+void set_hip_fuse_upconv(const Model& m, bool on) {
+    std::lock_guard<std::mutex> lock(g_upconv_off_mutex);
+    if (on) g_upconv_off.erase(&m);
+    else g_upconv_off.insert(&m);
+}
+
 Plan::Plan(Model& model, HipBackend& backend, ConstPool& cpool, size_t batch) : m(model), be(backend), pool(cpool), N((long)batch) {
     fp16 = m.m_use_fp16_arithmetic;
     fusion = fusion_req = m.m_hip_fusion_level;
@@ -90,6 +106,7 @@
     fuse_ln_gemm = m.m_hip_fuse_ln_gemm;
     concat_views = m.m_hip_concat_views;
     fuse_tblock = m.m_hip_fuse_tblock;
+    fuse_upconv = hip_fuse_upconv(m);
     gn_stats_req = m.m_hip_gn_stats;
     gn_stats_min_elems = m.m_hip_gn_stats == 2 ? (8L << 20) : 0;
     gn_stats_on = m.m_hip_gn_stats != 0 && !stream_weights && m.m_hip_fusion_level >= 2 && !m.m_use_uint8_arithmetic && !m.m_range_data_calibrate;
@@ -114,7 +131,7 @@
     const bool want_stream = mm.m_hip_stream_weights || mm.m_cuda_options.m_vram_to_use > 0;
     if ((long)batch != N) return no("batch size");
     if (mm.m_use_fp16_arithmetic != fp16 || mm.m_use_uint8_arithmetic != u8 || mm.m_use_uint8_qdq != u8_qdq) return no("arithmetic type");
-    if (mm.m_hip_fusion_level != fusion_req || mm.m_hip_fuse_ln_gemm != fuse_ln_gemm || mm.m_hip_concat_views != concat_views || mm.m_hip_fuse_tblock != fuse_tblock || mm.m_hip_gn_stats != gn_stats_req ||
+    if (mm.m_hip_fusion_level != fusion_req || mm.m_hip_fuse_ln_gemm != fuse_ln_gemm || mm.m_hip_concat_views != concat_views || mm.m_hip_fuse_tblock != fuse_tblock || hip_fuse_upconv(mm) != fuse_upconv || mm.m_hip_gn_stats != gn_stats_req ||
         mm.m_fuse_ops_in_attention != fuse_attn || mm.m_use_scaled_dp_attn_op != sdp_attn || mm.m_hip_autotune != autotune)
         return no("fusion / tuning options");
     if (want_stream != stream_weights || (size_t)mm.m_cuda_options.m_vram_to_use != vram_budget ||
@@ -418,7 +435,7 @@
     const bool cacheable = m.m_support_dynamic_shapes && !stream_weights && !budgeted;
     if (cacheable) {
         key = std::to_string(fusion) + "|" + std::to_string(m.m_hip_fusion_level) + (u8 ? "|u8" : "|f") + (fp16 ? "h" : "-") + (w8_resident ? "8" : "-") + (fuse_attn ? "a" : "-") +
-              (sdp_attn ? "s" : "-") + (fuse_ln_gemm ? "l" : "-") + "|" + std::to_string(m.m_attention_fused_ops_parts) + "|" + std::to_string(m.m_ops.size()) + "|";
+              (sdp_attn ? "s" : "-") + (fuse_ln_gemm ? "l" : "-") + (fuse_upconv ? "u" : "-") + "|" + std::to_string(m.m_attention_fused_ops_parts) + "|" + std::to_string(m.m_ops.size()) + "|";
         for (auto& e : extra_outputs) key += e + ",";
         key += "|";
         if (m.m_requires_upcast)
diff --git a/onnxstream_amd/csrc/host/plan.h b/onnxstream_amd/csrc/host/plan.h
--- a/onnxstream_amd/csrc/host/plan.h
+++ b/onnxstream_amd/csrc/host/plan.h
@@ -140,6 +140,9 @@
     return sign ? -v : v;
 }
 
+bool hip_fuse_upconv(const Model& m);
+void set_hip_fuse_upconv(const Model& m, bool on);
+
 struct Plan {
     Plan(Model& m, HipBackend& be, ConstPool& pool, size_t batch);
     ~Plan();
@@ -259,6 +262,7 @@
     bool fuse_ln_gemm = false;
     bool concat_views = true;
     bool fuse_tblock = true;
+    bool fuse_upconv = true;
     bool in_flight = false;
     bool gn_stats_on = false;
     int gn_stats_req = 2;
diff --git a/onnxstream_amd/csrc/osg_conv3x3_kernel.h b/onnxstream_amd/csrc/osg_conv3x3_kernel.h
--- a/onnxstream_amd/csrc/osg_conv3x3_kernel.h
+++ b/onnxstream_amd/csrc/osg_conv3x3_kernel.h
@@ -1,5 +1,6 @@
 #pragma once
 #include "osg_gemm_common.h"
+#include "osg_upconv.h"
 #include <algorithm>
 #include <array>
 #include <cmath>
@@ -21,7 +22,7 @@
 
 template <int N> __device__ __forceinline__ void wait_vmcnt() { asm volatile("s_waitcnt vmcnt(%0)" ::"n"(N) : "memory"); }
 
-template <int W_, int BN, int NLW = 4, int WQ = 0>
+template <int W_, int BN, int NLW = 4, int WQ = 0, int NT = 9>
 struct Geo {
     static constexpr int TI = W_ == 8 ? 2 : 1;
     static constexpr int TH = 128 / (W_ * TI);
@@ -35,9 +36,9 @@
     static constexpr int WLB = ((BN + BRW - 1) / BRW + NLW - 1) / NLW;
     static constexpr int BST_BYTES = WLB * NLW * 1024;
     static constexpr int NSTW_ = (160 * 1024 - 2 * PATCH_BYTES) / BST_BYTES;
-    static constexpr int NSTW = NSTW_ > 8 ? 8 : NSTW_;
+    static constexpr int NSTW = NSTW_ > 8 ? (NT < 8 ? NT : 8) : (NSTW_ > NT ? NT : NSTW_);
     static constexpr int D = NSTW - 1;
-    static constexpr int PT = 10 - D;
+    static constexpr int PT = NT + 1 - D;
     static constexpr int PPT = (NPW + PT - 1) / PT;
     static constexpr size_t SMEM = 2 * (size_t)PATCH_BYTES + (size_t)NSTW * BST_BYTES;
     static constexpr bool OK = D >= 3 && PT >= 2;
@@ -48,14 +49,15 @@
     }
     static constexpr int allowed_outstanding(int t) {
         int n = 0;
-        for (int d = 1; d <= D - 2; d++) n += WLB + patch_loads((t - d + 18) % 9);
+        for (int d = 1; d <= D - 2; d++) n += WLB + patch_loads((t - d + 2 * NT) % NT);
         return n;
     }
 };
 
-template <int W_, int BN, int WGM, int WGN, int MODE, int NLW, int WQ = 0>
+template <int W_, int BN, int WGM, int WGN, int MODE, int NLW, int WQ = 0, int NT = 9>
 __device__ __forceinline__ void conv3x3_body(const GemmParams& p) {
-    using G = Geo<W_, BN, NLW, WQ>;
+    using G = Geo<W_, BN, NLW, WQ, NT>;
+    static_assert(NT == 9 || (NT == 4 && WQ == 0 && MODE == 0), "taps per slab: 9, or the 4 of the up2x form (f16 weights)");
     constexpr int TI = G::TI, TH = G::TH, PW = G::PW, PPI = G::PPI, PP = G::PP, NPW = G::NPW, PATCH_BYTES = G::PATCH_BYTES;
     constexpr int WLB = G::WLB, BST_BYTES = G::BST_BYTES, NSTW = G::NSTW, D = G::D, PPT = G::PPT;
     constexpr int WM = 128 / WGM, WN = BN / WGN, TM = WM / 16, TN = WN / 16;
@@ -87,6 +89,12 @@
         m_tile = L / (p.splits * p.nt); L -= m_tile * p.splits * p.nt;
         zs = L / (p.nt); n_tile = L - zs * p.nt;
     }
+    int up_phase = 0;
+    if constexpr (NT == 4) {
+        const int tiles_low = p.M >> 7;
+        up_phase = osg_up::tile_phase(m_tile, tiles_low);
+        m_tile -= up_phase * tiles_low;
+    }
     const int m0 = m_tile * 128, n0 = n_tile * BN;
     const int slab_b = zs * (p.k_per_split >> 6);
     const int slab_e = min(p.Cin >> 6, slab_b + (p.k_per_split >> 6));
@@ -95,7 +103,7 @@
         const int img0 = m0 / (p.H * W_);
         const int y0 = (m0 - img0 * p.H * W_) / W_;
         __amdgpu_buffer_rsrc_t rsA = __builtin_amdgcn_make_buffer_rsrc((void*)p.A, 0, p.a_bytes, 0x00020000);
-        __amdgpu_buffer_rsrc_t rsB = __builtin_amdgcn_make_buffer_rsrc((void*)p.Bt, 0, p.b_bytes, 0x00020000);
+        __amdgpu_buffer_rsrc_t rsB = __builtin_amdgcn_make_buffer_rsrc((void*)(NT == 4 ? p.Bt + (long)up_phase * p.N * p.K : p.Bt), 0, p.b_bytes, 0x00020000);
         const int rsub = lane >> 3;
         const int gch = (lane & 7) ^ rsub;
         unsigned pa_off[NPW];
@@ -139,20 +147,20 @@
 #pragma unroll
         for (int pc = 0; pc < NPW; pc++) issue_patch_piece(pc, slab_b, patch0);
 #pragma unroll
-        for (int d = 1; d < D; d++) issue_weights(d, d % 9, slab_b + d / 9);
+        for (int d = 1; d < D; d++) issue_weights(d, d % NT, slab_b + d / NT);
         wait_vmcnt<(D - 1) * WLB>();
         __builtin_amdgcn_s_barrier();
         int ust = 0;
         for (int slab = slab_b; slab < slab_e; slab++) {
             char* patch_next = patch0 + (((slab - slab_b) & 1) ^ 1) * PATCH_BYTES;
-            static_for<0, 9>([&](auto tc) {
+            static_for<0, NT>([&](auto tc) {
                 constexpr int t = decltype(tc)::value;
                 wait_vmcnt<G::allowed_outstanding(t)>();
                 if (MODE != 5) __builtin_amdgcn_s_barrier();
-                constexpr int td = (t + D) % 9;
+                constexpr int td = (t + D) % NT;
                 int std_ = ust + D;
                 std_ = std_ >= NSTW ? std_ - NSTW : std_;
-                issue_weights(std_, td, slab + (t + D) / 9);
+                issue_weights(std_, td, slab + (t + D) / NT);
                 static_for<0, G::patch_loads(t)>([&](auto pc) { issue_patch_piece(t * PPT + decltype(pc)::value, slab + 1, patch_next); });
                 ust = ust + 1 == NSTW ? 0 : ust + 1;
             });
@@ -185,6 +193,8 @@
     W8Ops<WQ ? TN : 1, W8SC> w8;
     if constexpr (WQ) w8_prefetch<TN, W8SC>(p, w8, n0, wn0, lane);
 
+    const int up_off = NT == 4 ? osg_up::patch_row(up_phase >> 1, 0) * PW + osg_up::patch_row(up_phase & 1, 0) : 0;
+    auto tap_off = [&](int t) { return NT == 9 ? (t / 3) * PW + t % 3 : up_off + osg_up::patch_row(0, t / 2) * PW + osg_up::patch_row(0, t % 2); };
     f16x8 fa0[TM], fb0[TN], fa1[TM], fb1[TN];
     auto read_frags = [&](f16x8 (&fa)[TM], f16x8 (&fb)[TN], const char* pbuf, const char* bbuf, int tap_off, int ks) {
         if (MODE == 1 || (MODE == 4 && ks == 1)) return;
@@ -236,12 +246,12 @@
     kdbg_stamp(p, 2);
     if constexpr (WQ) {
         w8_finalize<TN, W8SC>(w8);
-        read_a(fa0, patch0, 0, 0);
+        read_a(fa0, patch0, tap_off(0), 0);
         read_codes(rb0, bst0, 0);
         read_codes(rb1, bst0, 1);
         convert(fb0, rb0);
     } else
-    read_frags(fa0, fb0, patch0, bst0, 0, 0);
+    read_frags(fa0, fb0, patch0, bst0, tap_off(0), 0);
     if (MODE == 4) {
 #pragma unroll
         for (int i = 0; i < TM; i++) fa1[i] = fa0[i];
@@ -252,16 +262,15 @@
     for (int slab = slab_b; slab < slab_e; slab++) {
         const char* patch = patch0 + ((slab - slab_b) & 1) * PATCH_BYTES;
         const char* patch_next = patch0 + (((slab - slab_b) & 1) ^ 1) * PATCH_BYTES;
-        static_for<0, 9>([&](auto tc) {
+        static_for<0, NT>([&](auto tc) {
             constexpr int t = decltype(tc)::value;
             if (MODE != 5) __builtin_amdgcn_s_barrier();
-            constexpr int kh = t / 3, kw = t % 3;
             const char* Bs = bst0 + ust * BST_BYTES;
             if constexpr (WQ) {
                 constexpr int KV = (8 * TN + TM * TN - 1) / (TM * TN);
                 const int ustn = ust + 1 == NSTW ? 0 : ust + 1;
                 const char* Bn = bst0 + ustn * BST_BYTES;
-                read_a(fa1, patch, kh * PW + kw, 1);
+                read_a(fa1, patch, tap_off(t), 1);
                 read_codes(rb0, Bn, 0);
                 convert(fb1, rb1);
                 mma(fa0, fb0);
@@ -272,8 +281,8 @@
                 });
                 __builtin_amdgcn_sched_barrier(0);
                 ust = ustn;
-                constexpr int tn8 = (t + 1) % 9;
-                read_a(fa0, t == 8 ? patch_next : patch, (tn8 / 3) * PW + tn8 % 3, 0);
+                constexpr int tn8 = (t + 1) % NT;
+                read_a(fa0, t == NT - 1 ? patch_next : patch, tap_off(tn8), 0);
                 read_codes(rb1, Bn, 1);
                 convert(fb0, rb0);
                 mma(fa1, fb1);
@@ -284,7 +293,7 @@
                 });
                 __builtin_amdgcn_sched_barrier(0);
             } else if constexpr (MODE == 0 || MODE == 7) {
-                read_frags(fa1, fb1, patch, Bs, kh * PW + kw, 1);
+                read_frags(fa1, fb1, patch, Bs, tap_off(t), 1);
                 mma(fa0, fb0);
                 if constexpr (MODE == 0) {
                     static_for<0, TM + TN>([&](auto) { __builtin_amdgcn_sched_group_barrier(0x008, 1, 0); __builtin_amdgcn_sched_group_barrier(0x100, 1, 0); });
@@ -295,8 +304,8 @@
                 }
                 __builtin_amdgcn_sched_barrier(0);
                 ust = ust + 1 == NSTW ? 0 : ust + 1;
-                constexpr int tn6 = (t + 1) % 9;
-                read_frags(fa0, fb0, t == 8 ? patch_next : patch, bst0 + ust * BST_BYTES, (tn6 / 3) * PW + tn6 % 3, 0);
+                constexpr int tn6 = (t + 1) % NT;
+                read_frags(fa0, fb0, t == NT - 1 ? patch_next : patch, bst0 + ust * BST_BYTES, tap_off(tn6), 0);
                 mma(fa1, fb1);
                 if constexpr (MODE == 0) {
                     static_for<0, TM + TN>([&](auto) { __builtin_amdgcn_sched_group_barrier(0x008, 1, 0); __builtin_amdgcn_sched_group_barrier(0x100, 1, 0); });
@@ -307,13 +316,13 @@
                 }
                 __builtin_amdgcn_sched_barrier(0);
             } else {
-            read_frags(fa1, fb1, patch, Bs, kh * PW + kw, 1);
+            read_frags(fa1, fb1, patch, Bs, tap_off(t), 1);
             __builtin_amdgcn_sched_barrier(0);
             mma(fa0, fb0);
             __builtin_amdgcn_sched_barrier(0);
             ust = ust + 1 == NSTW ? 0 : ust + 1;
-            constexpr int tn = (t + 1) % 9;
-            if (MODE != 4) read_frags(fa0, fb0, t == 8 ? patch_next : patch, bst0 + ust * BST_BYTES, (tn / 3) * PW + tn % 3, 0);
+            constexpr int tn = (t + 1) % NT;
+            if (MODE != 4) read_frags(fa0, fb0, t == NT - 1 ? patch_next : patch, bst0 + ust * BST_BYTES, tap_off(tn), 0);
             __builtin_amdgcn_sched_barrier(0);
             mma(fa1, fb1);
             __builtin_amdgcn_sched_barrier(0);
@@ -337,41 +346,44 @@
             return;
         }
     }
+    if constexpr (NT == 4) gemm_epilogue_fast<TM, TN, true, EPRE, false, EPI_ANY, W_>(p, acc, m0, n0, wm0, wn0, lane, 0, epre, stat_lds, up_phase);
+    else
     gemm_epilogue<TM, TN, true, EPRE, false>(p, acc, m0, n0, wm0, wn0, lane, 0, zs, epre, stat_lds);
     kdbg_stamp(p, 5);
     if (OSG_UNLIKELY(p.kdbg != nullptr)) { asm volatile("s_waitcnt vmcnt(0)" ::: "memory"); kdbg_stamp(p, 6); }
 }
 
-template <int W_, int BN, int WGM, int WGN, int MODE, int NLW, int WQ = 0>
+template <int W_, int BN, int WGM, int WGN, int MODE, int NLW, int WQ = 0, int NT = 9>
 __global__ __launch_bounds__(256 + 64 * NLW) void conv3x3_kernel(const void* A, const void* Bt, int M, int N, int K, int k_per_split, unsigned a_bytes, unsigned b_bytes, int grid,
                                                                  int H, int Cin, unsigned sp_nm, GemmParams pk) {
     GemmParams p = pk;
     p.A = (const f16*)A; p.Bt = (const f16*)Bt; p.M = M; p.N = N; p.K = K; p.k_per_split = k_per_split; p.a_bytes = a_bytes; p.b_bytes = b_bytes; p.grid = grid; p.H = H; p.Cin = Cin;
     p.splits = (int)(sp_nm & ((1u << kPackSplitsBits) - 1)); p.n_major = (sp_nm & kPackNMajor) != 0;
-    p.mt = (M + 127) / 128; p.nt = (N + BN - 1) / BN;
+    p.mt = NT == 4 ? 4 * (M >> 7) : (M + 127) / 128; p.nt = (N + BN - 1) / BN;
     p.kdbg = nullptr;
     if (OSG_UNLIKELY(sp_nm & kPackKdbg)) p.kdbg = kernarg_rare(pk.kdbg);
-    conv3x3_body<W_, BN, WGM, WGN, MODE, NLW, WQ>(p);
-}
-
-template <int W_, int BN, int WGM, int WGN, int MODE = 0, int NLW = 4, int WQ = 0>
+    conv3x3_body<W_, BN, WGM, WGN, MODE, NLW, WQ, NT>(p);
+}
+
+template <int W_, int BN, int WGM, int WGN, int MODE = 0, int NLW = 4, int WQ = 0, int NT = 9>
 int launch3(osg_ctx* ctx, GemmParams& p) {
-    constexpr size_t smem = Geo<W_, BN, NLW, WQ>::SMEM;
+    constexpr size_t smem = Geo<W_, BN, NLW, WQ, NT>::SMEM;
     static_assert(smem <= 160 * 1024, "LDS budget");
-    static_assert(Geo<W_, BN, NLW, WQ>::OK, "pipeline depth out of range");
-    auto kern = conv3x3_kernel<W_, BN, WGM, WGN, MODE, NLW, WQ>;
+    static_assert(Geo<W_, BN, NLW, WQ, NT>::OK, "pipeline depth out of range");
+    auto kern = conv3x3_kernel<W_, BN, WGM, WGN, MODE, NLW, WQ, NT>;
     static unsigned long long attr_mask = 0;
     if (osg_first_on_device(attr_mask)) {
         OSG_HIP(ctx, hipFuncSetAttribute((const void*)kern, hipFuncAttributeMaxDynamicSharedMemorySize, (int)smem));
     }
-    p.mt = (p.M + 127) / 128;
+    p.mt = NT == 4 ? 4 * (p.M / 128) : (p.M + 127) / 128;
     p.nt = (p.N + BN - 1) / BN;
     p.no_epre = osg_mm::no_epi_prefetch();
     p.kdbg = kdbg_buffer(ctx, (long)p.mt * p.nt * p.splits);
     const osg_mm::StatSink sinks_in[2] = {p.sink[0], p.sink[1]};
     if (p.sink[0].table || p.sink[1].table) {
-        const bool ok = !ctx->tuning && p.splits == 1 && MODE == 0 && (p.N & 3) == 0 && ((p.ldc | p.ldc2) & 3) == 0 && p.sink_hw > 0 && p.sink_hw % 128 == 0 && p.M % p.sink_hw == 0;
-        if (ok) { ctx->sink_fused = true; p.sink_imgs = p.M / p.sink_hw; p.sink_per_xcd = ctx->xcd_ids8 ? 1 : 0; }
+        constexpr int UP = NT == 4 ? 4 : 1;
+        const bool ok = !ctx->tuning && p.splits == 1 && MODE == 0 && (p.N & 3) == 0 && ((p.ldc | p.ldc2) & 3) == 0 && p.sink_hw > 0 && p.sink_hw % (128 * UP) == 0 && ((long)p.M * UP) % p.sink_hw == 0;
+        if (ok) { ctx->sink_fused = true; p.sink_imgs = (int)((long)p.M * UP / p.sink_hw); p.sink_per_xcd = ctx->xcd_ids8 ? 1 : 0; }
         else p.sink[0].table = p.sink[1].table = nullptr;
     }
     p.grid = p.mt * p.nt * p.splits;
diff --git a/onnxstream_amd/csrc/osg_gemm_common.h b/onnxstream_amd/csrc/osg_gemm_common.h
--- a/onnxstream_amd/csrc/osg_gemm_common.h
+++ b/onnxstream_amd/csrc/osg_gemm_common.h
@@ -4,6 +4,7 @@
 #include "osg_common.h"
 #include "osg_gemm_select.h"
 #include "osg_gemm_epi.h"
+#include "osg_upconv.h"
 
 #include <algorithm>
 #include <type_traits>
@@ -267,7 +268,7 @@
     v += dpp_get<0x128>(v);
     return v;
 }
-template <int TM, int TN>
+template <int TM, int TN, bool UP = false>
 __device__ __forceinline__ void gemm_colstats(const GemmParams& p, const f16x4 (&o)[TM][TN], int mrow0, int ncol0, int lane, float* st) {
     const int mb = mrow0 + (lane & 15);
 #pragma unroll
@@ -291,7 +292,7 @@
             }
         }
     asm volatile("s_waitcnt lgkmcnt(0)" ::: "memory");
-    const int n_img = mrow0 / p.sink_hw;
+    const int n_img = mrow0 / (UP ? p.sink_hw >> 2 : p.sink_hw);
     const int wn = min(TN * 16, p.N - ncol0);
 #pragma unroll
     for (int k = 0; k < 2; k++) {
@@ -335,9 +336,9 @@
     return 0;
 }
 
-template <int TM, int TN, bool RB, bool ON, bool BATCH = true, int EPI = EPI_ANY>
+template <int TM, int TN, bool RB, bool ON, bool BATCH = true, int EPI = EPI_ANY, int UPW = 0>
 __device__ __forceinline__ void gemm_epilogue_fast(const GemmParams& p, f32x4 (&acc)[TM][TN], int m0, int n0, int wm0, int wn0, int lane, int zb,
-                                                   const EpiOps<TM, TN, RB, ON>& pre, float* stat_lds = nullptr) {
+                                                   const EpiOps<TM, TN, RB, ON>& pre, float* stat_lds = nullptr, int up_phase = 0) {
     const int N = p.N;
     f16* __restrict__ C = p.C + zb * p.strideC;
     const f16* __restrict__ R = EPI_ON(EPI_RESIDUAL, p.residual != nullptr) ? p.residual + zb * p.strideC : nullptr;
@@ -517,6 +518,38 @@
     {
         typedef unsigned u32x2 __attribute__((ext_vector_type(2)));
         const int mr = wm0 + (lane & 15), rows_left = p.M - m0;
+        if constexpr (UPW != 0) {
+            constexpr int lw = UPW == 64 ? 6 : UPW == 32 ? 5 : UPW == 16 ? 4 : 3;
+            static_assert(UPW == 1 << lw, "up2x: the low-resolution width is 8, 16, 32 or 64");
+            __amdgpu_buffer_rsrc_t rsC = __builtin_amdgcn_make_buffer_rsrc((void*)C, 0, epi_extent(4 * p.M, ldc, N), 0x00020000);
+            __amdgpu_buffer_rsrc_t rsC2 = __builtin_amdgcn_make_buffer_rsrc((void*)p.C2, 0, p.C2 ? epi_extent(4 * p.M, p.ldc2, N) : 0u, 0x00020000);
+#pragma unroll
+            for (int i = 0; i < TM; i++) {
+                const int r = mr + i * 16;
+                const unsigned orow = (unsigned)osg_up::out_row(m0 + r, lw, up_phase);
+                const bool in = r < rows_left;
+#pragma unroll
+                for (int j = 0; j < TN; j++) {
+                    const int n = nb + j * 16;
+                    const unsigned off = in && n < N ? (orow * (unsigned)ldc + (unsigned)n) * 2u : kEpiOob;
+                    __builtin_amdgcn_raw_buffer_store_b64(__builtin_bit_cast(u32x2, o[i][j]), rsC, off, 0, OSG_EPI_STORE_AUX);
+                }
+            }
+            if (p.C2 != nullptr) {
+#pragma unroll
+                for (int i = 0; i < TM; i++) {
+                    const int r = mr + i * 16;
+                    const unsigned orow = (unsigned)osg_up::out_row(m0 + r, lw, up_phase);
+                    const bool in = r < rows_left;
+#pragma unroll
+                    for (int j = 0; j < TN; j++) {
+                        const int n = nb + j * 16;
+                        const unsigned off = in && n < N ? (orow * (unsigned)p.ldc2 + (unsigned)n) * 2u : kEpiOob;
+                        __builtin_amdgcn_raw_buffer_store_b64(__builtin_bit_cast(u32x2, o[i][j]), rsC2, off, 0, OSG_EPI_STORE_AUX);
+                    }
+                }
+            }
+        } else {
         __amdgpu_buffer_rsrc_t rsC = __builtin_amdgcn_make_buffer_rsrc((void*)(C + (long)m0 * ldc), 0, epi_extent(rows_left, ldc, N), 0x00020000);
 #pragma unroll
         for (int i = 0; i < TM; i++) {
@@ -541,8 +574,10 @@
                 }
             }
         }
+        }
     }
 #else
+    static_assert(UPW == 0, "the up2x row remap exists in the buffer-store form only");
 #pragma unroll
     for (int i = 0; i < TM; i++) {
         const int m = mb + i * 16;
@@ -565,7 +600,7 @@
         }
     }
 #endif
-    if (OSG_UNLIKELY_IF(BATCH, (EPI_ON(EPI_SINKS, stat_lds != nullptr)))) gemm_colstats<TM, TN>(p, o, m0 + wm0, n0 + wn0, lane, stat_lds);
+    if (OSG_UNLIKELY_IF(BATCH, (EPI_ON(EPI_SINKS, stat_lds != nullptr)))) gemm_colstats<TM, TN, UPW != 0>(p, o, m0 + wm0, n0 + wn0, lane, stat_lds);
     if (OSG_UNLIKELY_IF(BATCH, (EPI_ON(EPI_ROWSTATS, p.rs_out != nullptr)))) {
 #pragma unroll
         for (int i = 0; i < TM; i++) {
diff --git a/onnxstream_amd/csrc/osg_upconv.h b/onnxstream_amd/csrc/osg_upconv.h
--- /dev/null
+++ b/onnxstream_amd/csrc/osg_upconv.h
@@ -0,0 +1,81 @@
+#pragma once
+#include "osg_gemm_select.h"
+#include <cstdint>
+#include <cstring>
+
+#if defined(__HIPCC__)
+#define OSG_UP_HD __host__ __device__
+#else
+#define OSG_UP_HD
+#endif
+
+namespace osg_up {
+
+constexpr int tap_lo(int a, int u) { return a == 0 ? (u == 0 ? 0 : 1) : (u == 0 ? 0 : 2); }
+constexpr int tap_hi(int a, int u) { return a == 0 ? (u == 0 ? 0 : 2) : (u == 0 ? 1 : 2); }
+constexpr int patch_row(int a, int u) { return a + u; }
+
+OSG_UP_HD constexpr long out_row(long m, int lw, int phase) {
+    return ((m >> lw) << (lw + 2)) + ((m & ((1L << lw) - 1)) << 1) + (long)(phase >> 1) * (2L << lw) + (phase & 1);
+}
+OSG_UP_HD constexpr int tile_phase(int m_tile, int tiles_low) { return m_tile / tiles_low; }
+
+inline double half_to_double(uint16_t h) {
+    const int s = h >> 15, e = (h >> 10) & 31, m = h & 1023;
+    double v;
+    if (e == 31) v = m ? __builtin_nan("") : __builtin_inf();
+    else if (e == 0) v = (double)m * 5.9604644775390625e-08;
+    else v = (double)(m | 1024) * __builtin_ldexp(1.0, e - 25);
+    return s ? -v : v;
+}
+inline uint16_t double_to_half(double d) {
+    uint64_t x;
+    std::memcpy(&x, &d, 8);
+    const uint16_t sign = (uint16_t)((x >> 48) & 0x8000u);
+    x &= 0x7fffffffffffffffULL;
+    if (x > 0x7ff0000000000000ULL) return (uint16_t)(sign | 0x7e00u);
+    const int e = (int)(x >> 52) - 1023;
+    if (e >= 16) return (uint16_t)(sign | 0x7c00u);
+    if (e < -25) return sign;
+    uint64_t mant = (x & 0xfffffffffffffULL) | (1ULL << 52);
+    const int shift = e >= -14 ? 42 : 42 + (-14 - e);
+    uint64_t h = mant >> shift;
+    const uint64_t rem = mant & ((1ULL << shift) - 1), half = 1ULL << (shift - 1);
+    if (rem > half || (rem == half && (h & 1))) h++;
+    if (e >= -14) h += (uint64_t)(e + 14) << 10;
+    return (uint16_t)(sign | (h > 0x7c00u ? 0x7c00u : h));
+}
+
+inline void combine_weights(const uint16_t* w, long Cout, long Cin, uint16_t* out) {
+    for (int a = 0; a < 2; a++)
+        for (int b = 0; b < 2; b++)
+            for (long o = 0; o < Cout; o++)
+                for (int u = 0; u < 2; u++)
+                    for (int v = 0; v < 2; v++) {
+                        uint16_t* d = out + ((((long)(2 * a + b) * Cout + o) * 2 + u) * 2 + v) * Cin;
+                        for (long c = 0; c < Cin; c++) {
+                            double s = 0.0;
+                            for (int kh = tap_lo(a, u); kh <= tap_hi(a, u); kh++)
+                                for (int kw = tap_lo(b, v); kw <= tap_hi(b, v); kw++) s += half_to_double(w[((o * 3 + kh) * 3 + kw) * Cin + c]);
+                            d[c] = double_to_half(s);
+                        }
+                    }
+}
+
+inline constexpr int kBN = 80, kLoaders = 4;
+inline constexpr long kMinRowsDefault = 512;
+
+constexpr bool takes(long images, int H, int W, int Cin, int Cout, long pitch) {
+    if (images <= 0 || H <= 0 || W <= 0 || Cin <= 0 || Cout <= 0) return false;
+    const long M = images * H * W;
+    if (M > 0x7fffffffL / 4) return false;
+    osg_mm::SelectShape s;
+    s.M = (int)M; s.N = Cout; s.K = 9 * Cin; s.H = H; s.W = W; s.Cin = Cin; s.Ho = H; s.Wo = W; s.KW = 3; s.sh = 1; s.sw = 1; s.pt = 1; s.pl = 1;
+    if (!osg_mm::halo3_takes(s)) return false;
+    if (M % 128) return false;
+    if (pitch < Cout || (pitch & 3)) return false;
+    if ((double)(4 * M) * (double)pitch * 2.0 >= 2147483648.0) return false;
+    return true;
+}
+
+}
diff --git a/onnxstream_amd/csrc/osg_upconv.hip b/onnxstream_amd/csrc/osg_upconv.hip
--- /dev/null
+++ b/onnxstream_amd/csrc/osg_upconv.hip
@@ -0,0 +1,57 @@
+#include "osg_conv3x3_kernel.h"
+
+namespace {
+template <int W_>
+int launch_up(osg_ctx* ctx, GemmParams& p) { return launch3<W_, osg_up::kBN, 4, 1, 0, osg_up::kLoaders, 0, 4>(ctx, p); }
+}
+
+extern "C" {
+
+int osg_upconv2x_supported(osg_dtype w_dtype, int N, int H, int W, int Cin, int Cout, long max_pitch) {
+    const char* off = getenv("OSG_UPCONV_OFF");
+    if ((off && atoi(off) != 0) || w_dtype != OSG_F16) return 0;
+    return osg_up::takes(N, H, W, Cin, Cout, max_pitch > 0 ? max_pitch : (long)Cout) ? 1 : 0;
+}
+
+int osg_upconv2x_nhwc_v(osg_ctx* ctx, const void* x, const void* w_phases, const void* bias, osg_dtype bias_dtype, void* y, long y_ld, void* y2, long y2_ld,
+                        int N, int H, int W, int Cin, int Cout, osg_act act) {
+    if (y_ld < 0 || (y_ld && y_ld < Cout) || (y2 && y2_ld < Cout)) OSG_FAIL(ctx, "osg_upconv2x_nhwc_v: an output pitch is smaller than Cout");
+    if (bias && bias_dtype != OSG_F16 && bias_dtype != OSG_F32) OSG_FAIL(ctx, "osg_upconv2x_nhwc_v: invalid bias dtype");
+    if (act != OSG_ACT_NONE && act != OSG_ACT_SILU) OSG_FAIL(ctx, "osg_upconv2x_nhwc_v: the activation must be none or SiLU");
+    const long ld = y_ld ? y_ld : (long)Cout, ld2 = y2 ? y2_ld : 0;
+    if (!osg_up::takes(N, H, W, Cin, Cout, std::max(ld, ld2))) OSG_FAIL(ctx, "osg_upconv2x_nhwc_v: shape not taken (see osg_upconv2x_supported)");
+    if ((((uintptr_t)x | (uintptr_t)w_phases) & 15) != 0 || (((uintptr_t)y | (uintptr_t)y2) & 7) != 0 || ((uintptr_t)bias & 15) != 0)
+        OSG_FAIL(ctx, "osg_upconv2x_nhwc_v: operands must be 16-byte aligned, output views 8-byte aligned");
+    GemmParams p{};
+    p.A = (const f16*)x; p.Bt = (const f16*)w_phases; p.C = (f16*)y; p.bias = bias;
+    p.M = N * H * W; p.N = Cout; p.K = 4 * Cin; p.lda = 0;
+    p.bias_f32 = bias_dtype == OSG_F32; p.act = act;
+    p.a_bytes_l = (long)p.M * Cin * 2;
+    p.a_bytes = (unsigned)p.a_bytes_l;
+    p.b_bytes = (unsigned)((long)Cout * p.K * 2);
+    p.H = H; p.W = W; p.Cin = Cin; p.Ho = 2 * H; p.Wo = 2 * W; p.KW = 2; p.sh = 1; p.sw = 1; p.pt = 1; p.pl = 1;
+    p.rb_rows = 4 * H * W;
+    p.ldc = y_ld == Cout ? 0 : y_ld; p.C2 = (f16*)y2; p.ldc2 = ld2;
+    p.splits = 1; p.k_per_split = Cin; p.tickets = nullptr; p.fold_acc = 0;
+    p.n_major = (double)Cout * p.K * 2.0 > (double)p.a_bytes_l;
+    bool want_sinks = false;
+    for (int k = 0; k < 2; k++) {
+        const auto& ps = ctx->pending_sink[k];
+        if (ps.table && (k == 0 || y2)) {
+            p.sink[k] = StatSink{ps.table, ps.groups, ps.cpg, ps.ch_off};
+            want_sinks = true;
+        }
+        ctx->pending_sink[k] = osg_ctx::PendingSink{};
+    }
+    p.sink_hw = ctx->pending_hw;
+    ctx->sink_fused = false;
+    if (want_sinks && p.sink_hw != 4 * H * W) OSG_FAIL(ctx, "osg_upconv2x_nhwc_v: the statistics sinks were set for another image size");
+    if (epi_check(ctx, p)) return 1;
+    const int rc = W == 64 ? launch_up<64>(ctx, p) : W == 32 ? launch_up<32>(ctx, p) : W == 16 ? launch_up<16>(ctx, p) : launch_up<8>(ctx, p);
+    if (rc) return rc;
+    osg_set_route(ctx, 4, v3_find(W, osg_up::kBN, osg_up::kLoaders, 0), 1, 0);
+    if (!want_sinks || ctx->sink_fused) return 0;
+    return osg_mm::launch_colstats(ctx, p.C, ld, 4 * p.M, Cout, p.sink_hw, p.sink);
+}
+
+}
diff --git a/onnxstream_amd/osgpu.py b/onnxstream_amd/osgpu.py
--- a/onnxstream_amd/osgpu.py
+++ b/onnxstream_amd/osgpu.py
@@ -26,7 +26,8 @@
     "osg_sampler_prepare_single", "osg_sampler_euler_a_single", "osg_sampler_multistep_single",
     "osg_decode_gather", "osg_decode_blend",
     "osg_range_push", "osg_range_pop", "osg_marker_record", "osg_copy_wait_marker", "osg_timer_mark", "osg_timer_between", "osg_set_stat_sinks", "osg_group_norm_stats_nhwc", "osg_qu8_conv2d_nhwc", "osg_qu8_conv2d_nhwc_t", "osg_qu8_conv_tap_sums", "osg_qu8_gemm", "osg_qu8_lut", "osg_qu8_binary", "osg_qu8_instance_norm", "osg_qu8_instance_norm_nhwc", "osg_qu8_affine_act", "osg_qu8_norm_affine_act_nhwc", "osg_qu8_softmax_last", "osg_kdbg_read",
-    "osg_tblock_tail_supported", "osg_tblock_tail", "osg_tblock_kv_pack_elems", "osg_tblock_kv_pack_jobs", "osg_tblock_pack_weight", 
+    "osg_tblock_tail_supported", "osg_tblock_tail", "osg_tblock_kv_pack_elems", "osg_tblock_kv_pack_jobs", "osg_tblock_pack_weight",
+    "osg_upconv2x_supported", "osg_upconv2x_nhwc_v",
 ]
 
 
@@ -75,6 +76,8 @@
     lib.osg_conv2d_nhwc.argtypes = [vp, ci, vp, vp, vp, ci, vp, vp] + [ci] * 14
     lib.osg_conv2d_nhwc_rb.argtypes = [vp, ci, vp, vp, vp, ci, vp, cl, vp, vp] + [ci] * 14
     lib.osg_conv2d_nhwc_v.argtypes = [vp, ci, vp, vp, vp, ci, vp, cl, vp, vp, cl, vp, cl] + [ci] * 14
+    lib.osg_upconv2x_supported.argtypes = [ci, ci, ci, ci, ci, ci, cl]
+    lib.osg_upconv2x_nhwc_v.argtypes = [vp, vp, vp, vp, ci, vp, cl, vp, cl, ci, ci, ci, ci, ci, ci]
     lib.osg_gemm_w8.argtypes = [vp, vp, vp, cf, ci, vp, ci, vp, vp, ci, ci, ci, ci]
     lib.osg_conv2d_nhwc_w8.argtypes = [vp, vp, vp, cf, ci, vp, ci, vp, cl, vp, vp] + [ci] * 14
     lib.osg_gemm_w8_v.argtypes = [vp, vp, vp, cf, ci, vp, vp, vp, ci, vp, vp, ci, ci, ci, ci]
```
